# maxjaritz/mvpnet

Measured on AMD Instinct MI355X. Metric: chunks/sec (8192 pts, 3x160x120 views) fwd+bwd, higher is better.
Workload: dtype f32; 1 GPU; configs[2]: MVPNet lifting (unproject + pixel k-NN + gather) + FeatureAggregation + PN2SSG full train step (fwd+loss+bwd+Adam), 2D CNN replaced by a resident 64-ch feature map; cfg=mvpnet_3d_unet_resnet34_pn2ssg.yaml, chunks_per_gpu=32, points=8192, views=3x160x120, feature_channels=64, k=3, parallelism=dp1 (one process per GPU, 1 grad all-reduce/step), launch=eager, cpu_affinity=32 logical cpus of 256 (0 .. 183)

## Files before the change

include/mvp_hip.h:

```cpp
#ifndef MVP_HIP_H_
#define MVP_HIP_H_

#include <stdint.h>

#ifdef __cplusplus
extern "C" {
#endif

typedef void* mvp_stream_t;

#define MVP_OK 0
#define MVP_EINVAL (-1)
#define MVP_EUNSUPPORTED (-2)
#define MVP_ENULL (-3)

const char* mvp_version(void);
const char* mvp_strerror(int code);

int mvp_set_fps_mode(int mode);

int mvp_fps_f32(const float* points, int64_t B, int64_t N, int64_t D, int64_t M, int64_t* index, mvp_stream_t stream);
int mvp_fps_f64(const double* points, int64_t B, int64_t N, int64_t D, int64_t M, int64_t* index, mvp_stream_t stream);
int mvp_fps_shape_f32(const float* points, int64_t B, int64_t N, int64_t D, int64_t M, int64_t* index, int shape, mvp_stream_t stream);
int mvp_fps_shape_f64(const double* points, int64_t B, int64_t N, int64_t D, int64_t M, int64_t* index, int shape, mvp_stream_t stream);
// ... 46 lines not shown

int mvp_knn_distance_f32(const float* query, const float* key, int64_t B, int64_t N1, int64_t N2, int64_t k,
                         int64_t* index, float* distance, mvp_stream_t stream);
int mvp_knn_distance_f64(const double* query, const double* key, int64_t B, int64_t N1, int64_t N2, int64_t k,
                         int64_t* index, double* distance, mvp_stream_t stream);
int mvp_knn3_weights_f32(const float* query, const float* key, int64_t B, int64_t N1, int64_t N2, float eps, int64_t* index,
                         float* weight, float* distance, mvp_stream_t stream);

int mvp_interpolate_forward_f32(const float* input, const int64_t* index, const float* weight, int64_t B, int64_t C,
                                int64_t N1, int64_t N2, float* out, mvp_stream_t stream);
int mvp_interpolate_forward_f64(const double* input, const int64_t* index, const double* weight, int64_t B,
                                int64_t C, int64_t N1, int64_t N2, double* out, mvp_stream_t stream);
int mvp_interpolate_backward_f32(const float* grad_out, const int64_t* index, const float* weight, int64_t B,
                                 int64_t C, int64_t N1, int64_t N2, float* grad_in, mvp_stream_t stream);
int mvp_interpolate_backward_f64(const double* grad_out, const int64_t* index, const double* weight, int64_t B,
                                 int64_t C, int64_t N1, int64_t N2, double* grad_in, mvp_stream_t stream);
int mvp_interpolate_forward_strided_f32(const float* input, int64_t sb, int64_t sc, int64_t sn, const int64_t* index, const float* weight,
                                        int64_t B, int64_t C, int64_t N1, int64_t N2, float* out, mvp_stream_t stream);
int mvp_interpolate_forward_strided_f64(const double* input, int64_t sb, int64_t sc, int64_t sn, const int64_t* index, const double* weight,
                                        int64_t B, int64_t C, int64_t N1, int64_t N2, double* out, mvp_stream_t stream);
int mvp_interpolate_backward_strided_f32(const float* grad_out, int64_t sb, int64_t sc, int64_t sn, const int64_t* index,
                                         const float* weight, int64_t B, int64_t C, int64_t N1, int64_t N2, float* grad_in,
                                         mvp_stream_t stream);
int mvp_interpolate_backward_strided_f64(const double* grad_out, int64_t sb, int64_t sc, int64_t sn, const int64_t* index,
                                         const double* weight, int64_t B, int64_t C, int64_t N1, int64_t N2, double* grad_in,
                                         mvp_stream_t stream);
int mvp_interpolate_forward_bf16(const uint16_t* input, const int64_t* index, const float* weight, int64_t B, int64_t C, int64_t N1,
                                 int64_t N2, uint16_t* out, mvp_stream_t stream);
int mvp_interpolate_backward_bf16(const uint16_t* grad_out, const int64_t* index, const float* weight, int64_t B, int64_t C, int64_t N1,
                                  int64_t N2, uint16_t* grad_in, mvp_stream_t stream);
int mvp_interpolate_forward_strided_bf16(const uint16_t* input, int64_t sb, int64_t sc, int64_t sn, const int64_t* index,
                                         const float* weight, int64_t B, int64_t C, int64_t N1, int64_t N2, uint16_t* out,
                                         mvp_stream_t stream);
int mvp_interpolate_backward_strided_bf16(const uint16_t* grad_out, int64_t sb, int64_t sc, int64_t sn, const int64_t* index,
                                          const float* weight, int64_t B, int64_t C, int64_t N1, int64_t N2, uint16_t* grad_in,
                                          mvp_stream_t stream);

int mvp_unproject_f32(const float* depth_m, const float* kinv, const float* pose, const float* box, int64_t B,
                      int64_t nv, int64_t h, int64_t w, float* image_xyz, uint8_t* mask, mvp_stream_t stream);
int mvp_unproject_u16(const uint16_t* depth_mm, const float* kinv, const float* pose, const float* box, int64_t B,
                      int64_t nv, int64_t h, int64_t w, float* image_xyz, uint8_t* mask, mvp_stream_t stream);

int mvp_pixel_knn_bruteforce_f32(const float* image_xyz, const uint8_t* mask, const float* points, int64_t B,
                                 int64_t P, int64_t N, int64_t k, int64_t* index, float* distance,
                                 mvp_stream_t stream);
int mvp_pixel_knn_projective_f32(const float* image_xyz, const uint8_t* mask, const float* points, const float* cam,
                                 const float* pose, int64_t B, int64_t nv, int64_t h, int64_t w, int64_t N,
                                 int64_t k, int64_t* index, float* distance, mvp_stream_t stream);

int mvp_lift_gather_f32(const float* feature, const float* image_xyz, const int64_t* index, int64_t B, int64_t P,
                        int64_t C, int64_t N, int64_t k, float* gfeature, float* gxyz, mvp_stream_t stream);
int mvp_lift_gather_backward_f32(const float* grad_gfeature, const int64_t* index, int64_t B, int64_t P, int64_t C,
                                 int64_t N, int64_t k, float* grad_feature, mvp_stream_t stream);

int64_t mvp_lift_workspace_bytes(int64_t B, int64_t nv, int64_t h, int64_t w, int64_t N);
int mvp_lift_f32(const void* depth, int depth_is_u16, const float* kinv, const float* cam, const float* pose,
                 const float* box, const float* points, const float* feature, int64_t B, int64_t nv, int64_t h,
                 int64_t w, int64_t N, int64_t C, int64_t k, void* workspace, int64_t* knn_index, float* gfeature,
                 float* gxyz, float* image_xyz, uint8_t* mask, mvp_stream_t stream);
int mvp_lift_aug_f32(const void* depth, int depth_is_u16, const float* kinv, const float* cam, const float* pose,
                     const float* box, const float* points, const float* feature, int64_t B, int64_t nv, int64_t h,
                     int64_t w, int64_t N, int64_t C, int64_t k, void* workspace, int64_t* knn_index, float* gfeature,
                     float* gxyz, float* image_xyz, uint8_t* mask, const uint8_t* flip, const double* rot, float* points_out,
                     mvp_stream_t stream);
int mvp_rotate_rows_f32(const float* xyz, const double* rot, int64_t B, int64_t R, float* out, mvp_stream_t stream);

#define MVP_OVERLAP_MAX_BASE 4096
int mvp_frame_overlap_f32(const float* depth_m, const float* kinv, const float* pose, const float* base_points, int64_t F, int64_t h,
                          int64_t w, int64_t nb, float radius, uint32_t* overlap_bits, mvp_stream_t stream);
int mvp_frame_overlap_u16(const uint16_t* depth_mm, const float* kinv, const float* pose, const float* base_points, int64_t F, int64_t h,
                          int64_t w, int64_t nb, float radius, uint32_t* overlap_bits, mvp_stream_t stream);

int mvp_select_frames_u32(const uint32_t* overlap_bits, const uint32_t* chunk_bits, int64_t F, int64_t C, int64_t W, int64_t n_pick,
                          int64_t* picked, int32_t* gain, mvp_stream_t stream);

int mvp_copy_slices_f32(const int64_t* table, int64_t n, mvp_stream_t stream);

int mvp_group_rows_f32(const float* feature, const float* xyz, const float* center, const int64_t* index, int64_t B,
                       int64_t N, int64_t C, int64_t M, int64_t K, int64_t ld, float* out, mvp_stream_t stream);
int mvp_group_rows_backward_f32(const float* grad_out, const int64_t* index, int64_t B, int64_t N, int64_t C, int64_t M,
                                int64_t K, int64_t ld, float* grad_feature, mvp_stream_t stream);
int mvp_relation_rows_f32(const float* feature, const float* src_xyz, const float* tgt_xyz, int64_t R, int64_t K, int64_t C,
                          float* out, mvp_stream_t stream);
int64_t mvp_group_lin_partial_count(int64_t B, int64_t C, int64_t M, int64_t K);
int mvp_group_lin_rows_f32(const float* zf, const float* xyz, const float* centre, const float* wxyz, const int64_t* index,
                           int64_t B, int64_t N, int64_t C, int64_t M, int64_t K, float* out, float* diff, double* stat,
                           double* partial, mvp_stream_t stream);
int mvp_group_lin_rows_bn_f32(const float* zf, const float* xyz, const float* centre, const float* wxyz, const int64_t* index, int64_t B,
                              int64_t N, int64_t C, int64_t M, int64_t K, float* out, float* diff, double* stat, double* partial, float eps,
                              float momentum, float* mean, float* invstd, float* running_mean, float* running_var,
                              int64_t* num_batches_tracked, mvp_stream_t stream);
int mvp_colstats_f32(const float* y, int64_t R, int64_t C, double* stat, double* partial, mvp_stream_t stream);
int64_t mvp_colstats_partial_count(int64_t R, int64_t C);
int mvp_interp_rows_f32(const float* feature, const int64_t* index, const float* weight, int64_t B, int64_t N1, int64_t C,
                        int64_t N2, int64_t ld, float* out, mvp_stream_t stream);
int mvp_csr_build_i64(const int64_t* index, int64_t B, int64_t E, int64_t N, int32_t* offsets, int32_t* slots, int32_t* cursor,
                      mvp_stream_t stream);
int mvp_csr_build_sorted_i64(const int64_t* index, int64_t B, int64_t E, int64_t N, int32_t* offsets, int32_t* slots, int32_t* cursor,
                             mvp_stream_t stream);
int mvp_gather_rows_backward_csr_f32(const float* grad_out, const int32_t* offsets, const int32_t* slots, const float* weight,
                                     int64_t B, int64_t N, int64_t C, int64_t E, int64_t S, int64_t ld, float* grad_feature,
                                     mvp_stream_t stream);
int mvp_gather_rows_backward_csr_finish_f32(const float* dz, const float* y, const float* mean, const float* invstd, const float* gamma,
                                            const double* stat, int training, const int32_t* offsets, const int32_t* slots, const float* weight,
                                            int64_t B, int64_t N, int64_t C, int64_t E, int64_t S, int64_t ld, float* grad_feature,
                                            mvp_stream_t stream);
int mvp_interp_add_rows_f32(const float* feature, const int64_t* index, const float* weight, const float* add, int64_t B, int64_t N1,
                            int64_t C, int64_t N2, float* out, double* stat, double* partial, mvp_stream_t stream);
int mvp_interp_add_rows_bn_f32(const float* feature, const int64_t* index, const float* weight, const float* add, int64_t B, int64_t N1,
                               int64_t C, int64_t N2, float* out, double* stat, double* partial, float eps, float momentum, float* mean,
                               float* invstd, float* running_mean, float* running_var, int64_t* num_batches_tracked, mvp_stream_t stream);
int mvp_interp_rows_backward_f32(const float* grad_out, const int64_t* index, const float* weight, int64_t B, int64_t N1,
                                 int64_t C, int64_t N2, int64_t ld, float* grad_feature, mvp_stream_t stream);
int mvp_bn_rows_forward_f32(const float* y, const float* gamma, const float* beta, int64_t G, int64_t K, int64_t C,
                            int training, float eps, float momentum, int relu, float* running_mean, float* running_var,
                            double* stat, float* mean, float* invstd, float* out, uint8_t* arg, double* partial,
                            mvp_stream_t stream);
int mvp_bn_rows_backward_f32(const float* dsrc, const float* out, const uint8_t* arg, const float* y, const float* mean,
                             const float* invstd, const float* gamma, const float* beta, int64_t G, int64_t K, int64_t C,
                             int relu, int training, double* stat, float* dy, float* dgamma, float* dbeta, double* partial,
                             mvp_stream_t stream);
int mvp_bn_rows_forward_dropout_f32(const float* y, const float* gamma, const float* beta, int64_t R, int64_t C, int training, float eps,
                                    float momentum, int relu, float* running_mean, float* running_var, double* stat, float* mean,
                                    float* invstd, float* out, double* partial, float drop_p, uint64_t seed, mvp_stream_t stream);
int mvp_bn_rows_backward_dropout_f32(const float* dsrc, const float* y, const float* mean, const float* invstd, const float* gamma,
                                     const float* beta, int64_t R, int64_t C, int relu, int training, double* stat, float* dy,
                                     float* dgamma, float* dbeta, double* partial, float drop_p, uint64_t seed, mvp_stream_t stream);
int mvp_bn_rows_backward_finish_f32(const float* dz, const float* y, const float* mean, const float* invstd,
                                    const float* gamma, const float* beta, int64_t R, int64_t C, int training,
                                    const double* stat, float* dy, float* dgamma, float* dbeta, mvp_stream_t stream);
int mvp_bn_finalize_f32(const double* stat, int64_t R, int64_t C, float eps, float momentum, float* mean, float* invstd,
                        float* running_mean, float* running_var, int64_t* num_batches_tracked, mvp_stream_t stream);
int mvp_sa_fused_forward_f32(const float* zf, const float* xyz, const float* centre, const int64_t* index, const float* wxyz, int64_t B,
                             int64_t N, int64_t M, int64_t K, int64_t C1, const float* bn1_mean, const float* bn1_invstd,
                             const float* bn1_gamma, const float* bn1_beta, const float* W2, int64_t C2, const float* bn2_mean,
                             const float* bn2_invstd, const float* bn2_gamma, const float* bn2_beta, const float* W3, int64_t C3,
                             const float* bn3_mean, const float* bn3_invstd, const float* bn3_gamma, const float* bn3_beta, float* out,
                             uint8_t* arg, mvp_stream_t stream);

int mvp_set_mlp_precision(int terms, int min_width);
int mvp_get_mlp_precision(void);
int mvp_set_mlp_precision_backward(int terms);
int mvp_get_mlp_precision_backward(void);
int mvp_mlp_precision_scope(int terms, int terms_backward);
int mvp_adam_step_f32(void* const* params, const void* const* grads, void* const* exp_avg, void* const* exp_avg_sq, const int64_t* numel,
                      int64_t n, double lr, double beta1, double beta2, double eps, double weight_decay, double step, mvp_stream_t stream);

int mvp_mlp_forward_bf16(const uint16_t* X, int64_t R, int64_t Cin, int64_t ldx, const float* W, int64_t ldw, int64_t Cout,
                         const float* bias, const float* scale, const float* shift, int relu, uint16_t* Y, int64_t ldy,
                         mvp_stream_t stream);

int mvp_set_mlp_stream(int on);

int mvp_mlp_forward_f32(const float* X, int64_t R, int64_t Cin, int64_t ldx, const float* W, int64_t ldw, int64_t Cout,
                        const float* act_mean, const float* act_invstd, const float* act_gamma, const float* act_beta,
                        const float* bias, float* Y, double* stat, double* partial, mvp_stream_t stream);
int mvp_mlp_forward_bn_f32(const float* X, int64_t R, int64_t Cin, int64_t ldx, const float* W, int64_t ldw, int64_t Cout,
                           const float* act_mean, const float* act_invstd, const float* act_gamma, const float* act_beta, float* Y,
                           double* stat, double* partial, float eps, float momentum, float* mean, float* invstd, float* running_mean,
                           float* running_var, int64_t* num_batches_tracked, mvp_stream_t stream);
int mvp_mlp_forward_rel_bn_f32(const float* X, int64_t R, int64_t Cin, int64_t ldx, const float* W, int64_t ldw, int64_t Cout, const float* rel,
                               const float* wrel, float* Y, double* stat, double* partial, float eps, float momentum, float* mean,
                               float* invstd, float* running_mean, float* running_var, int64_t* num_batches_tracked, mvp_stream_t stream);
int mvp_relation4_rows_f32(const float* src_xyz, const float* tgt_xyz, int64_t R, int64_t K, float* out, mvp_stream_t stream);
int mvp_mlp_forward_pool_f32(const float* X, int64_t R, int64_t Cin, int64_t ldx, const float* W, int64_t ldw, int64_t Cout,
                             const float* act_mean, const float* act_invstd, const float* act_gamma, const float* act_beta, float* ymax,
                             float* ymin, uint8_t* amax, uint8_t* amin, double* stat, double* partial, float eps, float momentum,
                             float* mean, float* invstd, float* running_mean, float* running_var, int64_t* num_batches_tracked,
                             mvp_stream_t stream);
int mvp_pool_finalize_f32(const float* ymax, const float* ymin, const uint8_t* amax, const uint8_t* amin, const float* mean,
                          const float* invstd, const float* gamma, const float* beta, int64_t G, int64_t C, int relu, float* out,
                          uint8_t* arg, float* ysel, mvp_stream_t stream);
int mvp_pool_backward_stats_f32(const float* dout, const float* out, const float* ysel, const float* mean, const float* invstd,
                                int64_t G, int64_t C, int relu, double* stat, double* partial, mvp_stream_t stream);
int mvp_mlp_input_grad_f32(const float* dY, int64_t R, int64_t Cout, const float* W, int64_t Cin, const float* y_prev,
                           const float* mean, const float* invstd, const float* gamma, const float* beta, float* dZ,
                           double* stat, double* partial, mvp_stream_t stream);
int mvp_mlp_input_grad_dropout_f32(const float* dY, int64_t R, int64_t Cout, const float* W, int64_t Cin, const float* y_prev,
                                   const float* mean, const float* invstd, const float* gamma, const float* beta, float drop_p,
                                   uint64_t drop_seed, float* dZ, double* stat, double* partial, mvp_stream_t stream);

int64_t mvp_mlp_layer_backward_partial_count(int64_t R, int64_t Cp);
int mvp_mlp_layer_backward_f32(const float* G, const float* Yi, const float* mean_i, const float* invstd_i, const float* gamma_i,
                               const double* stat_i, float* dgamma_i, float* dbeta_i, int training, const float* X, int64_t ldx,
                               const float* act_mean, const float* act_invstd, const float* act_gamma, const float* act_beta,
                               const float* W, int64_t ldw, int64_t R, int64_t C, int64_t Cp, float* dW, int64_t lddw, float* dZ,
                               double* stat_prev, double* partial, const float* pool_dout, const float* pool_out,
                               const uint8_t* pool_arg, mvp_stream_t stream);
int mvp_mlp_layer_backward_ws_f32(const float* G, const float* Yi, const float* mean_i, const float* invstd_i, const float* gamma_i,
                               const double* stat_i, float* dgamma_i, float* dbeta_i, int training, const float* X, int64_t ldx,
                               const float* act_mean, const float* act_invstd, const float* act_gamma, const float* act_beta,
                               const float* W, int64_t ldw, int64_t R, int64_t C, int64_t Cp, float* dW, int64_t lddw, float* dZ,
                               double* stat_prev, double* partial, const float* pool_dout, const float* pool_out,
                               const uint8_t* pool_arg, float* workspace, int64_t workspace_floats, mvp_stream_t stream);
int mvp_mlp_layer_backward_wide_p_f32(const float* G, const float* Yi, const float* mean_i, const float* invstd_i, const float* gamma_i,
                                      const float* beta_i, const double* stat_i, float* dgamma_i, float* dbeta_i, int training, int mode,
                                      float drop_p, uint64_t drop_seed, const float* X, int64_t ldx, const float* act_mean,
                                      const float* act_invstd, const float* act_gamma, const float* act_beta, const float* W, int64_t ldw,
                                      int64_t R, int64_t C, int64_t Cp, float* dW, int64_t lddw, float* dZ, double* stat_prev, int* ticket,
                                      float* workspace, int64_t workspace_floats, int precision, int precision_backward, mvp_stream_t stream);
int mvp_mlp_layer_backward_wide_pooled_p_f32(const float* G, const float* Yi, const float* mean_i, const float* invstd_i, const float* gamma_i,
                                             const float* beta_i, const double* stat_i, float* dgamma_i, float* dbeta_i, int training, int mode,
                                             int64_t pool_k, float drop_p, uint64_t drop_seed, const float* X, int64_t ldx, const float* act_mean,
                                             const float* act_invstd, const float* act_gamma, const float* act_beta, const float* W, int64_t ldw,
                                             int64_t R, int64_t C, int64_t Cp, float* dW, int64_t lddw, float* dZ, double* stat_prev, int* ticket,
                                             float* workspace, int64_t workspace_floats, int precision, int precision_backward, mvp_stream_t stream);
int mvp_mlp_weight_grad_finish_p_f32(const float* dZ, const float* Y, const float* mean, const float* invstd, const float* gamma, const double* stat,
                                     int training, const float* X, int64_t R, int64_t Cout, int64_t Cin, int64_t ldx, float* dW, int64_t lddw,
                                     float* workspace, int64_t workspace_floats, int precision, int precision_backward, mvp_stream_t stream);
int mvp_mlp_weight_grad_finish_rel_p_f32(const float* dZ, const float* Y, const float* mean, const float* invstd, const float* gamma, const double* stat,
                                         int training, const float* X, int64_t R, int64_t Cout, int64_t Cin, int64_t ldx, const float* REL, float* dW,
                                         float* dWrel, int64_t lddw, int precision, int precision_backward, mvp_stream_t stream);
int mvp_mlp_weight_grad_finish_act_p_f32(const float* dZ, const float* Y, const float* mean, const float* invstd, const float* gamma, const double* stat,
                                         int training, const float* X, int64_t R, int64_t Cout, int64_t Cin, int64_t ldx, const float* act_mean,
                                         const float* act_invstd, const float* act_gamma, const float* act_beta, float* dW, int64_t lddw,
                                         float* workspace, int64_t workspace_floats, int precision, int precision_backward, mvp_stream_t stream);
int64_t mvp_mlp_input_grad_wide_workspace_bytes(int64_t C, int64_t Cp);
int mvp_mlp_input_grad_wide_p_f32(const float* G, const float* Yi, const float* mean_i, const float* invstd_i, const float* gamma_i,
                                  const double* stat_i, float* dgamma_i, float* dbeta_i, int training, const float* X, int64_t ldx,
                                  const float* act_mean, const float* act_invstd, const float* act_gamma, const float* act_beta, const float* W,
                                  int64_t ldw, int64_t R, int64_t C, int64_t Cp, float* dZ, double* stat_prev, void* workspace,
                                  int64_t workspace_bytes, int precision, int precision_backward, mvp_stream_t stream);
int mvp_mlp_weight_grad_f32(const float* dY, const float* X, int64_t R, int64_t Cout, int64_t Cin, int64_t ldx,
                            const float* act_mean, const float* act_invstd, const float* act_gamma, const float* act_beta,
                            float* dW, int64_t lddw, mvp_stream_t stream);
int64_t mvp_mlp_weight_grad_workspace_floats(void);
int mvp_mlp_weight_grad_ws_f32(const float* dY, const float* X, int64_t R, int64_t Cout, int64_t Cin, int64_t ldx,
                               const float* act_mean, const float* act_invstd, const float* act_gamma, const float* act_beta,
                               float* dW, int64_t lddw, float* workspace, int64_t workspace_floats, mvp_stream_t stream);

int mvp_sa_train_forward_f32(int stage, const float* zf, const float* xyz, const float* centre, const int64_t* index, const float* wxyz,
                             int64_t B, int64_t N, int64_t M, int64_t K, int64_t C1, const float* bn1_mean, const float* bn1_invstd,
                             const float* bn1_gamma, const float* bn1_beta, const float* W2, int64_t C2, const float* bn2_mean,
                             const float* bn2_invstd, const float* bn2_gamma, const float* bn2_beta, const float* W3, int64_t C3,
                             double* stat, float eps, float momentum, float* mean, float* invstd, float* running_mean,
                             float* running_var, int64_t* num_batches_tracked, float* ymax, float* ymin, uint8_t* amax, uint8_t* amin,
                             mvp_stream_t stream);
int mvp_sa_train_backward_f32(int layer, const float* zf, const float* xyz, const float* centre, const int64_t* index, const float* wxyz,
                              int64_t B, int64_t N, int64_t M, int64_t K, int64_t C1, const float* bn1_mean, const float* bn1_invstd,
                              const float* bn1_gamma, const float* bn1_beta, const float* W2, int64_t C2, const float* bn2_mean,
                              const float* bn2_invstd, const float* bn2_gamma, const float* bn2_beta, const float* W3, int64_t C3,
                              const float* mean_i, const float* invstd_i, const float* gamma_i, const double* stat_i, float* dgamma_i,
                              float* dbeta_i, int training, const float* G, const float* pool_dout, const float* pool_out,
                              const uint8_t* pool_arg, float* dW, int64_t lddw, float* dZ, double* stat_prev, float* tsum, mvp_stream_t stream);
int mvp_sa_train_backward1_f32(const float* dz1, const int32_t* offsets, const int32_t* slots, const float* zf, const float* dsum,
                               const float* wxyz, const float* tsum, const double* zsum, const double* gsum, int64_t B, int64_t N, int64_t M,
                               int64_t K, int64_t C1, const float* mean, const float* invstd, const float* gamma, const double* stat,
                               int training, float* dgamma, float* dbeta, float* gz, float* dWxyz, int64_t lddw, mvp_stream_t stream);
int mvp_sa_geom_sums_f32(const int32_t* offsets, const int32_t* slots, const float* xyz, const float* centre, int64_t B, int64_t N, int64_t M,
                         int64_t K, float* dsum, double* gsum, mvp_stream_t stream);
int mvp_sa_train_stats1_f32(const float* zf, const float* dsum, const float* wxyz, const double* gsum, int64_t B, int64_t N, int64_t M, int64_t K,
                            int64_t C1, double* stat, double* zsum, float eps, float momentum, float* mean, float* invstd, float* running_mean,
                            float* running_var, int64_t* num_batches_tracked, mvp_stream_t stream);
int mvp_sa_train_stats1_ws_f32(const float* zf, const float* dsum, const float* wxyz, const double* gsum, int64_t B, int64_t N, int64_t M, int64_t K,
                               int64_t C1, double* stat, double* zsum, float eps, float momentum, float* mean, float* invstd, float* running_mean,
                               float* running_var, int64_t* num_batches_tracked, double* scratch, int64_t scratch_doubles, mvp_stream_t stream);

int mvp_mlp_forward_p_f32(const float* X, int64_t R, int64_t Cin, int64_t ldx, const float* W, int64_t ldw, int64_t Cout, const
    float* act_mean, const float* act_invstd, const float* act_gamma, const float* act_beta, const float* bias, float* Y,
    double* stat, double* partial, int precision, int precision_backward, mvp_stream_t stream);
int mvp_mlp_forward_bn_p_f32(const float* X, int64_t R, int64_t Cin, int64_t ldx, const float* W, int64_t ldw, int64_t Cout,
    const float* act_mean, const float* act_invstd, const float* act_gamma, const float* act_beta, float* Y, double* stat,
    double* partial, float eps, float momentum, float* mean, float* invstd, float* running_mean, float* running_var, int64_t*
    num_batches_tracked, int precision, int precision_backward, mvp_stream_t stream);
int mvp_mlp_forward_rel_bn_p_f32(const float* X, int64_t R, int64_t Cin, int64_t ldx, const float* W, int64_t ldw, int64_t Cout,
    const float* rel, const float* wrel, float* Y, double* stat, double* partial, float eps, float momentum, float* mean, float*
    invstd, float* running_mean, float* running_var, int64_t* num_batches_tracked, int precision, int precision_backward,
    mvp_stream_t stream);
int mvp_mlp_forward_pool_p_f32(const float* X, int64_t R, int64_t Cin, int64_t ldx, const float* W, int64_t ldw, int64_t Cout,
    const float* act_mean, const float* act_invstd, const float* act_gamma, const float* act_beta, float* ymax, float* ymin,
    uint8_t* amax, uint8_t* amin, double* stat, double* partial, float eps, float momentum, float* mean, float* invstd, float*
    running_mean, float* running_var, int64_t* num_batches_tracked, int precision, int precision_backward, mvp_stream_t stream);
int mvp_mlp_input_grad_p_f32(const float* dY, int64_t R, int64_t Cout, const float* W, int64_t Cin, const float* y_prev, const
    float* mean, const float* invstd, const float* gamma, const float* beta, float* dZ, double* stat, double* partial, int
    precision, int precision_backward, mvp_stream_t stream);
int mvp_mlp_input_grad_dropout_p_f32(const float* dY, int64_t R, int64_t Cout, const float* W, int64_t Cin, const float* y_prev, const
    float* mean, const float* invstd, const float* gamma, const float* beta, float drop_p, uint64_t drop_seed, float* dZ, double* stat,
    double* partial, int precision, int precision_backward, mvp_stream_t stream);
int mvp_mlp_weight_grad_p_f32(const float* dY, const float* X, int64_t R, int64_t Cout, int64_t Cin, int64_t ldx, const float*
    act_mean, const float* act_invstd, const float* act_gamma, const float* act_beta, float* dW, int64_t lddw, int precision,
    int precision_backward, mvp_stream_t stream);
int mvp_mlp_weight_grad_ws_p_f32(const float* dY, const float* X, int64_t R, int64_t Cout, int64_t Cin, int64_t ldx, const
    float* act_mean, const float* act_invstd, const float* act_gamma, const float* act_beta, float* dW, int64_t lddw, float*
    workspace, int64_t workspace_floats, int precision, int precision_backward, mvp_stream_t stream);
int mvp_mlp_layer_backward_p_f32(const float* G, const float* Yi, const float* mean_i, const float* invstd_i, const float*
    gamma_i, const double* stat_i, float* dgamma_i, float* dbeta_i, int training, const float* X, int64_t ldx, const float*
    act_mean, const float* act_invstd, const float* act_gamma, const float* act_beta, const float* W, int64_t ldw, int64_t R,
    int64_t C, int64_t Cp, float* dW, int64_t lddw, float* dZ, double* stat_prev, double* partial, const float* pool_dout, const
    float* pool_out, const uint8_t* pool_arg, int precision, int precision_backward, mvp_stream_t stream);
int mvp_mlp_layer_backward_ws_p_f32(const float* G, const float* Yi, const float* mean_i, const float* invstd_i, const float*
    gamma_i, const double* stat_i, float* dgamma_i, float* dbeta_i, int training, const float* X, int64_t ldx, const float*
    act_mean, const float* act_invstd, const float* act_gamma, const float* act_beta, const float* W, int64_t ldw, int64_t R,
    int64_t C, int64_t Cp, float* dW, int64_t lddw, float* dZ, double* stat_prev, double* partial, const float* pool_dout, const
    float* pool_out, const uint8_t* pool_arg, float* workspace, int64_t workspace_floats, int precision, int precision_backward,
    mvp_stream_t stream);
int mvp_sa_fused_forward_p_f32(const float* zf, const float* xyz, const float* centre, const int64_t* index, const float* wxyz,
    int64_t B, int64_t N, int64_t M, int64_t K, int64_t C1, const float* bn1_mean, const float* bn1_invstd, const float*
    bn1_gamma, const float* bn1_beta, const float* W2, int64_t C2, const float* bn2_mean, const float* bn2_invstd, const float*
    bn2_gamma, const float* bn2_beta, const float* W3, int64_t C3, const float* bn3_mean, const float* bn3_invstd, const float*
    bn3_gamma, const float* bn3_beta, float* out, uint8_t* arg, int precision, int precision_backward, mvp_stream_t stream);

int mvp_sa_train_forward_p_f32(int stage, const float* zf, const float* xyz, const float* centre, const int64_t* index, const
    float* wxyz, int64_t B, int64_t N, int64_t M, int64_t K, int64_t C1, const float* bn1_mean, const float* bn1_invstd, const
    float* bn1_gamma, const float* bn1_beta, const float* W2, int64_t C2, const float* bn2_mean, const float* bn2_invstd, const
    float* bn2_gamma, const float* bn2_beta, const float* W3, int64_t C3, double* stat, float eps, float momentum, float* mean,
    float* invstd, float* running_mean, float* running_var, int64_t* num_batches_tracked, float* ymax, float* ymin, uint8_t*
// ... 35 lines not shown
```

mvpnet_amd/_lib.py:

```python
import ctypes
import os

import torch

_HERE = os.path.dirname(os.path.abspath(__file__))
LIB_PATH = os.environ.get('MVP_LIBRARY') or os.path.join(_HERE, 'libmvp_hip.so')
_lib = None
MLP_PRECISIONS = {'fp32': 0, 'bf16': 1, 'bf16x3': 3, 'bf16x6': 6}

_i64 = ctypes.c_int64
_ptr = ctypes.c_void_p
_f32 = ctypes.c_float

_SIGNATURES = {
    'mvp_fps_f32': [_ptr, _i64, _i64, _i64, _i64, _ptr, _ptr],
    'mvp_fps_f64': [_ptr, _i64, _i64, _i64, _i64, _ptr, _ptr],
    'mvp_fps_shape_f32': [_ptr, _i64, _i64, _i64, _i64, _ptr, ctypes.c_int, _ptr],
    'mvp_fps_shape_f64': [_ptr, _i64, _i64, _i64, _i64, _ptr, ctypes.c_int, _ptr],
    'mvp_fps_checked_f32': [_ptr, _i64, _i64, _i64, _i64, _ptr, ctypes.c_int, _ptr, _ptr],
    'mvp_fps_centroid_levels_f32': [_ptr, _ptr, _i64, _i64, _i64, _i64, _i64, _ptr, _ptr, _ptr],
    'mvp_ball_query_f32': [_ptr, _ptr, _i64, _i64, _i64, _f32, _i64, _ptr, _ptr],
    'mvp_ball_query_f64': [_ptr, _ptr, _i64, _i64, _i64, _f32, _i64, _ptr, _ptr],
    'mvp_ball_query_distance_f32': [_ptr, _ptr, _i64, _i64, _i64, _f32, _i64, _ptr, _ptr, _ptr],
    'mvp_ball_query_distance_f64': [_ptr, _ptr, _i64, _i64, _i64, _f32, _i64, _ptr, _ptr, _ptr],
    'mvp_ball_query_grid_f32': [_ptr, _ptr, _i64, _i64, _i64, _f32, _i64, _ptr, _ptr, _ptr, _i64, _ptr],
    'mvp_knn3_grid_f32': [_ptr, _ptr, _i64, _i64, _i64, _f32, _ptr, _ptr, _ptr, _ptr, _i64, _ptr],
    'mvp_group_points_forward_strided_f32': [_ptr, _i64, _i64, _i64, _ptr, _i64, _i64, _i64, _i64, _i64, _ptr, _ptr],
    'mvp_group_points_backward_strided_f32': [_ptr, _i64, _i64, _i64, _i64, _ptr, _i64, _i64, _i64, _i64, _i64, _ptr, _ptr],
    'mvp_interpolate_forward_strided_f32': [_ptr, _i64, _i64, _i64, _ptr, _ptr, _i64, _i64, _i64, _i64, _ptr, _ptr],
    'mvp_interpolate_backward_strided_f32': [_ptr, _i64, _i64, _i64, _ptr, _ptr, _i64, _i64, _i64, _i64, _ptr, _ptr],
    'mvp_group_points_forward_strided_f64': [_ptr, _i64, _i64, _i64, _ptr, _i64, _i64, _i64, _i64, _i64, _ptr, _ptr],
    'mvp_group_points_forward_strided_bf16': [_ptr, _i64, _i64, _i64, _ptr, _i64, _i64, _i64, _i64, _i64, _ptr, _ptr],
    'mvp_group_points_backward_strided_f64': [_ptr, _i64, _i64, _i64, _i64, _ptr, _i64, _i64, _i64, _i64, _i64, _ptr, _ptr],
    'mvp_group_points_backward_strided_bf16': [_ptr, _i64, _i64, _i64, _i64, _ptr, _i64, _i64, _i64, _i64, _i64, _ptr, _ptr],
    'mvp_interpolate_forward_strided_f64': [_ptr, _i64, _i64, _i64, _ptr, _ptr, _i64, _i64, _i64, _i64, _ptr, _ptr],
    'mvp_interpolate_forward_strided_bf16': [_ptr, _i64, _i64, _i64, _ptr, _ptr, _i64, _i64, _i64, _i64, _ptr, _ptr],
    'mvp_interpolate_backward_strided_f64': [_ptr, _i64, _i64, _i64, _ptr, _ptr, _i64, _i64, _i64, _i64, _ptr, _ptr],
    'mvp_interpolate_backward_strided_bf16': [_ptr, _i64, _i64, _i64, _ptr, _ptr, _i64, _i64, _i64, _i64, _ptr, _ptr],
    'mvp_group_points_forward_f32': [_ptr, _ptr, _i64, _i64, _i64, _i64, _i64, _ptr, _ptr],
    'mvp_group_points_forward_f64': [_ptr, _ptr, _i64, _i64, _i64, _i64, _i64, _ptr, _ptr],
    'mvp_group_points_forward_bf16': [_ptr, _ptr, _i64, _i64, _i64, _i64, _i64, _ptr, _ptr],
    'mvp_group_points_backward_f32': [_ptr, _ptr, _i64, _i64, _i64, _i64, _i64, _ptr, _ptr],
    'mvp_group_points_backward_f64': [_ptr, _ptr, _i64, _i64, _i64, _i64, _i64, _ptr, _ptr],
    'mvp_group_points_backward_bf16': [_ptr, _ptr, _i64, _i64, _i64, _i64, _i64, _ptr, _ptr],
    'mvp_knn_distance_f32': [_ptr, _ptr, _i64, _i64, _i64, _i64, _ptr, _ptr, _ptr],
    'mvp_knn_distance_f64': [_ptr, _ptr, _i64, _i64, _i64, _i64, _ptr, _ptr, _ptr],
    'mvp_knn3_weights_f32': [_ptr, _ptr, _i64, _i64, _i64, _f32, _ptr, _ptr, _ptr, _ptr],
    'mvp_interpolate_forward_f32': [_ptr, _ptr, _ptr, _i64, _i64, _i64, _i64, _ptr, _ptr],
    'mvp_interpolate_forward_f64': [_ptr, _ptr, _ptr, _i64, _i64, _i64, _i64, _ptr, _ptr],
    'mvp_interpolate_forward_bf16': [_ptr, _ptr, _ptr, _i64, _i64, _i64, _i64, _ptr, _ptr],
    'mvp_interpolate_backward_f32': [_ptr, _ptr, _ptr, _i64, _i64, _i64, _i64, _ptr, _ptr],
    'mvp_interpolate_backward_f64': [_ptr, _ptr, _ptr, _i64, _i64, _i64, _i64, _ptr, _ptr],
    'mvp_interpolate_backward_bf16': [_ptr, _ptr, _ptr, _i64, _i64, _i64, _i64, _ptr, _ptr],
    'mvp_unproject_f32': [_ptr, _ptr, _ptr, _ptr, _i64, _i64, _i64, _i64, _ptr, _ptr, _ptr],
    'mvp_unproject_u16': [_ptr, _ptr, _ptr, _ptr, _i64, _i64, _i64, _i64, _ptr, _ptr, _ptr],
    'mvp_pixel_knn_bruteforce_f32': [_ptr, _ptr, _ptr, _i64, _i64, _i64, _i64, _ptr, _ptr, _ptr],
    'mvp_pixel_knn_projective_f32': [_ptr, _ptr, _ptr, _ptr, _ptr, _i64, _i64, _i64, _i64, _i64, _i64, _ptr, _ptr, _ptr],
    'mvp_lift_gather_f32': [_ptr, _ptr, _ptr, _i64, _i64, _i64, _i64, _i64, _ptr, _ptr, _ptr],
    'mvp_lift_gather_backward_f32': [_ptr, _ptr, _i64, _i64, _i64, _i64, _i64, _ptr, _ptr],
    'mvp_lift_f32': [_ptr, ctypes.c_int, _ptr, _ptr, _ptr, _ptr, _ptr, _ptr, _i64, _i64, _i64, _i64, _i64, _i64, _i64, _ptr,
                     _ptr, _ptr, _ptr, _ptr, _ptr, _ptr],
    'mvp_lift_aug_f32': [_ptr, ctypes.c_int, _ptr, _ptr, _ptr, _ptr, _ptr, _ptr, _i64, _i64, _i64, _i64, _i64, _i64, _i64, _ptr,
                         _ptr, _ptr, _ptr, _ptr, _ptr, _ptr, _ptr, _ptr, _ptr],
    'mvp_rotate_rows_f32': [_ptr, _ptr, _i64, _i64, _ptr, _ptr],
    'mvp_copy_slices_f32': [_ptr, _i64, _ptr],
    'mvp_group_rows_f32': [_ptr, _ptr, _ptr, _ptr, _i64, _i64, _i64, _i64, _i64, _i64, _ptr, _ptr],
    'mvp_group_rows_backward_f32': [_ptr, _ptr, _i64, _i64, _i64, _i64, _i64, _i64, _ptr, _ptr],
    'mvp_group_lin_rows_f32': [_ptr, _ptr, _ptr, _ptr, _ptr, _i64, _i64, _i64, _i64, _i64, _ptr, _ptr, _ptr, _ptr, _ptr],
    'mvp_group_lin_rows_bn_f32': [_ptr, _ptr, _ptr, _ptr, _ptr, _i64, _i64, _i64, _i64, _i64, _ptr, _ptr, _ptr, _ptr, _f32, _f32, _ptr, _ptr, _ptr, _ptr, _ptr, _ptr],
    'mvp_colstats_f32': [_ptr, _i64, _i64, _ptr, _ptr, _ptr],
    'mvp_relation_rows_f32': [_ptr, _ptr, _ptr, _i64, _i64, _i64, _ptr, _ptr],
    'mvp_interp_rows_f32': [_ptr, _ptr, _ptr, _i64, _i64, _i64, _i64, _i64, _ptr, _ptr],
    'mvp_mlp_forward_bf16': [_ptr, _i64, _i64, _i64, _ptr, _i64, _i64, _ptr, _ptr, _ptr, ctypes.c_int, _ptr, _i64, _ptr],
    'mvp_adam_step_f32': [_ptr, _ptr, _ptr, _ptr, _ptr, _i64] + [ctypes.c_double] * 6 + [_ptr],
    'mvp_csr_build_i64': [_ptr, _i64, _i64, _i64, _ptr, _ptr, _ptr, _ptr],
    'mvp_csr_build_sorted_i64': [_ptr, _i64, _i64, _i64, _ptr, _ptr, _ptr, _ptr],
    'mvp_gather_rows_backward_csr_f32': [_ptr, _ptr, _ptr, _ptr, _i64, _i64, _i64, _i64, _i64, _i64, _ptr, _ptr],
    'mvp_gather_rows_backward_csr_finish_f32': [_ptr, _ptr, _ptr, _ptr, _ptr, _ptr, ctypes.c_int, _ptr, _ptr, _ptr, _i64, _i64, _i64, _i64, _i64, _i64, _ptr, _ptr],
    'mvp_interp_add_rows_f32': [_ptr, _ptr, _ptr, _ptr, _i64, _i64, _i64, _i64, _ptr, _ptr, _ptr, _ptr],
    'mvp_interp_add_rows_bn_f32': [_ptr, _ptr, _ptr, _ptr, _i64, _i64, _i64, _i64, _ptr, _ptr, _ptr, _f32, _f32, _ptr, _ptr, _ptr, _ptr, _ptr, _ptr],
    'mvp_interp_rows_backward_f32': [_ptr, _ptr, _ptr, _i64, _i64, _i64, _i64, _i64, _ptr, _ptr],
    'mvp_bn_rows_forward_f32': [_ptr, _ptr, _ptr, _i64, _i64, _i64, ctypes.c_int, _f32, _f32, ctypes.c_int, _ptr, _ptr, _ptr, _ptr,
                                _ptr, _ptr, _ptr, _ptr, _ptr],
    'mvp_bn_rows_backward_f32': [_ptr, _ptr, _ptr, _ptr, _ptr, _ptr, _ptr, _ptr, _i64, _i64, _i64, ctypes.c_int, ctypes.c_int, _ptr,
                                 _ptr, _ptr, _ptr, _ptr, _ptr],
    'mvp_bn_rows_forward_dropout_f32': [_ptr, _ptr, _ptr, _i64, _i64, ctypes.c_int, _f32, _f32, ctypes.c_int, _ptr, _ptr, _ptr, _ptr, _ptr, _ptr,
                                        _ptr, _f32, ctypes.c_uint64, _ptr],
    'mvp_bn_rows_backward_dropout_f32': [_ptr, _ptr, _ptr, _ptr, _ptr, _ptr, _i64, _i64, ctypes.c_int, ctypes.c_int, _ptr, _ptr, _ptr, _ptr,
                                         _ptr, _f32, ctypes.c_uint64, _ptr],
    'mvp_bn_rows_backward_finish_f32': [_ptr, _ptr, _ptr, _ptr, _ptr, _ptr, _i64, _i64, ctypes.c_int, _ptr, _ptr, _ptr, _ptr, _ptr],
    'mvp_bn_finalize_f32': [_ptr, _i64, _i64, _f32, _f32, _ptr, _ptr, _ptr, _ptr, _ptr, _ptr],
    'mvp_mlp_weight_grad_f32': [_ptr, _ptr, _i64, _i64, _i64, _i64, _ptr, _ptr, _ptr, _ptr, _ptr, _i64, _ptr],
    'mvp_mlp_weight_grad_ws_f32': [_ptr, _ptr, _i64, _i64, _i64, _i64, _ptr, _ptr, _ptr, _ptr, _ptr, _i64, _ptr, _i64, _ptr],
    'mvp_mlp_input_grad_f32': [_ptr, _i64, _i64, _ptr, _i64, _ptr, _ptr, _ptr, _ptr, _ptr, _ptr, _ptr, _ptr, _ptr],
    'mvp_mlp_input_grad_dropout_f32': [_ptr, _i64, _i64, _ptr, _i64, _ptr, _ptr, _ptr, _ptr, _ptr, _f32, ctypes.c_uint64, _ptr, _ptr, _ptr, _ptr],
    'mvp_mlp_layer_backward_f32': [_ptr, _ptr, _ptr, _ptr, _ptr, _ptr, _ptr, _ptr, ctypes.c_int, _ptr, _i64, _ptr, _ptr, _ptr, _ptr, _ptr, _i64,
                                   _i64, _i64, _i64, _ptr, _i64, _ptr, _ptr, _ptr, _ptr, _ptr, _ptr, _ptr],
    'mvp_mlp_layer_backward_ws_f32': [_ptr, _ptr, _ptr, _ptr, _ptr, _ptr, _ptr, _ptr, ctypes.c_int, _ptr, _i64, _ptr, _ptr, _ptr, _ptr, _ptr, _i64,
                                   _i64, _i64, _i64, _ptr, _i64, _ptr, _ptr, _ptr, _ptr, _ptr, _ptr, _ptr, _i64, _ptr],
    'mvp_mlp_forward_pool_f32': [_ptr, _i64, _i64, _i64, _ptr, _i64, _i64, _ptr, _ptr, _ptr, _ptr, _ptr, _ptr, _ptr, _ptr, _ptr, _ptr, _f32, _f32,
                                 _ptr, _ptr, _ptr, _ptr, _ptr, _ptr],
    'mvp_pool_finalize_f32': [_ptr, _ptr, _ptr, _ptr, _ptr, _ptr, _ptr, _ptr, _i64, _i64, ctypes.c_int, _ptr, _ptr, _ptr, _ptr],
    'mvp_pool_backward_stats_f32': [_ptr, _ptr, _ptr, _ptr, _ptr, _i64, _i64, ctypes.c_int, _ptr, _ptr, _ptr],
    'mvp_sa_fused_forward_f32': [_ptr, _ptr, _ptr, _ptr, _ptr, _i64, _i64, _i64, _i64, _i64, _ptr, _ptr, _ptr, _ptr, _ptr, _i64, _ptr, _ptr, _ptr,
                                 _ptr, _ptr, _i64, _ptr, _ptr, _ptr, _ptr, _ptr, _ptr, _ptr],
    'mvp_sa_train_forward_f32': [ctypes.c_int, _ptr, _ptr, _ptr, _ptr, _ptr, _i64, _i64, _i64, _i64, _i64, _ptr, _ptr, _ptr, _ptr, _ptr, _i64, _ptr, _ptr,
                                 _ptr, _ptr, _ptr, _i64, _ptr, _f32, _f32, _ptr, _ptr, _ptr, _ptr, _ptr, _ptr, _ptr, _ptr, _ptr, _ptr],
    'mvp_sa_train_backward_f32': [ctypes.c_int, _ptr, _ptr, _ptr, _ptr, _ptr, _i64, _i64, _i64, _i64, _i64, _ptr, _ptr, _ptr, _ptr, _ptr, _i64, _ptr, _ptr,
                                  _ptr, _ptr, _ptr, _i64, _ptr, _ptr, _ptr, _ptr, _ptr, _ptr, ctypes.c_int, _ptr, _ptr, _ptr, _ptr, _ptr, _i64, _ptr, _ptr,
                                  _ptr, _ptr],
    'mvp_sa_train_backward1_f32': [_ptr, _ptr, _ptr, _ptr, _ptr, _ptr, _ptr, _ptr, _ptr, _i64, _i64, _i64, _i64, _i64, _ptr, _ptr, _ptr, _ptr,
                                   ctypes.c_int, _ptr, _ptr, _ptr, _ptr, _i64, _ptr],
    'mvp_pn2_plan_f32': [_ptr, _i64, _i64, _i64, _ptr, _ptr, _ptr, _ptr, ctypes.c_int, ctypes.c_int, _f32, _ptr, _i64, _ptr, _ptr, _ptr],
    'mvp_sa_geom_sums_f32': [_ptr, _ptr, _ptr, _ptr, _i64, _i64, _i64, _i64, _ptr, _ptr, _ptr],
    'mvp_sa_train_stats1_f32': [_ptr, _ptr, _ptr, _ptr, _i64, _i64, _i64, _i64, _i64, _ptr, _ptr, _f32, _f32, _ptr, _ptr, _ptr, _ptr, _ptr, _ptr],
    'mvp_sa_train_stats1_ws_f32': [_ptr, _ptr, _ptr, _ptr, _i64, _i64, _i64, _i64, _i64, _ptr, _ptr, _f32, _f32, _ptr, _ptr, _ptr, _ptr, _ptr, _ptr, _i64, _ptr],
    'mvp_mlp_forward_bn_f32': [_ptr, _i64, _i64, _i64, _ptr, _i64, _i64, _ptr, _ptr, _ptr, _ptr, _ptr, _ptr, _ptr, _f32, _f32, _ptr, _ptr, _ptr,
                               _ptr, _ptr, _ptr],
    'mvp_mlp_forward_rel_bn_f32': [_ptr, _i64, _i64, _i64, _ptr, _i64, _i64, _ptr, _ptr, _ptr, _ptr, _ptr, _f32, _f32, _ptr, _ptr, _ptr, _ptr, _ptr, _ptr],
    'mvp_relation4_rows_f32': [_ptr, _ptr, _i64, _i64, _ptr, _ptr],
    'mvp_mlp_forward_f32': [_ptr, _i64, _i64, _i64, _ptr, _i64, _i64, _ptr, _ptr, _ptr, _ptr, _ptr, _ptr, _ptr, _ptr, _ptr],
    'mvp_vote_accumulate_f32': [_ptr, _i64, _i64, _ptr, _i64, _i64, _ptr, _ptr, _ptr],
    'mvp_vote_gather_f32': [_ptr, _i64, _i64, _i64, _ptr, _i64, _ptr, _ptr, _i64, _i64, _ptr, _ptr, _ptr],
    'mvp_vote_finish_f32': [_ptr, _ptr, _i64, _i64, _ptr, _ptr, _ptr],
    'mvp_seg_loss_f32': [_ptr, _i64, _i64, _i64, _i64, _i64, _i64, _ptr, _ptr, _i64, _ptr, _ptr, _ptr],
    'mvp_seg_loss_backward_f32': [_ptr, _i64, _i64, _i64, _i64, _i64, _i64, _ptr, _ptr, _i64, _ptr, _ptr, _ptr, _i64, _i64, _i64, _ptr],
    'mvp_seg_confusion_f32': [_ptr, _i64, _i64, _i64, _i64, _i64, _i64, _ptr, _i64, _ptr, _ptr],
    'mvp_frame_overlap_f32': [_ptr, _ptr, _ptr, _ptr, _i64, _i64, _i64, _i64, _f32, _ptr, _ptr],
    'mvp_frame_overlap_u16': [_ptr, _ptr, _ptr, _ptr, _i64, _i64, _i64, _i64, _f32, _ptr, _ptr],
    'mvp_select_frames_u32': [_ptr, _ptr, _i64, _i64, _i64, _i64, _ptr, _ptr, _ptr],
}
for _n in ['mvp_mlp_forward_f32', 'mvp_mlp_forward_bn_f32', 'mvp_mlp_forward_rel_bn_f32', 'mvp_mlp_forward_pool_f32', 'mvp_mlp_input_grad_f32', 'mvp_mlp_input_grad_dropout_f32',
           'mvp_mlp_weight_grad_f32', 'mvp_mlp_weight_grad_ws_f32', 'mvp_mlp_layer_backward_f32', 'mvp_mlp_layer_backward_ws_f32',
           'mvp_sa_fused_forward_f32', 'mvp_sa_train_forward_f32', 'mvp_sa_train_backward_f32']:
    _SIGNATURES[_n[:-4] + '_p_f32'] = _SIGNATURES[_n][:-1] + [ctypes.c_int, ctypes.c_int, _ptr]
_SIGNATURES['mvp_mlp_layer_backward_wide_p_f32'] = [_ptr] * 9 + [ctypes.c_int, ctypes.c_int, _f32, ctypes.c_uint64, _ptr, _i64, _ptr, _ptr, _ptr, _ptr, _ptr, _i64,
                                                    _i64, _i64, _i64, _ptr, _i64, _ptr, _ptr, _ptr, _ptr, _i64, ctypes.c_int, ctypes.c_int, _ptr]
_SIGNATURES['mvp_mlp_layer_backward_wide_pooled_p_f32'] = [_ptr] * 9 + [ctypes.c_int, ctypes.c_int, _i64, _f32, ctypes.c_uint64, _ptr, _i64, _ptr, _ptr, _ptr, _ptr, _ptr, _i64,
                                                           _i64, _i64, _i64, _ptr, _i64, _ptr, _ptr, _ptr, _ptr, _i64, ctypes.c_int, ctypes.c_int, _ptr]
_SIGNATURES['mvp_mlp_weight_grad_finish_p_f32'] = [_ptr] * 6 + [ctypes.c_int, _ptr, _i64, _i64, _i64, _i64, _ptr, _i64, _ptr, _i64, ctypes.c_int, ctypes.c_int, _ptr]
_SIGNATURES['mvp_mlp_weight_grad_finish_rel_p_f32'] = [_ptr] * 6 + [ctypes.c_int, _ptr, _i64, _i64, _i64, _i64, _ptr, _ptr, _ptr, _i64, ctypes.c_int, ctypes.c_int, _ptr]
_SIGNATURES['mvp_mlp_weight_grad_finish_act_p_f32'] = [_ptr] * 6 + [ctypes.c_int, _ptr, _i64, _i64, _i64, _i64, _ptr, _ptr, _ptr, _ptr, _ptr, _i64, _ptr, _i64, ctypes.c_int,
                                                        ctypes.c_int, _ptr]
_SIGNATURES['mvp_mlp_input_grad_wide_p_f32'] = [_ptr] * 8 + [ctypes.c_int, _ptr, _i64, _ptr, _ptr, _ptr, _ptr, _ptr, _i64, _i64, _i64, _i64, _ptr, _ptr, _ptr, _i64,
                                                 ctypes.c_int, ctypes.c_int, _ptr]
EXPORTS = ['mvp_version', 'mvp_strerror', 'mvp_lift_workspace_bytes', 'mvp_ball_query_grid_workspace', 'mvp_knn3_grid_workspace', 'mvp_mlp_weight_grad_workspace_floats', 'mvp_mlp_input_grad_wide_workspace_bytes', 'mvp_group_lin_partial_count', 'mvp_colstats_partial_count',
           'mvp_set_mlp_precision', 'mvp_get_mlp_precision', 'mvp_mlp_layer_backward_partial_count', 'mvp_set_mlp_stream', 'mvp_set_mlp_precision_backward', 'mvp_get_mlp_precision_backward', 'mvp_mlp_precision_scope', 'mvp_set_fps_mode', 'mvp_fps_debug_spin_limit', 'mvp_fps_last_kernel'] + sorted(_SIGNATURES)


def lib():
    global _lib
    if _lib is None:
        if not os.path.exists(LIB_PATH):
            raise RuntimeError('libmvp_hip.so is not built: run `python -c "import __graft_entry__ as g; g.build()"` '
                               'or `make -C mvpnet_amd/csrc` ({})'.format(LIB_PATH))
        handle = ctypes.CDLL(LIB_PATH)
        handle.mvp_version.restype = ctypes.c_char_p
        handle.mvp_strerror.restype = ctypes.c_char_p
        handle.mvp_strerror.argtypes = [ctypes.c_int]
        handle.mvp_lift_workspace_bytes.restype = ctypes.c_int64
        handle.mvp_lift_workspace_bytes.argtypes = [_i64, _i64, _i64, _i64, _i64]
        handle.mvp_ball_query_grid_workspace.restype = ctypes.c_int64
        handle.mvp_ball_query_grid_workspace.argtypes = [_i64, _i64, _i64]
        handle.mvp_knn3_grid_workspace.restype = ctypes.c_int64
        handle.mvp_knn3_grid_workspace.argtypes = [_i64, _i64, _i64]
        handle.mvp_group_lin_partial_count.restype = ctypes.c_int64
        handle.mvp_group_lin_partial_count.argtypes = [_i64, _i64, _i64, _i64]
        handle.mvp_mlp_weight_grad_workspace_floats.restype = ctypes.c_int64
        handle.mvp_mlp_weight_grad_workspace_floats.argtypes = []
        handle.mvp_mlp_input_grad_wide_workspace_bytes.restype = ctypes.c_int64
        handle.mvp_mlp_input_grad_wide_workspace_bytes.argtypes = [ctypes.c_int64, ctypes.c_int64]
        handle.mvp_colstats_partial_count.restype = ctypes.c_int64
        handle.mvp_colstats_partial_count.argtypes = [_i64, _i64]
        handle.mvp_set_mlp_precision.restype = ctypes.c_int
        handle.mvp_set_mlp_precision.argtypes = [ctypes.c_int, ctypes.c_int]
        handle.mvp_get_mlp_precision.restype = ctypes.c_int
        handle.mvp_get_mlp_precision.argtypes = []
        handle.mvp_mlp_layer_backward_partial_count.restype = ctypes.c_int64
        handle.mvp_mlp_layer_backward_partial_count.argtypes = [_i64, _i64]
        for name, argtypes in _SIGNATURES.items():
            fn = getattr(handle, name)
            fn.argtypes = argtypes
            fn.restype = ctypes.c_int
        _lib = handle
        handle.mvp_set_mlp_stream.restype = ctypes.c_int
        handle.mvp_set_mlp_stream.argtypes = [ctypes.c_int]
        handle.mvp_set_fps_mode.restype = ctypes.c_int
        handle.mvp_set_fps_mode.argtypes = [ctypes.c_int]
        handle.mvp_fps_debug_spin_limit.restype = ctypes.c_int
        handle.mvp_fps_debug_spin_limit.argtypes = [ctypes.c_int]
        handle.mvp_fps_last_kernel.restype = ctypes.c_int
        handle.mvp_fps_last_kernel.argtypes = []
        if os.environ.get('MVP_MLP_STREAM') is not None:
            handle.mvp_set_mlp_stream(int(os.environ['MVP_MLP_STREAM']))
        handle.mvp_set_mlp_precision_backward.restype = ctypes.c_int
        handle.mvp_set_mlp_precision_backward.argtypes = [ctypes.c_int]
        handle.mvp_get_mlp_precision_backward.restype = ctypes.c_int
        handle.mvp_get_mlp_precision_backward.argtypes = []
        handle.mvp_mlp_precision_scope.restype = ctypes.c_int
        handle.mvp_mlp_precision_scope.argtypes = [ctypes.c_int, ctypes.c_int]
        if os.environ.get('MVP_MLP_PRECISION_BWD'):
            check(handle.mvp_set_mlp_precision_backward(MLP_PRECISIONS[os.environ['MVP_MLP_PRECISION_BWD']]), 'mvp_set_mlp_precision_backward')
        env = os.environ.get('MVP_MLP_PRECISION')
        if env:
            set_mlp_precision(env, int(os.environ.get('MVP_MLP_MIN_WIDTH', '0')))
    return _lib




def set_mlp_precision(name, min_width=0):
    if name not in MLP_PRECISIONS:
        raise ValueError('mlp precision must be one of {}'.format(sorted(MLP_PRECISIONS)))
    check(lib().mvp_set_mlp_precision(MLP_PRECISIONS[name], int(min_width)), 'mvp_set_mlp_precision')
    global _mlp_min_width
    _mlp_min_width = int(min_width)


_mlp_min_width = 0


def mlp_min_width():
    return _mlp_min_width


def set_mlp_precision_backward(name):
    if name not in ('bf16', 'bf16x3', 'bf16x6'):
        raise ValueError("backward mlp precision must be 'bf16', 'bf16x3' or 'bf16x6'")
    check(lib().mvp_set_mlp_precision_backward(MLP_PRECISIONS[name]), 'mvp_set_mlp_precision_backward')


class mlp_precision:

    def __init__(self, forward=None, backward=None):
        self.terms = -1 if forward is None else MLP_PRECISIONS[forward]
        self.bwd = -1 if backward is None else MLP_PRECISIONS[backward]
        if self.bwd == 0:
            raise ValueError("backward mlp precision must be 'bf16', 'bf16x3' or 'bf16x6'")

    def __enter__(self):
        old = lib().mvp_mlp_precision_scope(self.terms, self.bwd)
        if old < 0:
            check(old, 'mvp_mlp_precision_scope')
        self.old = (old // 16 - 1, old % 16 - 1)
        return self

    def __exit__(self, *exc):
        lib().mvp_mlp_precision_scope(*self.old)


def current_precision():
    h = lib()
    return (h.mvp_get_mlp_precision(), h.mvp_get_mlp_precision_backward())


def get_mlp_precision():
    terms = lib().mvp_get_mlp_precision()
    return {v: k for k, v in MLP_PRECISIONS.items()}[terms]


_FPS_STATUS = {}


def fps_status(device):
    t = _FPS_STATUS.get(device)
    if t is None:
        t = _FPS_STATUS[device] = torch.zeros(1, dtype=torch.int32, device=device)
    return t


def fps_timed_out(device=None, reset=False):
    device = torch.device('cuda', torch.cuda.current_device()) if device is None else torch.device(device)
    t = _FPS_STATUS.get(device)
    if t is None:
        return False
    hit = bool(int(t.item()))
    if reset:
        t.zero_()
    return hit


def check(code, what):
    if code != 0:
        raise RuntimeError('{} failed: {} (code {})'.format(what, lib().mvp_strerror(code).decode(), code))


def stream_of(t):
    return ctypes.c_void_p(torch.cuda.current_stream(t.device).cuda_stream)


def ptr(t):
    return None if t is None else t.data_ptr()


def ptr_at(t, element_offset):
    return t.data_ptr() + int(element_offset) * t.element_size()


def require_gpu(*tensors):
    for t in tensors:
        if t is None:
            continue
        if not t.is_cuda:
            raise RuntimeError('mvpnet_amd ops run on the GPU only (got a {} tensor); there is no CPU fallback'.format(t.device))
        if not t.is_contiguous():
            raise RuntimeError('tensor must be contiguous')


def suffix(t):
    if t.dtype == torch.float32:
        return 'f32'
    if t.dtype == torch.float64:
        return 'f64'
    raise RuntimeError('expected a float32 or float64 tensor, got {}'.format(t.dtype))


def value_suffix(t):
    return 'bf16' if t.dtype == torch.bfloat16 else suffix(t)


_FN = {}
_raw_stream = getattr(torch._C, '_cuda_getCurrentRawStream', None)
_raw_device = getattr(torch._C, '_cuda_getDevice', None)


def _fn(name):
    f = _FN.get(name)
    if f is None:
        f = _FN[name] = getattr(_lib if _lib is not None else lib(), name)
    return f


DW_WORKSPACE = os.environ.get('MVP_DETERMINISTIC', '0') == '1'


def set_deterministic(flag):
    global DW_WORKSPACE
    old, DW_WORKSPACE = DW_WORKSPACE, bool(flag)
    return old
# ... 55 lines not shown
```

mvpnet_amd/csrc/mlp.hip:

```cpp
#include "common.h"
#include "stats_reduce.h"
#include "mlp_common.h"
#include "dropout.h"
#include <algorithm>

int mvp_mlp_stream_forward(const float* X, int64_t R, int Cin, int ldx, const float* W, int ldw, int Cout, const float* act_mean,
                           const float* act_invstd, const float* act_gamma, const float* act_beta, const float* bias, float* Y,
                           double* stat, double* partial, int ns, float bn_eps, float bn_momentum, float* bn_mean, float* bn_invstd,
                           float* bn_running_mean, float* bn_running_var, int64_t* bn_num_batches, float* ymax, float* ymin,
                           uint8_t* amax, uint8_t* amin, hipStream_t s);

int g_mlp_terms = 6;
int g_mlp_terms_bwd = 3;
int g_mlp_min_width = 0;
thread_local int tl_mlp_terms = -1;
thread_local int tl_mlp_terms_bwd = -1;
int g_mlp_stream = 1;

namespace {


constexpr int kMT = 256;
constexpr int kBM = 128;


struct EpiBwd {
  const float* y;
  const float* mean;
  const float* invstd;
  const float* gamma;
  const float* beta;
  const float* rel;
  const float* wrel;
  Dropout drop;
};

#ifndef MVP_MFMA_PRIO
#define MVP_MFMA_PRIO 2
#endif
#ifndef MVP_DW_PRIO
#define MVP_DW_PRIO 2
#endif
constexpr int kMaxActCin = 512;

#ifndef MVP_MLP_WAVES128
#define MVP_MLP_WAVES128 3
#endif
template <int BN, int BK, bool WT, bool VEC, int ACT, int NS>
__global__ __launch_bounds__(kMT, (BN == 128 && VEC && WT && NS == 0) ? MVP_MLP_WAVES128 : (NS != 0 && BN == 128) ? 2 : 1) void mlp_fwd_kernel(const float* __restrict__ X, int64_t R, int Cin, int ldx,
                                                      const float* __restrict__ W, int ldw, int Cout,
                                                      InAct act, const float* __restrict__ bias, EpiBwd epi,
                                                      float* __restrict__ Y , double* __restrict__ stat,
                                                      double* __restrict__ partial) {
  static_assert(NS == 0 || (VEC && BK == 32), "split-bf16 needs the vector path and 32-wide slabs");
  constexpr int kLdB = BK + 4;
  constexpr int NT = BK / 8;
  constexpr int kColB = 80;
  constexpr int kPieceB = BN * kColB;
  constexpr int kBufB = NS == 0 ? BN * kLdB * 4 : NS * kPieceB;
  __shared__ __attribute__((aligned(16))) unsigned char BsRaw[2 * kBufB];
  float* const Bs0 = reinterpret_cast<float*>(BsRaw);
  __shared__ __attribute__((aligned(16))) float Ps[4][kMaxActCin];
  constexpr int kLdS = 36;
  constexpr int kSsFloats = 4 * 32 * kLdS;
  constexpr bool kAliasS = sizeof(float) * kSsFloats + sizeof(double) * 2 * 4 * BN <= (size_t)2 * kBufB;
  __shared__ __attribute__((aligned(16))) float Ss_own[kAliasS ? 4 : kSsFloats];
  float (*Ss)[32 * kLdS] = reinterpret_cast<float (*)[32 * kLdS]>(kAliasS ? Bs0 : &Ss_own[0]);
  static_assert(sizeof(double) * 2 * 4 * BN <= (size_t)2 * kBufB, "sred must fit in Bs");
  double (*sred)[4][BN] = reinterpret_cast<double (*)[4][BN]>(Bs0 + (kAliasS ? kSsFloats : 0));
  constexpr int NB = BN / 32;
  const int tid = threadIdx.x, lane = tid & 63, wave = tid >> 6;
  const int64_t row0 = (int64_t)blockIdx.x * kBM;
  const int col0 = blockIdx.y * BN;
  const int li = lane & 31, lh = lane >> 5;

  f32x16 acc[NB];
#pragma unroll
  for (int j = 0; j < NB; ++j)
#pragma unroll
    for (int i = 0; i < 16; ++i) acc[j][i] = 0.f;

  constexpr bool has_act = ACT != 0;
  constexpr bool act_lds = ACT == 1;
  if constexpr (act_lds) {
    for (int k = tid; k < min(kMaxActCin, (Cin + BK - 1) / BK * BK); k += kMT) {
      const int kc = min(k, Cin - 1);
      Ps[0][k] = act.mean[kc];
      Ps[1][k] = act.invstd[kc];
      Ps[2][k] = act.gamma[kc];
      Ps[3][k] = act.beta[kc];
    }
  }

  const int64_t arow = row0 + wave * 32 + li;
  const bool arow_ok = arow < R;
  const float* xrow = X + (size_t)(arow_ok ? arow : 0) * ldx;
  float4 an[NT];
  auto load_a = [&](int k0) {
#pragma unroll
    for (int t = 0; t < NT; ++t) {
      const int k = k0 + 8 * t + 4 * lh;
      if constexpr (VEC) {
        an[t] = *reinterpret_cast<const float4*>(xrow + min(k, Cin - 4));
      } else {
        an[t].x = xrow[min(k + 0, Cin - 1)];
        an[t].y = xrow[min(k + 1, Cin - 1)];
        an[t].z = xrow[min(k + 2, Cin - 1)];
        an[t].w = xrow[min(k + 3, Cin - 1)];
      }
    }
  };
  float ac[NT][4];
  auto activate = [&](int k0) {
#pragma unroll
    for (int t = 0; t < NT; ++t) {
      const int k = k0 + 8 * t + 4 * lh;
      float v[4] = {an[t].x, an[t].y, an[t].z, an[t].w};
      if constexpr (has_act) {
        float pm[4], pi[4], pg[4], pb[4];
        if constexpr (act_lds) {
          const float4 m4 = *reinterpret_cast<const float4*>(&Ps[0][k]), i4 = *reinterpret_cast<const float4*>(&Ps[1][k]);
          const float4 g4 = *reinterpret_cast<const float4*>(&Ps[2][k]), b4 = *reinterpret_cast<const float4*>(&Ps[3][k]);
          pm[0] = m4.x; pm[1] = m4.y; pm[2] = m4.z; pm[3] = m4.w;
          pi[0] = i4.x; pi[1] = i4.y; pi[2] = i4.z; pi[3] = i4.w;
          pg[0] = g4.x; pg[1] = g4.y; pg[2] = g4.z; pg[3] = g4.w;
          pb[0] = b4.x; pb[1] = b4.y; pb[2] = b4.z; pb[3] = b4.w;
        } else {
#pragma unroll
          for (int e = 0; e < 4; ++e) {
            const int kc = min(k + e, Cin - 1);
            pm[e] = act.mean[kc];
            pi[e] = act.invstd[kc];
            pg[e] = act.gamma[kc];
            pb[e] = act.beta[kc];
          }
        }
#pragma unroll
        for (int e = 0; e < 4; ++e) {
          const float a = ((v[e] - pm[e]) * pi[e]) * pg[e] + pb[e];
          v[e] = a > 0.f ? a : 0.f;
        }
      }
#pragma unroll
      for (int e = 0; e < 4; ++e) ac[t][e] = v[e];
    }
  };

  constexpr int LPC = BK / 4;
  constexpr int CPP = kMT / LPC;
  constexpr int NV = BN / CPP;
  constexpr int KH = BK / 32;
  float4 bn[WT ? NB * KH : NV];
  auto load_b = [&](int k0) {
    if constexpr (WT && NS != 0) {
      const int c = tid & 31, kq = (tid >> 5) * 4;
#pragma unroll
      for (int u = 0; u < NB; ++u) {
        const int co = min(col0 + u * 32 + c, Cout - 1);
        bn[u].x = W[(size_t)min(k0 + kq + 0, Cin - 1) * ldw + co];
        bn[u].y = W[(size_t)min(k0 + kq + 1, Cin - 1) * ldw + co];
        bn[u].z = W[(size_t)min(k0 + kq + 2, Cin - 1) * ldw + co];
        bn[u].w = W[(size_t)min(k0 + kq + 3, Cin - 1) * ldw + co];
      }
    } else if constexpr (!WT) {
      const int c = tid / LPC, k = k0 + (tid % LPC) * 4;
#pragma unroll
      for (int u = 0; u < NV; ++u) {
        const float* src = W + (size_t)min(col0 + u * CPP + c, Cout - 1) * ldw;
        if constexpr (VEC) {
          bn[u] = *reinterpret_cast<const float4*>(src + min(k, Cin - 4));
// ... 982 lines not shown
                                             float* dW, int64_t lddw, float* workspace, int64_t workspace_floats, int precision,
                                             int precision_backward, mvp_stream_t stream) {
  MVP_NONNULL(Y);
  MVP_NONNULL(mean);
  MVP_NONNULL(invstd);
  MVP_NONNULL(gamma);
  MVP_NONNULL(stat);
  MVP_REQUIRE((precision == -1 || precision == 0 || precision == 1 || precision == 3 || precision == 6) &&
              (precision_backward == -1 || precision_backward == 1 || precision_backward == 3 || precision_backward == 6));
  if (Cout % 4 != 0 || Cout <= 32 || ((uintptr_t)dZ | (uintptr_t)Y) % 16 != 0) return MVP_EUNSUPPORTED;
  const int old_terms = tl_mlp_terms, old_bwd = tl_mlp_terms_bwd;
  if (precision >= 0) tl_mlp_terms = precision;
  if (precision_backward >= 0) tl_mlp_terms_bwd = precision_backward;
  const DyFinish fin{Y, mean, invstd, gamma, stat, (training && R > 0) ? 1.0f / (float)R : 0.f};
  const int rc = weight_grad_impl(dZ, X, R, Cout, Cin, ldx, nullptr, nullptr, nullptr, nullptr, dW, lddw, workspace, workspace_floats, stream, &fin);
  tl_mlp_terms = old_terms;
  tl_mlp_terms_bwd = old_bwd;
  return rc;
}

MVP_API int mvp_mlp_weight_grad_finish_rel_p_f32(const float* dZ, const float* Y, const float* mean, const float* invstd, const float* gamma,
                                                 const double* stat, int training, const float* X, int64_t R, int64_t Cout, int64_t Cin, int64_t ldx,
                                                 const float* REL, float* dW, float* dWrel, int64_t lddw, int precision, int precision_backward,
                                                 mvp_stream_t stream) {
  MVP_NONNULL(dZ);
  MVP_NONNULL(Y);
  MVP_NONNULL(mean);
  MVP_NONNULL(invstd);
  MVP_NONNULL(gamma);
  MVP_NONNULL(stat);
  MVP_NONNULL(X);
  MVP_NONNULL(REL);
  MVP_NONNULL(dW);
  MVP_NONNULL(dWrel);
  MVP_REQUIRE(R >= 0 && Cin > 0 && Cout > 0 && ldx >= Cin && lddw >= Cin && lddw >= 4 && lddw < (1 << 24) && Cout < (1 << 20));
  MVP_REQUIRE((precision == -1 || precision == 0 || precision == 1 || precision == 3 || precision == 6) &&
              (precision_backward == -1 || precision_backward == 1 || precision_backward == 3 || precision_backward == 6));
  const int terms = precision >= 0 ? precision : mlp_terms();
  const int bwd = precision_backward >= 0 ? precision_backward : mlp_terms_bwd();
  const int ns = terms == 0 ? 0 : (bwd == 6 ? 3 : bwd == 1 ? 1 : 2);
  if ((ns != 1 && ns != 2) || Cout <= 32 || Cin <= 32 || Cin > 64 || std::max(Cin, Cout) < g_mlp_min_width) return MVP_EUNSUPPORTED;
  if (R == 0) return MVP_OK;
  hipStream_t s = static_cast<hipStream_t>(stream);
  static const int64_t wg_target = []() { const char* e = getenv("MVP_DW_WORKGROUPS"); return e ? (int64_t)atoi(e) : (int64_t)1024; }();
  const int64_t tiles = cdiv(Cout, 64);
  int64_t splits = std::min<int64_t>(cdiv(wg_target, tiles), 512);
  int64_t rows_per_block = cdiv(cdiv(R, splits), 64) * 64;
  if (rows_per_block < 256) rows_per_block = 256;
  splits = cdiv(R, rows_per_block);
  const DyFinish fin{Y, mean, invstd, gamma, stat, training ? 1.0f / (float)R : 0.f};
  const InAct act{nullptr, nullptr, nullptr, nullptr};
  dim3 grid((unsigned)tiles, 1, (unsigned)splits);
  if (ns == 1)
    hipLaunchKernelGGL((mlp_dw_bf_kernel<2, 2, 1, true, true>), grid, dim3(kMT), 0, s, dZ, X, R, (int)Cout, (int)Cin, (int)ldx, act, rows_per_block, dW,
                       (int)lddw, nullptr, fin, REL, dWrel);
  else
    hipLaunchKernelGGL((mlp_dw_bf_kernel<2, 2, 2, true, true>), grid, dim3(kMT), 0, s, dZ, X, R, (int)Cout, (int)Cin, (int)ldx, act, rows_per_block, dW,
                       (int)lddw, nullptr, fin, REL, dWrel);
  return mvp_launch_status();
}

MVP_API int mvp_mlp_weight_grad_finish_act_p_f32(const float* dZ, const float* Y, const float* mean, const float* invstd, const float* gamma,
                                                 const double* stat, int training, const float* X, int64_t R, int64_t Cout, int64_t Cin, int64_t ldx,
                                                 const float* act_mean, const float* act_invstd, const float* act_gamma, const float* act_beta,
                                                 float* dW, int64_t lddw, float* workspace, int64_t workspace_floats, int precision,
                                                 int precision_backward, mvp_stream_t stream) {
  MVP_NONNULL(Y);
  MVP_NONNULL(mean);
  MVP_NONNULL(invstd);
  MVP_NONNULL(gamma);
  MVP_NONNULL(stat);
  MVP_REQUIRE((precision == -1 || precision == 0 || precision == 1 || precision == 3 || precision == 6) &&
              (precision_backward == -1 || precision_backward == 1 || precision_backward == 3 || precision_backward == 6));
  if (Cout % 4 != 0 || Cout <= 32 || ((uintptr_t)dZ | (uintptr_t)Y) % 16 != 0 || (act_mean && Cin <= 32)) return MVP_EUNSUPPORTED;
  const int old_terms = tl_mlp_terms, old_bwd = tl_mlp_terms_bwd;
  if (precision >= 0) tl_mlp_terms = precision;
  if (precision_backward >= 0) tl_mlp_terms_bwd = precision_backward;
  const DyFinish fin{Y, mean, invstd, gamma, stat, (training && R > 0) ? 1.0f / (float)R : 0.f};
  const int rc = weight_grad_impl(dZ, X, R, Cout, Cin, ldx, act_mean, act_invstd, act_gamma, act_beta, dW, lddw, workspace, workspace_floats, stream, &fin);
  tl_mlp_terms = old_terms;
  tl_mlp_terms_bwd = old_bwd;
  return rc;
}

namespace {
int input_grad_impl(const float* dY, int64_t R, int64_t Cout, const float* W, int64_t Cin, const float* y_prev, const float* mean, const float* invstd,
                    const float* gamma, const float* beta, float drop_p, uint64_t drop_seed, float* dZ, double* stat, double* partial, mvp_stream_t stream) {
  MVP_NONNULL(dY);
  MVP_NONNULL(W);
  MVP_NONNULL(dZ);
  MVP_REQUIRE(R >= 0 && Cin > 0 && Cout > 0 && Cin < (1 << 20) && Cout < (1 << 20));
  if (y_prev) {
    MVP_NONNULL(mean);
    MVP_NONNULL(invstd);
    MVP_NONNULL(gamma);
    MVP_NONNULL(beta);
    MVP_NONNULL(stat);
  }
  hipStream_t s = static_cast<hipStream_t>(stream);
  if (R == 0) return MVP_OK;
  InAct act{nullptr, nullptr, nullptr, nullptr};
  EpiBwd epi{y_prev, mean, invstd, gamma, beta};
  if (make_dropout(y_prev ? drop_p : 0.f, drop_seed, R, Cin, 1, &epi.drop) != MVP_OK) return MVP_EINVAL;
  double* st = y_prev ? stat : nullptr;
  const unsigned gx = (unsigned)cdiv(R, kBM);
  launch_mlp<true>(dY, R, (int)Cout, (int)Cout, W, (int)Cin, (int)Cin, act, nullptr, epi, dZ, st, st ? partial : nullptr, s);
  if (st && partial)
    launch_stats_reduce(partial, (int64_t)gx, (int)(2 * Cin), stat, s);
  return mvp_launch_status();
}
}

MVP_API int mvp_mlp_input_grad_f32(const float* dY, int64_t R, int64_t Cout, const float* W, int64_t Cin,
                                   const float* y_prev, const float* mean, const float* invstd, const float* gamma,
                                   const float* beta, float* dZ, double* stat, double* partial, mvp_stream_t stream) {
  return input_grad_impl(dY, R, Cout, W, Cin, y_prev, mean, invstd, gamma, beta, 0.f, 0, dZ, stat, partial, stream);
}

MVP_API int mvp_mlp_input_grad_dropout_f32(const float* dY, int64_t R, int64_t Cout, const float* W, int64_t Cin, const float* y_prev, const float* mean,
                                           const float* invstd, const float* gamma, const float* beta, float drop_p, uint64_t drop_seed, float* dZ,
                                           double* stat, double* partial, mvp_stream_t stream) {
  MVP_NONNULL(y_prev);
  return input_grad_impl(dY, R, Cout, W, Cin, y_prev, mean, invstd, gamma, beta, drop_p, drop_seed, dZ, stat, partial, stream);
}

MVP_API int mvp_set_mlp_precision(int terms, int min_width) {
  MVP_REQUIRE(terms == 0 || terms == 1 || terms == 3 || terms == 6);
  MVP_REQUIRE(min_width >= 0);
  g_mlp_terms = terms;
  g_mlp_min_width = min_width;
  return MVP_OK;
}
MVP_API int mvp_get_mlp_precision(void) { return mlp_terms(); }
MVP_API int mvp_set_mlp_precision_backward(int terms) {
  MVP_REQUIRE(terms == 1 || terms == 3 || terms == 6);
  g_mlp_terms_bwd = terms;
  return MVP_OK;
}
MVP_API int mvp_get_mlp_precision_backward(void) { return mlp_terms_bwd(); }
MVP_API int mvp_mlp_precision_scope(int terms, int terms_backward) {
  if (!(terms == -1 || terms == 0 || terms == 1 || terms == 3 || terms == 6) ||
      !(terms_backward == -1 || terms_backward == 1 || terms_backward == 3 || terms_backward == 6))
    return MVP_EINVAL;
  const int old = (tl_mlp_terms + 1) * 16 + (tl_mlp_terms_bwd + 1);
  tl_mlp_terms = terms;
  tl_mlp_terms_bwd = terms_backward;
  return old;
}
MVP_API int mvp_set_mlp_stream(int on) {
  const int old = g_mlp_stream;
  g_mlp_stream = on ? 1 : 0;
  return old;
}
```

mvpnet_amd/csrc/mlp_common.h:

```cpp
#pragma once
#include "common.h"

extern int g_mlp_terms;
extern int g_mlp_terms_bwd;
extern int g_mlp_min_width;

extern thread_local int tl_mlp_terms;
extern thread_local int tl_mlp_terms_bwd;
static inline int mlp_terms() { return tl_mlp_terms >= 0 ? tl_mlp_terms : g_mlp_terms; }
static inline int mlp_terms_bwd() { return tl_mlp_terms_bwd >= 0 ? tl_mlp_terms_bwd : g_mlp_terms_bwd; }
static inline int mlp_fwd_pieces() { return mlp_terms() == 1 ? 1 : mlp_terms() == 3 ? 2 : mlp_terms() == 6 ? 3 : 0; }
static inline int mlp_bwd_pieces() { return mlp_terms() == 0 ? 0 : (mlp_terms_bwd() == 6 ? 3 : mlp_terms_bwd() == 1 ? 1 : 2); }

int mlp_dw_wide_launch(const float* G, const float* Yi, const float* mean_i, const float* invstd_i, const float* gamma_i, const double* stat_i,
                       float inv_rows, const float* X, int64_t ldx, const float* act_mean, const float* act_invstd, const float* act_gamma,
                       const float* act_beta, int64_t R, int64_t C, int64_t Cp, float* dW, int64_t lddw, int ns, hipStream_t s);

namespace {

struct InAct {
  const float* mean;
  const float* invstd;
  const float* gamma;
  const float* beta;
};

struct DyFinish {
  const float* Y;
  const float* mean;
  const float* invstd;
  const float* gamma;
  const double* stat;
  float inv_rows;
};

typedef float f32x16 __attribute__((ext_vector_type(16)));
typedef float f32x4 __attribute__((ext_vector_type(4)));
typedef __bf16 bf16x8 __attribute__((ext_vector_type(8)));
typedef __bf16 bf16x2 __attribute__((ext_vector_type(2)));
typedef unsigned u32x4 __attribute__((ext_vector_type(4)));

__device__ __forceinline__ unsigned pack_bf16(float x, float y) {
  bf16x2 p = {(__bf16)x, (__bf16)y};
  return __builtin_bit_cast(unsigned, p);
}
template <int NS>
__device__ __forceinline__ void split_pair(float x, float y, unsigned (&pc)[NS]) {
  pc[0] = pack_bf16(x, y);
  if constexpr (NS == 1) return;
  float rx = x - __uint_as_float(pc[0] << 16), ry = y - __uint_as_float(pc[0] & 0xffff0000u);
  pc[1] = pack_bf16(rx, ry);
  if constexpr (NS == 3) {
    rx -= __uint_as_float(pc[1] << 16);
    ry -= __uint_as_float(pc[1] & 0xffff0000u);
    pc[2] = pack_bf16(rx, ry);
  }
}
template <int NS> struct SplitPairs;
template <> struct SplitPairs<1> { static constexpr int N = 1; static constexpr int A[1] = {0}; static constexpr int B[1] = {0}; };
template <> struct SplitPairs<2> { static constexpr int N = 3; static constexpr int A[3] = {1, 0, 0}; static constexpr int B[3] = {0, 1, 0}; };
template <> struct SplitPairs<3> { static constexpr int N = 6; static constexpr int A[6] = {2, 0, 1, 1, 0, 0}; static constexpr int B[6] = {0, 2, 1, 0, 1, 0}; };


template <int TMB, int TNB>
__global__ __launch_bounds__(256) void dw_reduce_kernel(const float* __restrict__ ws, int splits, int tiles_x, int tiles_y, int Cout, int Cin,
                                                        float* __restrict__ dW, int lddw) {
  constexpr int NBLK = TMB * TNB;
  __shared__ float part[4][64];
  const int lane = threadIdx.x & 63, wave = threadIdx.x >> 6;
  const int e = blockIdx.x;
  const int i = e & 15, ab = (e >> 4) % NBLK, tile = (e >> 4) / NBLK;
  const int a = ab / TNB, b = ab % TNB;
  const int tx = tile / tiles_y, ty = tile % tiles_y;
  const size_t stride = (size_t)tiles_x * tiles_y * NBLK * 1024;
  const float* p = ws + (size_t)tile * (NBLK * 1024) + (size_t)(ab * 16 + i) * 64 + lane;
  float v0 = 0.f, v1 = 0.f, v2 = 0.f, v3 = 0.f;
  int sI = wave;
  for (; sI + 12 < splits; sI += 16) {
    v0 += p[(size_t)sI * stride];
    v1 += p[(size_t)(sI + 4) * stride];
    v2 += p[(size_t)(sI + 8) * stride];
    v3 += p[(size_t)(sI + 12) * stride];
  }
  for (; sI < splits; sI += 4) v0 += p[(size_t)sI * stride];
  part[wave][lane] = (v0 + v1) + (v2 + v3);
  __syncthreads();
  if (wave == 0) {
    const float sum = (part[0][lane] + part[1][lane]) + (part[2][lane] + part[3][lane]);
    const int co = tx * (32 * TMB) + 32 * a + (i & 3) + 8 * (i >> 2) + 4 * (lane >> 5);
    const int ci = ty * (32 * TNB) + 32 * b + (lane & 31);
    if (co < Cout && ci < Cin) dW[(size_t)co * lddw + ci] += sum;
  }
}


}
```

mvpnet_amd/csrc/mlp_stream.hip:

```cpp
#include "mlp_common.h"
#include "stats_reduce.h"
#include <algorithm>

namespace {

constexpr int kST = 256;
constexpr int kSLd = 36;

struct StreamArgs {
  const float* X;
  int64_t R;
  int Cin, ldx;
  const float* W;
  int ldw, Cout;
  InAct act;
  const float* bias;
  float* Y;
  double* partial;
  double* stat;
  int finalize;
  BnFinalize fin;
  int64_t tiles_per_wg;
  float* ymax;
  float* ymin;
  uint8_t* amax;
  uint8_t* amin;
};

template <int KS, int NB, bool ACT, int NS, bool POOL>
__global__ __launch_bounds__(kST) void mlp_stream_fwd_kernel(StreamArgs p) {
  using SP = SplitPairs<NS>;
  constexpr int kCols = NB * 32;
  constexpr int kWBytes = KS * NS * kCols * 64;
  __shared__ __attribute__((aligned(16))) unsigned char Wl[kWBytes];
  __shared__ __attribute__((aligned(16))) float Ps[4][KS * 32];
  __shared__ __attribute__((aligned(16))) float tiles[4][32 * kSLd];
  __shared__ double sred[2][4][kCols];
  const int tid = threadIdx.x, lane = tid & 63, wave = tid >> 6;
  const int li = lane & 31, lh = lane >> 5;
  const int Cin = p.Cin, Cout = p.Cout;

  for (int t = tid; t < kCols * KS * 8; t += kST) {
    const int co = t % kCols, kqi = t / kCols;
    const int k = 4 * kqi;
    float v[4];
#pragma unroll
    for (int e = 0; e < 4; ++e) v[e] = (co < Cout && k + e < Cin) ? p.W[(size_t)co * p.ldw + k + e] : 0.f;
    unsigned lo[NS], hi[NS];
    split_pair<NS>(v[0], v[1], lo);
    split_pair<NS>(v[2], v[3], hi);
    const int slab = kqi >> 3, kq = (kqi & 7) * 4;
    const int tt = kq >> 3, hh = (kq >> 2) & 1;
    const int unit = 2 * (tt >> 1) + hh, half = tt & 1;
#pragma unroll
    for (int pc = 0; pc < NS; ++pc)
      *reinterpret_cast<uint2*>(Wl + ((size_t)(slab * NS + pc) * kCols + co) * 64 + ((unit ^ ((co >> 2) & 3)) * 16) + half * 8) = make_uint2(lo[pc], hi[pc]);
  }
  if constexpr (ACT) {
    for (int k = tid; k < KS * 32; k += kST) {
      const int kc = min(k, Cin - 1);
      Ps[0][k] = p.act.mean[kc];
      Ps[1][k] = p.act.invstd[kc];
      Ps[2][k] = p.act.gamma[kc];
      Ps[3][k] = p.act.beta[kc];
    }
  }
  float bv[NB];
#pragma unroll
  for (int j = 0; j < NB; ++j) bv[j] = (p.bias && 32 * j + li < Cout) ? p.bias[32 * j + li] : 0.f;
  float ssum[NB], qsum[NB];
#pragma unroll
  for (int j = 0; j < NB; ++j) ssum[j] = qsum[j] = 0.f;
  __syncthreads();

  const int64_t ntiles = (p.R + 31) / 32;
  const int64_t t_begin = (int64_t)blockIdx.x * p.tiles_per_wg;
  const int64_t t_end = min(ntiles, t_begin + p.tiles_per_wg);
  float* st = tiles[wave];
  constexpr int PF = KS == 1 ? 3 : KS == 2 ? 2 : 1;
  float4 an[PF][KS][4];
  auto load_a = [&](float4 (&dst)[KS][4], int64_t t) {
    const int64_t row = min(t * 32 + li, p.R - 1);
    const float* xrow = p.X + (size_t)row * p.ldx;
#pragma unroll
    for (int sl = 0; sl < KS; ++sl)
#pragma unroll
      for (int tt = 0; tt < 4; ++tt) dst[sl][tt] = *reinterpret_cast<const float4*>(xrow + min(32 * sl + 8 * tt + 4 * lh, Cin - 4));
  };
#pragma unroll
  for (int u = 0; u < PF; ++u)
    if (t_begin + wave + 4 * u < t_end) load_a(an[u], t_begin + wave + 4 * u);
  for (int64_t tb = t_begin + wave; tb < t_end; tb += 4 * PF) {
#pragma unroll
   for (int u = 0; u < PF; ++u) {
    const int64_t t = tb + 4 * u;
    if (t >= t_end) break;
    float4 ac[KS][4];
#pragma unroll
    for (int sl = 0; sl < KS; ++sl)
#pragma unroll
      for (int tt = 0; tt < 4; ++tt) ac[sl][tt] = an[u][sl][tt];
    if (t + 4 * PF < t_end) load_a(an[u], t + 4 * PF);
    f32x16 acc[NB];
#pragma unroll
    for (int j = 0; j < NB; ++j)
#pragma unroll
      for (int i = 0; i < 16; ++i) acc[j][i] = 0.f;
#pragma unroll
    for (int sl = 0; sl < KS; ++sl) {
      float v[4][4];
#pragma unroll
      for (int tt = 0; tt < 4; ++tt) {
        v[tt][0] = ac[sl][tt].x; v[tt][1] = ac[sl][tt].y; v[tt][2] = ac[sl][tt].z; v[tt][3] = ac[sl][tt].w;
        if constexpr (ACT) {
          const int k = 32 * sl + 8 * tt + 4 * lh;
          const float4 m4 = *reinterpret_cast<const float4*>(&Ps[0][k]), i4 = *reinterpret_cast<const float4*>(&Ps[1][k]);
          const float4 g4 = *reinterpret_cast<const float4*>(&Ps[2][k]), b4 = *reinterpret_cast<const float4*>(&Ps[3][k]);
          const float pm[4] = {m4.x, m4.y, m4.z, m4.w}, pi[4] = {i4.x, i4.y, i4.z, i4.w};
          const float pg[4] = {g4.x, g4.y, g4.z, g4.w}, pb[4] = {b4.x, b4.y, b4.z, b4.w};
#pragma unroll
          for (int e = 0; e < 4; ++e) {
            const float a = ((v[tt][e] - pm[e]) * pi[e]) * pg[e] + pb[e];
            v[tt][e] = a > 0.f ? a : 0.f;
          }
        }
      }
#pragma unroll
      for (int s = 0; s < 2; ++s) {
        unsigned q0[NS], q1[NS], q2[NS], q3[NS];
        split_pair<NS>(v[2 * s][0], v[2 * s][1], q0);
        split_pair<NS>(v[2 * s][2], v[2 * s][3], q1);
        split_pair<NS>(v[2 * s + 1][0], v[2 * s + 1][1], q2);
        split_pair<NS>(v[2 * s + 1][2], v[2 * s + 1][3], q3);
        u32x4 af[NS];
#pragma unroll
        for (int pc = 0; pc < NS; ++pc) af[pc] = u32x4{q0[pc], q1[pc], q2[pc], q3[pc]};
        constexpr int JG = NB >= 2 ? 2 : 1;
#pragma unroll
        for (int j0 = 0; j0 < NB; j0 += JG) {
          u32x4 bfr[JG][NS];
#pragma unroll
          for (int jj = 0; jj < JG; ++jj) {
            const int co = 32 * (j0 + jj) + li;
#pragma unroll
            for (int pc = 0; pc < NS; ++pc)
              bfr[jj][pc] = *reinterpret_cast<const u32x4*>(Wl + ((size_t)(sl * NS + pc) * kCols + co) * 64 + (((2 * s + lh) ^ ((co >> 2) & 3)) * 16));
          }
#pragma unroll
          for (int qd = 0; qd < SP::N; ++qd)
#pragma unroll
            for (int jj = 0; jj < JG; ++jj)
              acc[j0 + jj] = __builtin_amdgcn_mfma_f32_32x32x16_bf16(__builtin_bit_cast(bf16x8, af[SP::A[qd]]),
                                                                     __builtin_bit_cast(bf16x8, bfr[jj][SP::B[qd]]), acc[j0 + jj], 0, 0, 0);
        }
      }
    }
    const int64_t r0 = t * 32;
#pragma unroll
    for (int j = 0; j < NB; ++j) {
      const bool cok = 32 * j + li < Cout;
      float s = 0.f, q = 0.f;
      if constexpr (POOL) {
        float vmax = -INFINITY, vmin = INFINITY;
        int rmax = 0, rmin = 0;
#pragma unroll
        for (int i = 0; i < 16; ++i) {
          const int m = (i & 3) + 8 * (i >> 2) + 4 * lh;
          const float y = acc[j][i] + bv[j];
          s += y;
          q += y * y;
          if (y > vmax) { vmax = y; rmax = m; }
          if (y < vmin) { vmin = y; rmin = m; }
        }
        const float omax = __shfl_xor(vmax, 32, kWave), omin = __shfl_xor(vmin, 32, kWave);
        const int ormax = __shfl_xor(rmax, 32, kWave), ormin = __shfl_xor(rmin, 32, kWave);
        if (omax > vmax || (omax == vmax && ormax < rmax)) { vmax = omax; rmax = ormax; }
        if (omin < vmin || (omin == vmin && ormin < rmin)) { vmin = omin; rmin = ormin; }
        if (lh == 0 && cok) {
          const size_t o = (size_t)t * Cout + 32 * j + li;
          p.ymax[o] = vmax;
          p.ymin[o] = vmin;
          p.amax[o] = (uint8_t)rmax;
          p.amin[o] = (uint8_t)rmin;
        }
        if (!cok) s = q = 0.f;
        ssum[j] += s;
        qsum[j] += q;
        continue;
      }
#pragma unroll
      for (int i = 0; i < 16; ++i) {
        const int m = (i & 3) + 8 * (i >> 2) + 4 * lh;
        float y = acc[j][i] + bv[j];
        y = (r0 + m < p.R && cok) ? y : 0.f;
        s += y;
        q += y * y;
        st[m * kSLd + li] = y;
      }
      ssum[j] += s;
      qsum[j] += q;
      __builtin_amdgcn_wave_barrier();
#pragma unroll
      for (int pp = 0; pp < 4; ++pp) {
        const int row = pp * 8 + (lane >> 3), c4 = (lane & 7) * 4;
        const f32x4 vv = *reinterpret_cast<const f32x4*>(st + row * kSLd + c4);
        const int64_t r = r0 + row;
        const int cc = 32 * j + c4;
        if (r < p.R && cc < Cout) __builtin_nontemporal_store(vv, reinterpret_cast<f32x4*>(p.Y + (size_t)r * Cout + cc));
      }
      __builtin_amdgcn_wave_barrier();
    }
   }
  }
  if (p.partial) {
#pragma unroll
    for (int j = 0; j < NB; ++j) {
      const float s = ssum[j] + __shfl_xor(ssum[j], 32, kWave), q = qsum[j] + __shfl_xor(qsum[j], 32, kWave);
      if (lane < 32) {
        sred[0][wave][32 * j + li] = (double)s;
        sred[1][wave][32 * j + li] = (double)q;
      }
    }
    __syncthreads();
    for (int col = tid; col < kCols; col += kST)
      if (col < Cout) {
        p.partial[((size_t)blockIdx.x * 2 + 0) * Cout + col] = sred[0][0][col] + sred[0][1][col] + sred[0][2][col] + sred[0][3][col];
        p.partial[((size_t)blockIdx.x * 2 + 1) * Cout + col] = sred[1][0][col] + sred[1][1][col] + sred[1][2][col] + sred[1][3][col];
      }
  } else if (p.stat) {
#pragma unroll
    for (int j = 0; j < NB; ++j) {
      const float s = ssum[j] + __shfl_xor(ssum[j], 32, kWave), q = qsum[j] + __shfl_xor(qsum[j], 32, kWave);
      if (lane < 32) {
        sred[0][wave][32 * j + li] = (double)s;
        sred[1][wave][32 * j + li] = (double)q;
      }
    }
    __syncthreads();
    for (int col = tid; col < kCols; col += kST)
      if (col < Cout) {
        atomicAdd(p.stat + col, sred[0][0][col] + sred[0][1][col] + sred[0][2][col] + sred[0][3][col]);
        atomicAdd(p.stat + Cout + col, sred[1][0][col] + sred[1][1][col] + sred[1][2][col] + sred[1][3][col]);
      }
    if (p.finalize) {
      __shared__ unsigned last;
      wait_vm_complete();
      __syncthreads();
      unsigned* ticket = reinterpret_cast<unsigned*>(p.stat + 2 * Cout);
      if (tid == 0) last = atomicAdd(ticket, 1u) == gridDim.x - 1 ? 1u : 0u;
      __syncthreads();
      if (!last) return;
      const BnFinalize& fin = p.fin;
      for (int c = tid; c < Cout; c += kST) {
        const double s1 = __hip_atomic_load(p.stat + c, __ATOMIC_RELAXED, __HIP_MEMORY_SCOPE_AGENT);
        const double s2 = __hip_atomic_load(p.stat + Cout + c, __ATOMIC_RELAXED, __HIP_MEMORY_SCOPE_AGENT);
        const double m = s1 / (double)fin.rows;
        double var = s2 / (double)fin.rows - m * m;
        if (var < 0.0) var = 0.0;
        fin.mean[c] = (float)m;
        fin.invstd[c] = (float)(1.0 / sqrt(var + (double)fin.eps));
        if (fin.running_mean) {
          const double unbiased = fin.rows > 1 ? var * ((double)fin.rows / (double)(fin.rows - 1)) : var;
          fin.running_mean[c] = (float)((1.0 - fin.momentum) * (double)fin.running_mean[c] + fin.momentum * m);
          fin.running_var[c] = (float)((1.0 - fin.momentum) * (double)fin.running_var[c] + fin.momentum * unbiased);
        }
      }
      if (tid == 0) {
        if (fin.num_batches_tracked) *fin.num_batches_tracked += 1;
        *ticket = 0u;
      }
    }
  }
}

template <int KS, int NB, int NS>
void launch_stream(const StreamArgs& a, unsigned grid, bool has_act, hipStream_t s) {
  if (a.ymax) {
    if (has_act) hipLaunchKernelGGL((mlp_stream_fwd_kernel<KS, NB, true, NS, true>), dim3(grid), dim3(kST), 0, s, a);
    else hipLaunchKernelGGL((mlp_stream_fwd_kernel<KS, NB, false, NS, true>), dim3(grid), dim3(kST), 0, s, a);
    return;
  }
  if (has_act) hipLaunchKernelGGL((mlp_stream_fwd_kernel<KS, NB, true, NS, false>), dim3(grid), dim3(kST), 0, s, a);
  else hipLaunchKernelGGL((mlp_stream_fwd_kernel<KS, NB, false, NS, false>), dim3(grid), dim3(kST), 0, s, a);
}

}

int mvp_mlp_stream_forward(const float* X, int64_t R, int Cin, int ldx, const float* W, int ldw, int Cout, const float* act_mean,
                           const float* act_invstd, const float* act_gamma, const float* act_beta, const float* bias, float* Y,
                           double* stat, double* partial, int ns, float bn_eps, float bn_momentum, float* bn_mean, float* bn_invstd,
                           float* bn_running_mean, float* bn_running_var, int64_t* bn_num_batches, float* ymax, float* ymin,
                           uint8_t* amax, uint8_t* amin, hipStream_t s) {
  const InAct act{act_mean, act_invstd, act_gamma, act_beta};
  if (ns == 0 || Cin > 128 || Cout > 128 || Cin < 4 || Cout % 4 != 0 || R < 32768 || (stat && !partial)) return MVP_EUNSUPPORTED;
  if (ldx % 4 != 0 || Cin % 4 != 0 || ((uintptr_t)X % 16) != 0 || (!ymax && ((uintptr_t)Y % 16) != 0)) return MVP_EUNSUPPORTED;
  if (ymax && R % 32 != 0) return MVP_EUNSUPPORTED;
  static const bool tail = []() { const char* e = getenv("MVP_STREAM_TAIL"); return !(e && e[0] == '0'); }();
  StreamArgs a{X, R, Cin, ldx, W, ldw, Cout, act, bias, Y, (stat && !tail) ? partial : nullptr, (stat && tail) ? stat : nullptr, bn_mean ? 1 : 0,
               BnFinalize{R, bn_eps, bn_momentum, bn_mean, bn_invstd, bn_running_mean, bn_running_var, bn_num_batches}, 0, ymax, ymin, amax, amin};
  const int64_t ntiles = cdiv(R, 32);
  const int ks = (int)cdiv(Cin, 32), nb = Cout <= 32 ? 1 : Cout <= 64 ? 2 : 4;
  const int64_t lds = (int64_t)ks * ns * nb * 32 * 64;
  const int64_t per_cu = std::max<int64_t>(1, std::min<int64_t>(4, (140 * 1024) / (lds + 24 * 1024)));
  int64_t wgs = std::min<int64_t>(256 * per_cu, std::min<int64_t>(cdiv(R, 128), cdiv(ntiles, 16)));
  wgs = std::max<int64_t>(wgs, 1);
  a.tiles_per_wg = cdiv(cdiv(ntiles, wgs), 4) * 4;
  const unsigned grid = (unsigned)cdiv(ntiles, a.tiles_per_wg);
  const bool has_act = act.mean != nullptr;
#define MVP_STREAM(KS_, NB_)                                                      \
  do {                                                                            \
    if (ns == 1) launch_stream<KS_, NB_, 1>(a, grid, has_act, s);                  \
    else if (ns == 2) launch_stream<KS_, NB_, 2>(a, grid, has_act, s);             \
    else launch_stream<KS_, NB_, 3>(a, grid, has_act, s);                          \
  } while (0)
#define MVP_STREAM_NB(KS_)                       \
  do {                                           \
    if (nb == 1) MVP_STREAM(KS_, 1);             \
    else if (nb == 2) MVP_STREAM(KS_, 2);        \
    else MVP_STREAM(KS_, 4);                     \
  } while (0)
  switch (ks) {
    case 1: MVP_STREAM_NB(1); break;
    case 2: MVP_STREAM_NB(2); break;
    case 3: MVP_STREAM_NB(3); break;
    default: MVP_STREAM_NB(4); break;
  }
#undef MVP_STREAM_NB
#undef MVP_STREAM
  int rc = mvp_launch_status();
  if (rc != MVP_OK) return rc;
  if (a.partial) {
    if (bn_mean)
      launch_stats_reduce_finalize(partial, (int64_t)grid, 2 * Cout, stat,
                                   BnFinalize{R, bn_eps, bn_momentum, bn_mean, bn_invstd, bn_running_mean, bn_running_var, bn_num_batches}, s);
    else
      launch_stats_reduce(partial, (int64_t)grid, 2 * Cout, stat, s);
  }
  return mvp_launch_status();
}
```

mvpnet_amd/csrc/sa_common.h:

```cpp
#pragma once
#include "mlp_common.h"

namespace {

constexpr int kFT = 256;
constexpr int kFLd = 36;


template <int NS>
__device__ __forceinline__ void stage_weight(unsigned char* Wl, const float* __restrict__ W, int Cout, int Cin, int cols, int slabs, int tid) {
  for (int t = tid; t < cols * slabs * 8; t += kFT) {
    const int co = t % cols, kqi = t / cols;
    const int k = 4 * kqi;
    float v[4];
#pragma unroll
    for (int e = 0; e < 4; ++e) v[e] = (co < Cout && k + e < Cin) ? W[(size_t)co * Cin + k + e] : 0.f;
    unsigned lo[NS], hi[NS];
    split_pair<NS>(v[0], v[1], lo);
    split_pair<NS>(v[2], v[3], hi);
    const int slab = kqi >> 3, kq = (kqi & 7) * 4;
    const int tt = kq >> 3, hh = (kq >> 2) & 1;
    const int unit = 2 * (tt >> 1) + hh, half = tt & 1;
#pragma unroll
    for (int pc = 0; pc < NS; ++pc)
      *reinterpret_cast<uint2*>(Wl + ((size_t)(slab * NS + pc) * cols + co) * 64 + ((unit ^ ((co >> 2) & 3)) * 16) + half * 8) = make_uint2(lo[pc], hi[pc]);
  }
}

template <int KS, int NB, int NS>
__device__ __forceinline__ void layer_mfma(const float (&v)[KS][4][4], const unsigned char* Wl, int li, int lh, f32x16 (&acc)[NB]) {
  using SP = SplitPairs<NS>;
  constexpr int kCols = NB * 32;
#pragma unroll
  for (int j = 0; j < NB; ++j)
#pragma unroll
    for (int i = 0; i < 16; ++i) acc[j][i] = 0.f;
#pragma unroll
  for (int sl = 0; sl < KS; ++sl)
#pragma unroll
    for (int s = 0; s < 2; ++s) {
      unsigned q0[NS], q1[NS], q2[NS], q3[NS];
      split_pair<NS>(v[sl][2 * s][0], v[sl][2 * s][1], q0);
      split_pair<NS>(v[sl][2 * s][2], v[sl][2 * s][3], q1);
      split_pair<NS>(v[sl][2 * s + 1][0], v[sl][2 * s + 1][1], q2);
      split_pair<NS>(v[sl][2 * s + 1][2], v[sl][2 * s + 1][3], q3);
      u32x4 af[NS];
#pragma unroll
      for (int pc = 0; pc < NS; ++pc) af[pc] = u32x4{q0[pc], q1[pc], q2[pc], q3[pc]};
      constexpr int JG = NB >= 2 ? 2 : 1;
#pragma unroll
      for (int j0 = 0; j0 < NB; j0 += JG) {
        u32x4 bfr[JG][NS];
#pragma unroll
        for (int jj = 0; jj < JG; ++jj) {
          const int co = 32 * (j0 + jj) + li;
#pragma unroll
          for (int pc = 0; pc < NS; ++pc)
            bfr[jj][pc] = *reinterpret_cast<const u32x4*>(Wl + ((size_t)(sl * NS + pc) * kCols + co) * 64 + (((2 * s + lh) ^ ((co >> 2) & 3)) * 16));
        }
#pragma unroll
        for (int qd = 0; qd < SP::N; ++qd)
#pragma unroll
          for (int jj = 0; jj < JG; ++jj)
            acc[j0 + jj] = __builtin_amdgcn_mfma_f32_32x32x16_bf16(__builtin_bit_cast(bf16x8, af[SP::A[qd]]),
                                                                   __builtin_bit_cast(bf16x8, bfr[jj][SP::B[qd]]), acc[j0 + jj], 0, 0, 0);
      }
    }
}


}
```

mvpnet_amd/csrc/sa_train.hip:

```cpp
#include "sa_common.h"
#include "stats_reduce.h"
#include <algorithm>
#include <stdlib.h>

namespace {

struct SaSrc {
  const float* zf;
  const float* xyz;
  const float* centre;
  const int64_t* index;
  const float* wxyz;
  const float* bn1[4];
  int64_t G;
  int N, M, C1;
};

template <int C1B>
__device__ __forceinline__ void stage_layer1(const SaSrc& p, float* P1 , float (*Wx)[4], int tid) {
  for (int k = tid; k < C1B * 32; k += kFT) {
    const int kc = min(k, p.C1 - 1);
#pragma unroll
    for (int a = 0; a < 4; ++a) P1[a * (C1B * 32) + k] = p.bn1[a] ? p.bn1[a][kc] : 0.f;
    Wx[k][0] = k < p.C1 ? p.wxyz[k * 3 + 0] : 0.f;
    Wx[k][1] = k < p.C1 ? p.wxyz[k * 3 + 1] : 0.f;
    Wx[k][2] = k < p.C1 ? p.wxyz[k * 3 + 2] : 0.f;
    Wx[k][3] = 0.f;
  }
}

template <int C1B>
struct BallRows {
  float4 z[C1B][4];
  float p[3], q[3];
  bool ok;
};
template <int C1B>
__device__ __forceinline__ void gather_issue(const SaSrc& p, int g, int64_t j, int lh, BallRows<C1B>& r) {
  const int b = g / p.M;
  r.ok = j >= 0 && j < p.N;
  const unsigned jj = r.ok ? (unsigned)j : 0u;
  const float* zr = p.zf + (size_t)b * p.N * p.C1 + jj * (unsigned)p.C1;
#pragma unroll
  for (int sl = 0; sl < C1B; ++sl)
#pragma unroll
    for (int tt = 0; tt < 4; ++tt) r.z[sl][tt] = *reinterpret_cast<const float4*>(zr + min(32 * sl + 8 * tt + 4 * lh, p.C1 - 4));
  const float* pp = p.xyz + (size_t)b * p.N * 3 + jj * 3u;
  const float* qc = p.centre + (size_t)g * 3;
  r.p[0] = pp[0]; r.p[1] = pp[1]; r.p[2] = pp[2];
  r.q[0] = qc[0]; r.q[1] = qc[1]; r.q[2] = qc[2];
}
template <int C1B>
__device__ __forceinline__ void gather_finish(const BallRows<C1B>& r, int lh, const float (*Wx)[4], float (&v)[C1B][4][4], float (&diff)[3]) {
  const bool ok = r.ok;
  const float dx = r.p[0] - r.q[0], dy = r.p[1] - r.q[1], dz = r.p[2] - r.q[2];
  diff[0] = ok ? dx : 0.f;
  diff[1] = ok ? dy : 0.f;
  diff[2] = ok ? dz : 0.f;
#pragma unroll
  for (int sl = 0; sl < C1B; ++sl)
#pragma unroll
    for (int tt = 0; tt < 4; ++tt) {
      const int k = 32 * sl + 8 * tt + 4 * lh;
      const float zz[4] = {r.z[sl][tt].x, r.z[sl][tt].y, r.z[sl][tt].z, r.z[sl][tt].w};
#pragma unroll
      for (int e = 0; e < 4; ++e) {
        const float4 w = *reinterpret_cast<const float4*>(&Wx[k + e][0]);
        float y = (w.x * dx + w.y * dy) + w.z * dz;
        y = y + zz[e];
        v[sl][tt][e] = ok ? y : 0.f;
      }
    }
}

template <int C1B>
__device__ __forceinline__ void act_rows(float (&v)[C1B][4][4], const float* P1, int lh) {
#pragma unroll
  for (int sl = 0; sl < C1B; ++sl)
#pragma unroll
    for (int tt = 0; tt < 4; ++tt) {
      const int k = 32 * sl + 8 * tt + 4 * lh;
      const float4 mm = *reinterpret_cast<const float4*>(P1 + 0 * (C1B * 32) + k), ii = *reinterpret_cast<const float4*>(P1 + 1 * (C1B * 32) + k);
      const float4 gg = *reinterpret_cast<const float4*>(P1 + 2 * (C1B * 32) + k), bb = *reinterpret_cast<const float4*>(P1 + 3 * (C1B * 32) + k);
      const float pm[4] = {mm.x, mm.y, mm.z, mm.w}, pi[4] = {ii.x, ii.y, ii.z, ii.w};
      const float pg[4] = {gg.x, gg.y, gg.z, gg.w}, pb[4] = {bb.x, bb.y, bb.z, bb.w};
#pragma unroll
      for (int e = 0; e < 4; ++e) {
        const float a = ((v[sl][tt][e] - pm[e]) * pi[e]) * pg[e] + pb[e];
        v[sl][tt][e] = a > 0.f ? a : 0.f;
      }
    }
}

template <int NB>
__device__ __forceinline__ void stats_tail(const float (&ssum)[NB], const float (&qsum)[NB], double (*sred)[4][NB * 32], double* stat, int C,
                                           const BnFinalize& fin, bool finalize) {
  const int tid = threadIdx.x, lane = tid & 63, wave = tid >> 6, li = lane & 31;
#pragma unroll
  for (int j = 0; j < NB; ++j) {
    const float s = ssum[j] + __shfl_xor(ssum[j], 32, kWave), q = qsum[j] + __shfl_xor(qsum[j], 32, kWave);
    if (lane < 32) {
      sred[0][wave][32 * j + li] = (double)s;
      sred[1][wave][32 * j + li] = (double)q;
    }
  }
  __syncthreads();
  for (int col = tid; col < NB * 32; col += kFT)
    if (col < C) {
      atomicAdd(stat + col, sred[0][0][col] + sred[0][1][col] + sred[0][2][col] + sred[0][3][col]);
      atomicAdd(stat + C + col, sred[1][0][col] + sred[1][1][col] + sred[1][2][col] + sred[1][3][col]);
    }
  if (!finalize) return;
  __shared__ unsigned last;
  wait_vm_complete();
  __syncthreads();
  unsigned* ticket = reinterpret_cast<unsigned*>(stat + 2 * C);
  if (tid == 0) last = atomicAdd(ticket, 1u) == gridDim.x - 1 ? 1u : 0u;
  __syncthreads();
  if (!last) return;
  for (int c = tid; c < C; c += kFT) {
    const double s1 = __hip_atomic_load(stat + c, __ATOMIC_RELAXED, __HIP_MEMORY_SCOPE_AGENT);
    const double s2 = __hip_atomic_load(stat + C + c, __ATOMIC_RELAXED, __HIP_MEMORY_SCOPE_AGENT);
    const double m = s1 / (double)fin.rows;
    double var = s2 / (double)fin.rows - m * m;
    if (var < 0.0) var = 0.0;
    fin.mean[c] = (float)m;
    fin.invstd[c] = (float)(1.0 / sqrt(var + (double)fin.eps));
    if (fin.running_mean) {
      const double unbiased = fin.rows > 1 ? var * ((double)fin.rows / (double)(fin.rows - 1)) : var;
      fin.running_mean[c] = (float)((1.0 - fin.momentum) * (double)fin.running_mean[c] + fin.momentum * m);
      fin.running_var[c] = (float)((1.0 - fin.momentum) * (double)fin.running_var[c] + fin.momentum * unbiased);
    }
  }
  if (tid == 0) {
    if (fin.num_batches_tracked) *fin.num_batches_tracked += 1;
    *ticket = 0u;
  }
}

struct SaFwdArgs {
  SaSrc s;
  const float* W2;
  const float* bn2[4];
  const float* W3;
  int C2, C3;
  double* stat;
  BnFinalize fin;
  float* ymax;
  float* ymin;
  uint8_t* amax;
  uint8_t* amin;
  int64_t tiles_per_wg;
};

template <int C1B, int C2B, int C3B, int NS, int STAGE>
__global__ __launch_bounds__(kFT) void sa_train_fwd_kernel(SaFwdArgs p) {
  constexpr bool PF = STAGE == 2;
  constexpr int kW2 = C1B * NS * C2B * 32 * 64;
  constexpr int kW3 = STAGE == 3 ? C2B * NS * C3B * 32 * 64 : 16;
  constexpr int NBS = STAGE == 3 ? C3B : C2B;
  __shared__ __attribute__((aligned(16))) unsigned char W2l[kW2];
  __shared__ __attribute__((aligned(16))) unsigned char W3l[kW3];
  __shared__ __attribute__((aligned(16))) float P1[4 * C1B * 32];
  __shared__ __attribute__((aligned(16))) float Wx[C1B * 32][4];
  __shared__ __attribute__((aligned(16))) float tiles[4][32 * kFLd];
  __shared__ double sred[2][4][NBS * 32];
  const int tid = threadIdx.x, lane = tid & 63, wave = tid >> 6;
  const int li = lane & 31, lh = lane >> 5;
  const int C1 = p.s.C1, C2 = p.C2, C3 = p.C3;
  stage_weight<NS>(W2l, p.W2, C2, C1, C2B * 32, C1B, tid);
  if constexpr (STAGE == 3) stage_weight<NS>(W3l, p.W3, C3, C2, C3B * 32, C2B, tid);
  stage_layer1<C1B>(p.s, P1, Wx, tid);
  float m2[C2B], i2[C2B], g2[C2B], b2[C2B];
#pragma unroll
  for (int j = 0; j < C2B; ++j) {
    m2[j] = i2[j] = g2[j] = b2[j] = 0.f;
    if constexpr (STAGE == 3) {
      const int col = min(32 * j + li, C2 - 1);
      m2[j] = p.bn2[0][col]; i2[j] = p.bn2[1][col]; g2[j] = p.bn2[2][col]; b2[j] = p.bn2[3][col];
    }
  }
  float ssum[NBS], qsum[NBS];
#pragma unroll
  for (int j = 0; j < NBS; ++j) ssum[j] = qsum[j] = 0.f;
  __syncthreads();
  float* st = tiles[wave];
  const int64_t t_begin = (int64_t)blockIdx.x * p.tiles_per_wg;
  const int64_t t_end = min(p.s.G, t_begin + p.tiles_per_wg);
  int g = __builtin_amdgcn_readfirstlane((int)(t_begin + wave));
  BallRows<C1B> rn;
  int64_t jn = -1;
  if (PF) {
    if (g < t_end) gather_issue<C1B>(p.s, g, p.s.index[(size_t)g * 32 + li], lh, rn);
    if (g + 4 < t_end) jn = p.s.index[(size_t)(g + 4) * 32 + li];
  } else if (g < t_end) {
    jn = p.s.index[(size_t)g * 32 + li];
  }
  for (; g < t_end; g += 4) {
    BallRows<C1B> rc = rn;
    if (PF && g + 4 < t_end) {
      gather_issue<C1B>(p.s, g + 4, jn, lh, rn);
      if (g + 8 < t_end) jn = p.s.index[(size_t)(g + 8) * 32 + li];
    }
    if (!PF) {
      const int64_t j = jn;
      if (g + 4 < t_end) jn = p.s.index[(size_t)(g + 4) * 32 + li];
      gather_issue<C1B>(p.s, g, j, lh, rc);
    }
    float v1[C1B][4][4], dif[3];
    gather_finish<C1B>(rc, lh, Wx, v1, dif);
    act_rows<C1B>(v1, P1, lh);
    f32x16 acc2[C2B];
    layer_mfma<C1B, C2B, NS>(v1, W2l, li, lh, acc2);
    if constexpr (STAGE == 2) {
#pragma unroll
      for (int jb = 0; jb < C2B; ++jb) {
        float s = 0.f, q = 0.f;
#pragma unroll
        for (int i = 0; i < 16; ++i) {
          const float y = acc2[jb][i];
          s += y;
          q += y * y;
        }
        ssum[jb] += s;
        qsum[jb] += q;
      }
    } else {
      float v2[C2B][4][4];
#pragma unroll
      for (int jb = 0; jb < C2B; ++jb) {
#pragma unroll
        for (int i = 0; i < 16; ++i) {
          const int m = (i & 3) + 8 * (i >> 2) + 4 * lh;
          const float a = ((acc2[jb][i] - m2[jb]) * i2[jb]) * g2[jb] + b2[jb];
          st[m * kFLd + li] = a > 0.f ? a : 0.f;
        }
        __builtin_amdgcn_wave_barrier();
#pragma unroll
        for (int tt = 0; tt < 4; ++tt) {
          const float4 a = *reinterpret_cast<const float4*>(st + li * kFLd + 8 * tt + 4 * lh);
          v2[jb][tt][0] = a.x; v2[jb][tt][1] = a.y; v2[jb][tt][2] = a.z; v2[jb][tt][3] = a.w;
        }
        __builtin_amdgcn_wave_barrier();
      }
      f32x16 acc3[C3B];
      layer_mfma<C2B, C3B, NS>(v2, W3l, li, lh, acc3);
#pragma unroll
      for (int jb = 0; jb < C3B; ++jb) {
        const bool cok = 32 * jb + li < C3;
        float s = 0.f, q = 0.f;
        float vmax = -INFINITY, vmin = INFINITY;
        int rmax = 0, rmin = 0;
#pragma unroll
        for (int i = 0; i < 16; ++i) {
          const int m = (i & 3) + 8 * (i >> 2) + 4 * lh;
          const float y = acc3[jb][i];
          s += y;
          q += y * y;
          if (y > vmax) { vmax = y; rmax = m; }
          if (y < vmin) { vmin = y; rmin = m; }
        }
        const float omax = __shfl_xor(vmax, 32, kWave), omin = __shfl_xor(vmin, 32, kWave);
        const int ormax = __shfl_xor(rmax, 32, kWave), ormin = __shfl_xor(rmin, 32, kWave);
        if (omax > vmax || (omax == vmax && ormax < rmax)) { vmax = omax; rmax = ormax; }
        if (omin < vmin || (omin == vmin && ormin < rmin)) { vmin = omin; rmin = ormin; }
        if (lh == 0 && cok) {
          const size_t ob = (size_t)g * C3;
          const unsigned o = (unsigned)(32 * jb + li);
          (p.ymax + ob)[o] = vmax;
          (p.ymin + ob)[o] = vmin;
          (p.amax + ob)[o] = (uint8_t)rmax;
          (p.amin + ob)[o] = (uint8_t)rmin;
        }
        if (!cok) s = q = 0.f;
        ssum[jb] += s;
        qsum[jb] += q;
      }
    }
  }
  stats_tail<NBS>(ssum, qsum, sred, p.stat, STAGE == 3 ? C3 : C2, p.fin, true);
}

struct SaBwdArgs {
  SaSrc s;
  const float* W2;
  const float* bn2[4];
  const float* W3;
  int C2, C3;
  const float* mean_i;
  const float* invstd_i;
  const float* gamma_i;
  const double* stat_i;
  float* dgamma_i;
  float* dbeta_i;
  float inv_rows;
  const float* G;
  const float* pool_dout;
  const float* pool_out;
  const uint8_t* pool_arg;
  float* dW;
  int lddw;
  float* dZ;
  double* stat_prev;
  float* tsum;
  int64_t tiles_per_wg;
};

template <int C1B, int C2B, int C3B, int NS, int LAYER, int NSF>
__global__ __launch_bounds__(kFT, ((LAYER == 3 ? C1B * C2B * C3B <= 2 : C1B * C2B == 1) ? 2 : 1)) void sa_train_bwd_kernel(SaBwdArgs p) {
  using SP = SplitPairs<NS>;
  constexpr bool PF = LAYER == 3;
  constexpr int CB = LAYER == 3 ? C3B : C2B;
  constexpr int CPB = LAYER == 3 ? C2B : C1B;
  constexpr int kW2f = C1B * NSF * C2B * 32 * 64;
  constexpr int kW3f = LAYER == 3 ? C2B * NS * C3B * 32 * 64 : 0;
  constexpr int kWb = NS * CB * CPB * 32 * 64;
  constexpr int kTileBytes = 4 * 32 * kFLd * 4;
  constexpr int kRedBytes = 2 * CB * CPB * 16 * 64 * 4;
  constexpr int kMain = kW2f + kW3f + kWb + kTileBytes;
  constexpr int kLds = kMain > kRedBytes ? kMain : kRedBytes;
  __shared__ __attribute__((aligned(16))) unsigned char lds[kLds];
  __shared__ __attribute__((aligned(16))) float P1[4 * C1B * 32];
  __shared__ __attribute__((aligned(16))) float Wx[C1B * 32][4];
  __shared__ __attribute__((aligned(16))) float dtile[4][32][4];
  __shared__ double sred[2][4][CPB * 32];
  unsigned char* W2f = lds;
  unsigned char* W3f = lds + kW2f;
  unsigned char* Wb = lds + kW2f + kW3f;
  const int tid = threadIdx.x, lane = tid & 63, wave = tid >> 6;
  const int c = lane & 31, h = lane >> 5;
  float* tile = reinterpret_cast<float*>(lds + kW2f + kW3f + kWb) + wave * 32 * kFLd;
  const int C1 = p.s.C1, C2 = p.C2, C3 = p.C3;
  const int C = LAYER == 3 ? C3 : C2, Cp = LAYER == 3 ? C2 : C1;
  const float* W = LAYER == 3 ? p.W3 : p.W2;

  stage_weight<NSF>(W2f, p.W2, C2, C1, C2B * 32, C1B, tid);
  if constexpr (LAYER == 3) stage_weight<NS>(W3f, p.W3, C3, C2, C3B * 32, C2B, tid);
  stage_layer1<C1B>(p.s, P1, Wx, tid);
  {
    const int quads = CB * 8;
    for (int t = tid; t < quads * CPB * 32; t += kFT) {
      const int ci = t % (CPB * 32), cq = t / (CPB * 32);
      const int co = 4 * cq;
      float v[4];
#pragma unroll
      for (int e = 0; e < 4; ++e) v[e] = (co + e < C && ci < Cp) ? W[(size_t)(co + e) * Cp + ci] : 0.f;
      unsigned lo[NS], hi[NS];
      split_pair<NS>(v[0], v[1], lo);
      split_pair<NS>(v[2], v[3], hi);
      const int a = cq >> 3, coq = cq & 7;
      const int tt = coq >> 1, hh = coq & 1;
      const int unit = 2 * (tt >> 1) + hh, half = tt & 1;
      const int sw = (ci >> 2) & 3;
#pragma unroll
      for (int pc = 0; pc < NS; ++pc)
        *reinterpret_cast<uint2*>(Wb + ((size_t)(pc * CB + a) * (CPB * 32) + ci) * 64 + ((unit ^ sw) * 16) + half * 8) = make_uint2(lo[pc], hi[pc]);
    }
  }
  if (p.dgamma_i && blockIdx.x == 0)
    for (int col = tid; col < C; col += kFT) {
      p.dbeta_i[col] = (float)p.stat_i[col];
      p.dgamma_i[col] = (float)p.stat_i[C + col];
    }
  float sc[CB], mu[CB], is[CB], db[CB], dg[CB];
  bool cok[CB];
#pragma unroll
  for (int a = 0; a < CB; ++a) {
    const int col = 32 * a + c;
    cok[a] = col < C;
    sc[a] = mu[a] = is[a] = db[a] = dg[a] = 0.f;
    if (cok[a]) {
      mu[a] = p.mean_i[col];
      is[a] = p.invstd_i[col];
      sc[a] = p.gamma_i[col] * is[a];
      db[a] = (float)p.stat_i[col] * p.inv_rows;
      dg[a] = (float)p.stat_i[C + col] * p.inv_rows;
    }
  }
  const float* const act_mean = LAYER == 3 ? p.bn2[0] : p.s.bn1[0];
  const float* const act_invstd = LAYER == 3 ? p.bn2[1] : p.s.bn1[1];
  const float* const act_gamma = LAYER == 3 ? p.bn2[2] : p.s.bn1[2];
  const float* const act_beta = LAYER == 3 ? p.bn2[3] : p.s.bn1[3];
  float pm[CPB], pi[CPB], pg[CPB], pb[CPB];
  bool xok[CPB];
#pragma unroll
  for (int b = 0; b < CPB; ++b) {
    const int col = 32 * b + c;
    xok[b] = col < Cp;
    pm[b] = pi[b] = pg[b] = pb[b] = 0.f;
    if (xok[b]) {
      pm[b] = act_mean[col];
      pi[b] = act_invstd[col];
      pg[b] = act_gamma[col];
      pb[b] = act_beta[col];
    }
  }
  f32x16 accw[CB][CPB];
#pragma unroll
  for (int a = 0; a < CB; ++a)
#pragma unroll
    for (int b = 0; b < CPB; ++b)
#pragma unroll
      for (int i = 0; i < 16; ++i) accw[a][b][i] = 0.f;
  float ssum[CPB], tsum[CPB], txs[CPB][3];
#pragma unroll
  for (int b = 0; b < CPB; ++b) ssum[b] = tsum[b] = txs[b][0] = txs[b][1] = txs[b][2] = 0.f;
  __syncthreads();

  const int64_t t_begin = (int64_t)blockIdx.x * p.tiles_per_wg;
  const int64_t t_end = min(p.s.G, t_begin + p.tiles_per_wg);
  int g = __builtin_amdgcn_readfirstlane((int)(t_begin + wave));
  BallRows<C1B> rn;
  int64_t jn = -1;
  if (PF) {
    if (g < t_end) gather_issue<C1B>(p.s, g, p.s.index[(size_t)g * 32 + c], h, rn);
    if (g + 4 < t_end) jn = p.s.index[(size_t)(g + 4) * 32 + c];
  } else if (g < t_end) {
    jn = p.s.index[(size_t)g * 32 + c];
  }
  for (; g < t_end; g += 4) {
    BallRows<C1B> rc = rn;
    if (PF && g + 4 < t_end) {
      gather_issue<C1B>(p.s, g + 4, jn, h, rn);
      if (g + 8 < t_end) jn = p.s.index[(size_t)(g + 8) * 32 + c];
    }
    if (!PF) {
      const int64_t j = jn;
      if (g + 4 < t_end) jn = p.s.index[(size_t)(g + 4) * 32 + c];
      gather_issue<C1B>(p.s, g, j, h, rc);
    }
    float gn[16];
    auto load_g = [&](int a) {
      const float* Gt = p.G + (size_t)g * 32 * C;
// ... 372 lines not shown
      for (int u = 0; u < 20; ++u) tot[u] += (double)red[gq * C4 + c4][u];
    if (blockIdx.x == 0) {
      const double* S = p.gsum;
#pragma unroll
      for (int i = 0; i < 4; ++i) {
        const double a = w[i][0], b = w[i][1], cc = w[i][2];
        tot[i] += a * S[0] + b * S[1] + cc * S[2];
        tot[4 + i] += a * a * S[3] + b * b * S[6] + cc * cc * S[8] + 2.0 * (a * b * S[4] + a * cc * S[5] + b * cc * S[7]);
      }
    }
    double* s1 = p.rep ? p.rep + (size_t)(blockIdx.x % p.nrep) * 5 * C1 : p.stat;
    double* zz = p.rep ? s1 + 2 * C1 : p.zsum;
#pragma unroll
    for (int i = 0; i < 4; ++i) {
      atomicAdd(s1 + c + i, tot[i]);
      atomicAdd(s1 + C1 + c + i, tot[4 + i]);
#pragma unroll
      for (int k = 0; k < 3; ++k) atomicAdd(zz + (c + i) * 3 + k, tot[8 + 3 * i + k]);
    }
  }
  __shared__ unsigned last;
  wait_vm_complete();
  __syncthreads();
  unsigned* ticket = reinterpret_cast<unsigned*>(p.stat + 2 * C1);
  if (threadIdx.x == 0) last = atomicAdd(ticket, 1u) == gridDim.x - 1 ? 1u : 0u;
  __syncthreads();
  if (!last) return;
  const BnFinalize& fin = p.fin;
  if (p.rep) {
    for (int e = threadIdx.x; e < 5 * C1; e += 256) {
      double t = 0.0;
      for (int r = 0; r < p.nrep; ++r) t += __hip_atomic_load(p.rep + (size_t)r * 5 * C1 + e, __ATOMIC_RELAXED, __HIP_MEMORY_SCOPE_AGENT);
      if (e < 2 * C1) __hip_atomic_store(p.stat + e, t, __ATOMIC_RELAXED, __HIP_MEMORY_SCOPE_AGENT);
      else p.zsum[e - 2 * C1] = t;
    }
    __syncthreads();
  }
  for (int col = threadIdx.x; col < C1; col += 256) {
    const double s1 = __hip_atomic_load(p.stat + col, __ATOMIC_RELAXED, __HIP_MEMORY_SCOPE_AGENT);
    const double s2 = __hip_atomic_load(p.stat + C1 + col, __ATOMIC_RELAXED, __HIP_MEMORY_SCOPE_AGENT);
    const double m = s1 / (double)fin.rows;
    double var = s2 / (double)fin.rows - m * m;
    if (var < 0.0) var = 0.0;
    fin.mean[col] = (float)m;
    fin.invstd[col] = (float)(1.0 / sqrt(var + (double)fin.eps));
    if (fin.running_mean) {
      const double unbiased = fin.rows > 1 ? var * ((double)fin.rows / (double)(fin.rows - 1)) : var;
      fin.running_mean[col] = (float)((1.0 - fin.momentum) * (double)fin.running_mean[col] + fin.momentum * m);
      fin.running_var[col] = (float)((1.0 - fin.momentum) * (double)fin.running_var[col] + fin.momentum * unbiased);
    }
  }
  if (threadIdx.x == 0) {
    if (fin.num_batches_tracked) *fin.num_batches_tracked += 1;
    *ticket = 0u;
  }
}

struct SaBwd1Args {
  const float* dz1;
  const int* offsets;
  const int* slots;
  const float* zf;
  const float4* dsum;
  const float* wxyz;
  const float* mean;
  const float* invstd;
  const float* gamma;
  const double* stat;
  const float* tsum;
  const double* zsum;
  const double* gsum;
  float inv_rows;
  float* dgamma;
  float* dbeta;
  float* gz;
  float* dWx;
  int lddw;
  int B, N, M, C1;
};

__global__ __launch_bounds__(256) void sa_train_bwd1_kernel(SaBwd1Args p) {
  const int C1 = p.C1, C4 = C1 >> 2;
  if (blockIdx.x == 0 && blockIdx.y == 0) {
    const double* S = p.gsum;
    for (int t = threadIdx.x; t < C1 * 3; t += 256) {
      const int col = t / 3, k = t - col * 3;
      const double is = p.invstd[col], sc = (double)p.gamma[col] * is, mu = p.mean[col];
      const double db = p.stat[col] * (double)p.inv_rows, dg = p.stat[C1 + col] * (double)p.inv_rows;
      const double w0 = p.wxyz[col * 3 + 0], w1 = p.wxyz[col * 3 + 1], w2 = p.wxyz[col * 3 + 2];
      const double s2k0 = k == 0 ? S[3] : k == 1 ? S[4] : S[5], s2k1 = k == 0 ? S[4] : k == 1 ? S[6] : S[7], s2k2 = k == 0 ? S[5] : k == 1 ? S[7] : S[8];
      const double q = is * (p.zsum[col * 3 + k] + (w0 * s2k0 + w1 * s2k1 + w2 * s2k2) - mu * S[k]);
      double T = 0.0;
      for (int slot = 0; slot < 16; ++slot) T += (double)p.tsum[(size_t)slot * C1 * 4 + col * 4 + k];
      const double g = sc * ((T - db * S[k]) - dg * q);
      p.dWx[(size_t)col * p.lddw + k] += (float)g;
    }
    if (p.dgamma)
      for (int col = threadIdx.x; col < C1; col += 256) {
        p.dbeta[col] = (float)p.stat[col];
        p.dgamma[col] = (float)p.stat[C1 + col];
      }
  }
  const int b = blockIdx.y;
  const int64_t t = (int64_t)blockIdx.x * 256 + threadIdx.x;
  const int64_t j = t / C4;
  const int c = (int)(t - j * C4) * 4;
  if (j >= p.N) return;
  const int64_t E = (int64_t)p.M * 32;
  const int* o = p.offsets + (size_t)b * (p.N + 1) + j;
  const int p0 = o[0], p1 = o[1];
  const int* sl = p.slots + (size_t)b * E;
  const float* g = p.dz1 + (size_t)b * E * C1;
  float4 acc = make_float4(0.f, 0.f, 0.f, 0.f);
  int q = p0;
  for (; q + 3 < p1; q += 4) {
    int e[4];
#pragma unroll
    for (int u = 0; u < 4; ++u) e[u] = sl[q + u];
    float4 a[4];
#pragma unroll
    for (int u = 0; u < 4; ++u) a[u] = *reinterpret_cast<const float4*>(g + (size_t)e[u] * C1 + c);
#pragma unroll
    for (int u = 0; u < 4; ++u) {
      acc.x += a[u].x; acc.y += a[u].y; acc.z += a[u].z; acc.w += a[u].w;
    }
  }
  for (; q < p1; ++q) {
    const float4 a = *reinterpret_cast<const float4*>(g + (size_t)sl[q] * C1 + c);
    acc.x += a.x; acc.y += a.y; acc.z += a.z; acc.w += a.w;
  }
  const size_t pt = (size_t)b * p.N + j;
  const float4 z4 = *reinterpret_cast<const float4*>(p.zf + pt * C1 + c);
  const float4 d = p.dsum[pt];
  const float A[4] = {acc.x, acc.y, acc.z, acc.w}, z[4] = {z4.x, z4.y, z4.z, z4.w};
  float out[4];
#pragma unroll
  for (int i = 0; i < 4; ++i) {
    const int col = c + i;
    const float is = p.invstd[col], sc = p.gamma[col] * is, mu = p.mean[col];
    const float db = (float)p.stat[col] * p.inv_rows, dg = (float)p.stat[C1 + col] * p.inv_rows;
    const float wd = (p.wxyz[col * 3 + 0] * d.x + p.wxyz[col * 3 + 1] * d.y) + p.wxyz[col * 3 + 2] * d.z;
    const float xs = is * (d.w * (z[i] - mu) + wd);
    out[i] = sc * ((A[i] - d.w * db) - dg * xs);
  }
  *reinterpret_cast<float4*>(p.gz + pt * C1 + c) = make_float4(out[0], out[1], out[2], out[3]);
}

int blocks_of(int64_t c) { return c <= 32 ? 1 : c <= 64 ? 2 : 4; }

bool level_supported(int64_t K, int64_t C1, int64_t C2, int64_t C3) {
  return K == 32 && C1 >= 4 && C1 <= 64 && C2 <= 64 && C3 <= 128 && C1 % 4 == 0 && C2 % 4 == 0 && C3 % 4 == 0;
}

int64_t grid_for(int64_t G, int64_t lds_bytes, int64_t* tiles_per_wg, int64_t max_per_cu = 4) {
  const int64_t per_cu = std::max<int64_t>(1, std::min<int64_t>(max_per_cu, (150 * 1024) / lds_bytes));
  const int64_t wgs = std::max<int64_t>(1, std::min<int64_t>(std::min<int64_t>(1024, 256 * per_cu), cdiv(G, 16)));
  *tiles_per_wg = cdiv(cdiv(G, wgs), 4) * 4;
  return cdiv(G, *tiles_per_wg);
}

}

MVP_API int mvp_sa_train_forward_f32(int stage, const float* zf, const float* xyz, const float* centre, const int64_t* index, const float* wxyz,
                                     int64_t B, int64_t N, int64_t M, int64_t K, int64_t C1, const float* bn1_mean, const float* bn1_invstd,
                                     const float* bn1_gamma, const float* bn1_beta, const float* W2, int64_t C2, const float* bn2_mean,
                                     const float* bn2_invstd, const float* bn2_gamma, const float* bn2_beta, const float* W3, int64_t C3,
                                     double* stat, float eps, float momentum, float* mean, float* invstd, float* running_mean,
                                     float* running_var, int64_t* num_batches_tracked, float* ymax, float* ymin, uint8_t* amax,
                                     uint8_t* amin, mvp_stream_t stream) {
  MVP_NONNULL(zf);
  MVP_NONNULL(xyz);
  MVP_NONNULL(centre);
  MVP_NONNULL(index);
  MVP_NONNULL(wxyz);
  MVP_NONNULL(bn1_mean);
  MVP_NONNULL(bn1_invstd);
  MVP_NONNULL(bn1_gamma);
  MVP_NONNULL(bn1_beta);
  MVP_NONNULL(W2);
  MVP_NONNULL(stat);
  MVP_NONNULL(mean);
  MVP_NONNULL(invstd);
  MVP_REQUIRE(stage == 2 || stage == 3);
  MVP_REQUIRE(B >= 0 && N > 0 && M >= 0 && K > 0 && C1 > 0 && C2 > 0);
  if (stage == 3) {
    MVP_NONNULL(bn2_mean);
    MVP_NONNULL(bn2_invstd);
    MVP_NONNULL(bn2_gamma);
    MVP_NONNULL(bn2_beta);
    MVP_NONNULL(W3);
    MVP_NONNULL(ymax);
    MVP_NONNULL(ymin);
    MVP_NONNULL(amax);
    MVP_NONNULL(amin);
    MVP_REQUIRE(C3 > 0);
  }
  const int ns = mlp_fwd_pieces();
  if (ns == 0 || !level_supported(K, C1, C2, stage == 3 ? C3 : 4) || ((uintptr_t)zf % 16) != 0) return MVP_EUNSUPPORTED;
  if (B == 0 || M == 0) return MVP_OK;
  SaFwdArgs a;
  a.s.zf = zf; a.s.xyz = xyz; a.s.centre = centre; a.s.index = index; a.s.wxyz = wxyz;
  a.s.bn1[0] = bn1_mean; a.s.bn1[1] = bn1_invstd; a.s.bn1[2] = bn1_gamma; a.s.bn1[3] = bn1_beta;
  a.s.G = B * M; a.s.N = (int)N; a.s.M = (int)M; a.s.C1 = (int)C1;
  a.W2 = W2; a.C2 = (int)C2; a.W3 = W3; a.C3 = (int)(stage == 3 ? C3 : 0);
  a.bn2[0] = bn2_mean; a.bn2[1] = bn2_invstd; a.bn2[2] = bn2_gamma; a.bn2[3] = bn2_beta;
  a.stat = stat;
  a.fin = BnFinalize{B * M * K, eps, momentum, mean, invstd, running_mean, running_var, num_batches_tracked};
  a.ymax = ymax; a.ymin = ymin; a.amax = amax; a.amin = amin;
  const int c1b = blocks_of(C1), c2b = blocks_of(C2), c3b = stage == 3 ? blocks_of(C3) : 1;
  const int64_t lds = (int64_t)ns * 2048 * (c1b * c2b + (stage == 3 ? c2b * c3b : 0)) + 32 * 1024;
  const unsigned grid = (unsigned)grid_for(a.s.G, lds, &a.tiles_per_wg);
  hipStream_t s = static_cast<hipStream_t>(stream);
#define MVP_SAF(A_, B_, C_, ST_)                                                                                     \
  do {                                                                                                               \
    if (ns == 1) hipLaunchKernelGGL((sa_train_fwd_kernel<A_, B_, C_, 1, ST_>), dim3(grid), dim3(kFT), 0, s, a);       \
    else if (ns == 2) hipLaunchKernelGGL((sa_train_fwd_kernel<A_, B_, C_, 2, ST_>), dim3(grid), dim3(kFT), 0, s, a);  \
    else hipLaunchKernelGGL((sa_train_fwd_kernel<A_, B_, C_, 3, ST_>), dim3(grid), dim3(kFT), 0, s, a);               \
  } while (0)
  const int key = c1b * 100 + c2b * 10 + c3b;
  if (stage == 2) {
    switch (c1b * 10 + c2b) {
      case 11: MVP_SAF(1, 1, 1, 2); break;
      case 12: MVP_SAF(1, 2, 1, 2); break;
      case 21: MVP_SAF(2, 1, 1, 2); break;
      case 22: MVP_SAF(2, 2, 1, 2); break;
      default: return MVP_EUNSUPPORTED;
    }
  } else {
    switch (key) {
      case 111: MVP_SAF(1, 1, 1, 3); break;
      case 112: MVP_SAF(1, 1, 2, 3); break;
      case 121: MVP_SAF(1, 2, 1, 3); break;
      case 122: MVP_SAF(1, 2, 2, 3); break;
      case 211: MVP_SAF(2, 1, 1, 3); break;
      case 212: MVP_SAF(2, 1, 2, 3); break;
      case 221: MVP_SAF(2, 2, 1, 3); break;
      case 222: MVP_SAF(2, 2, 2, 3); break;
      case 224: MVP_SAF(2, 2, 4, 3); break;
      default: return MVP_EUNSUPPORTED;
    }
  }
#undef MVP_SAF
  return mvp_launch_status();
}

MVP_API int mvp_sa_train_backward_f32(int layer, const float* zf, const float* xyz, const float* centre, const int64_t* index,
                                      const float* wxyz, int64_t B, int64_t N, int64_t M, int64_t K, int64_t C1, const float* bn1_mean,
                                      const float* bn1_invstd, const float* bn1_gamma, const float* bn1_beta, const float* W2, int64_t C2,
                                      const float* bn2_mean, const float* bn2_invstd, const float* bn2_gamma, const float* bn2_beta,
                                      const float* W3, int64_t C3, const float* mean_i, const float* invstd_i, const float* gamma_i,
                                      const double* stat_i, float* dgamma_i, float* dbeta_i, int training, const float* G,
                                      const float* pool_dout, const float* pool_out, const uint8_t* pool_arg, float* dW, int64_t lddw,
                                      float* dZ, double* stat_prev, float* tsum, mvp_stream_t stream) {
  MVP_NONNULL(zf);
  MVP_NONNULL(xyz);
  MVP_NONNULL(centre);
  MVP_NONNULL(index);
  MVP_NONNULL(wxyz);
  MVP_NONNULL(bn1_mean);
  MVP_NONNULL(bn1_invstd);
  MVP_NONNULL(bn1_gamma);
  MVP_NONNULL(bn1_beta);
  MVP_NONNULL(W2);
  MVP_NONNULL(mean_i);
  MVP_NONNULL(invstd_i);
  MVP_NONNULL(gamma_i);
  MVP_NONNULL(stat_i);
  MVP_NONNULL(dW);
  MVP_NONNULL(dZ);
  MVP_NONNULL(stat_prev);
  MVP_REQUIRE(layer == 2 || layer == 3);
  MVP_REQUIRE(B >= 0 && N > 0 && M >= 0 && K > 0 && C1 > 0 && C2 > 0 && lddw > 0 && lddw < (1 << 24));
  if (layer == 3) {
    MVP_NONNULL(bn2_mean);
    MVP_NONNULL(bn2_invstd);
    MVP_NONNULL(bn2_gamma);
    MVP_NONNULL(bn2_beta);
    MVP_NONNULL(W3);
    MVP_NONNULL(pool_dout);
    MVP_NONNULL(pool_out);
    MVP_NONNULL(pool_arg);
    MVP_REQUIRE(C3 > 0 && lddw >= C2);
  } else {
    MVP_NONNULL(G);
    MVP_NONNULL(tsum);
    MVP_REQUIRE(lddw >= C1);
  }
  const int ns = mlp_bwd_pieces();
  if (ns == 0 || !level_supported(K, C1, C2, layer == 3 ? C3 : 4) || ((uintptr_t)zf % 16) != 0 || ((uintptr_t)dZ % 16) != 0) return MVP_EUNSUPPORTED;
  if (B == 0 || M == 0) return MVP_OK;
  SaBwdArgs a;
  a.s.zf = zf; a.s.xyz = xyz; a.s.centre = centre; a.s.index = index; a.s.wxyz = wxyz;
  a.s.bn1[0] = bn1_mean; a.s.bn1[1] = bn1_invstd; a.s.bn1[2] = bn1_gamma; a.s.bn1[3] = bn1_beta;
  a.s.G = B * M; a.s.N = (int)N; a.s.M = (int)M; a.s.C1 = (int)C1;
  a.W2 = W2; a.C2 = (int)C2; a.W3 = W3; a.C3 = (int)(layer == 3 ? C3 : 0);
  a.bn2[0] = bn2_mean; a.bn2[1] = bn2_invstd; a.bn2[2] = bn2_gamma; a.bn2[3] = bn2_beta;
  a.mean_i = mean_i; a.invstd_i = invstd_i; a.gamma_i = gamma_i; a.stat_i = stat_i;
  a.dgamma_i = dbeta_i ? dgamma_i : nullptr; a.dbeta_i = dbeta_i;
  a.inv_rows = training ? 1.0f / (float)(B * M * K) : 0.f;
  a.G = G; a.pool_dout = pool_dout; a.pool_out = pool_out; a.pool_arg = pool_arg;
  a.dW = dW; a.lddw = (int)lddw; a.dZ = dZ; a.stat_prev = stat_prev; a.tsum = tsum;
  const int c1b = blocks_of(C1), c2b = blocks_of(C2), c3b = layer == 3 ? blocks_of(C3) : 1;
  const int cb = layer == 3 ? c3b : c2b, cpb = layer == 3 ? c2b : c1b;
  const int nsf = (mlp_fwd_pieces() == 3) ? 3 : ns;
  const int64_t lds = (int64_t)2048 * (nsf * c1b * c2b + ns * ((layer == 3 ? c2b * c3b : 0) + cb * cpb)) + 32 * 1024;
  const bool narrow = layer == 3 ? c1b * c2b * c3b <= 2 : c1b * c2b == 1;
  const unsigned grid = (unsigned)grid_for(a.s.G, lds, &a.tiles_per_wg, narrow ? 2 : 1);
  hipStream_t s = static_cast<hipStream_t>(stream);
#define MVP_SAB(A_, B_, C_, L_)                                                                                          \
  do {                                                                                                                   \
    if (ns == 1 && nsf == 3) hipLaunchKernelGGL((sa_train_bwd_kernel<A_, B_, C_, 1, L_, 3>), dim3(grid), dim3(kFT), 0, s, a);      \
    else if (ns == 1) hipLaunchKernelGGL((sa_train_bwd_kernel<A_, B_, C_, 1, L_, 1>), dim3(grid), dim3(kFT), 0, s, a);             \
    else if (ns == 2 && nsf == 3) hipLaunchKernelGGL((sa_train_bwd_kernel<A_, B_, C_, 2, L_, 3>), dim3(grid), dim3(kFT), 0, s, a); \
    else if (ns == 2) hipLaunchKernelGGL((sa_train_bwd_kernel<A_, B_, C_, 2, L_, 2>), dim3(grid), dim3(kFT), 0, s, a);             \
    else hipLaunchKernelGGL((sa_train_bwd_kernel<A_, B_, C_, 3, L_, 3>), dim3(grid), dim3(kFT), 0, s, a);                          \
  } while (0)
  if (layer == 2) {
    switch (c1b * 10 + c2b) {
      case 11: MVP_SAB(1, 1, 1, 2); break;
      case 12: MVP_SAB(1, 2, 1, 2); break;
      case 21: MVP_SAB(2, 1, 1, 2); break;
      case 22: MVP_SAB(2, 2, 1, 2); break;
      default: return MVP_EUNSUPPORTED;
    }
  } else {
    switch (c1b * 100 + c2b * 10 + c3b) {
      case 111: MVP_SAB(1, 1, 1, 3); break;
      case 112: MVP_SAB(1, 1, 2, 3); break;
      case 121: MVP_SAB(1, 2, 1, 3); break;
      case 122: MVP_SAB(1, 2, 2, 3); break;
      case 211: MVP_SAB(2, 1, 1, 3); break;
      case 212: MVP_SAB(2, 1, 2, 3); break;
      case 221: MVP_SAB(2, 2, 1, 3); break;
      case 222: MVP_SAB(2, 2, 2, 3); break;
      case 224: MVP_SAB(2, 2, 4, 3); break;
      default: return MVP_EUNSUPPORTED;
    }
  }
#undef MVP_SAB
  return mvp_launch_status();
}

MVP_API int mvp_sa_geom_sums_f32(const int32_t* offsets, const int32_t* slots, const float* xyz, const float* centre, int64_t B, int64_t N,
                                 int64_t M, int64_t K, float* dsum, double* gsum, mvp_stream_t stream) {
  MVP_NONNULL(offsets);
  MVP_NONNULL(slots);
  MVP_NONNULL(xyz);
  MVP_NONNULL(centre);
  MVP_NONNULL(dsum);
  MVP_NONNULL(gsum);
  MVP_REQUIRE(B >= 0 && N > 0 && M >= 0);
  if (K != 32 || ((uintptr_t)dsum % 16) != 0) return MVP_EUNSUPPORTED;
  if (B == 0) return MVP_OK;
  const unsigned grid = (unsigned)std::max<int64_t>(1, std::min<int64_t>(1024, cdiv(B * N, 256)));
  hipLaunchKernelGGL(sa_geom_sums_kernel, dim3(grid), dim3(256), 0, static_cast<hipStream_t>(stream), offsets, slots, xyz, centre, (int)B, (int)N,
                     (int)M, reinterpret_cast<float4*>(dsum), gsum);
  return mvp_launch_status();
}

MVP_API int mvp_sa_train_stats1_ws_f32(const float* zf, const float* dsum, const float* wxyz, const double* gsum, int64_t B, int64_t N, int64_t M,
                                       int64_t K, int64_t C1, double* stat, double* zsum, float eps, float momentum, float* mean, float* invstd,
                                       float* running_mean, float* running_var, int64_t* num_batches_tracked, double* scratch,
                                       int64_t scratch_doubles, mvp_stream_t stream) {
  MVP_NONNULL(zf);
  MVP_NONNULL(dsum);
  MVP_NONNULL(wxyz);
  MVP_NONNULL(gsum);
  MVP_NONNULL(stat);
  MVP_NONNULL(zsum);
  MVP_NONNULL(mean);
  MVP_NONNULL(invstd);
  MVP_REQUIRE(B >= 0 && N > 0 && M >= 0 && K > 0 && C1 > 0);
  if (C1 % 4 != 0 || C1 > 1024 || 256 % (C1 / 4) != 0 || ((uintptr_t)zf % 16) != 0 || ((uintptr_t)dsum % 16) != 0) return MVP_EUNSUPPORTED;
  if (B == 0 || M == 0) return MVP_OK;
  MVP_REQUIRE(scratch_doubles >= 0 && (scratch != nullptr || scratch_doubles == 0));
  const int nrep = scratch ? (int)std::min<int64_t>(16, scratch_doubles / (5 * C1)) : 0;
  SaStats1Args a{zf, reinterpret_cast<const float4*>(dsum), wxyz, gsum, stat, zsum, nrep >= 2 ? scratch : nullptr, nrep,
                 BnFinalize{B * M * K, eps, momentum, mean, invstd, running_mean, running_var, num_batches_tracked}, B * N, (int)C1};
  const int64_t ppw = 256 / (C1 / 4);
  static const int wgs = []() { const char* e = getenv("MVP_SA_STATS1_WGS"); return e ? atoi(e) : 256; }();
  const unsigned grid = (unsigned)std::max<int64_t>(1, std::min<int64_t>(wgs, cdiv(B * N, ppw * 8)));
  hipLaunchKernelGGL(sa_train_stats1_kernel, dim3(grid), dim3(256), 0, static_cast<hipStream_t>(stream), a);
  return mvp_launch_status();
}

MVP_API int mvp_sa_train_stats1_f32(const float* zf, const float* dsum, const float* wxyz, const double* gsum, int64_t B, int64_t N, int64_t M,
                                    int64_t K, int64_t C1, double* stat, double* zsum, float eps, float momentum, float* mean, float* invstd,
                                    float* running_mean, float* running_var, int64_t* num_batches_tracked, mvp_stream_t stream) {
  return mvp_sa_train_stats1_ws_f32(zf, dsum, wxyz, gsum, B, N, M, K, C1, stat, zsum, eps, momentum, mean, invstd, running_mean, running_var,
                                    num_batches_tracked, nullptr, 0, stream);
}
// ... 30 lines not shown
```

Baseline: 5166 chunks/s.

## Add eight-wave workgroup variants for streaming MLP and SA stage-3 forward kernels

Moves the streaming MLP forward and SA train-forward kernel bodies into shared headers parameterised by wave count, and adds 8-wave (512-thread) instances for the widest configurations (KS=4, NB=4, NS=3 MLP; SA stage 3 with 2/2/4 blocks). With the default setting of 8 waves, these shapes launch with twice the waves per workgroup, sharing one staged copy of the weights in LDS across more waves and changing how tiles are split across workgroups. The aim is to spread the weight-staging cost over more tiles and hide more latency. The risk is fewer workgroups per CU, since the SA path caps at one per CU, plus some register pressure.

```diff
diff --git a/include/mvp_hip.h b/include/mvp_hip.h
--- a/include/mvp_hip.h
+++ b/include/mvp_hip.h
@@ -222,6 +222,8 @@
 
 int mvp_set_mlp_stream(int on);
 
+int mvp_set_forward_waves(int waves);
+
 int mvp_mlp_forward_f32(const float* X, int64_t R, int64_t Cin, int64_t ldx, const float* W, int64_t ldw, int64_t Cout,
                         const float* act_mean, const float* act_invstd, const float* act_gamma, const float* act_beta,
                         const float* bias, float* Y, double* stat, double* partial, mvp_stream_t stream);
diff --git a/mvpnet_amd/_lib.py b/mvpnet_amd/_lib.py
--- a/mvpnet_amd/_lib.py
+++ b/mvpnet_amd/_lib.py
@@ -145,7 +145,7 @@
 _SIGNATURES['mvp_mlp_input_grad_wide_p_f32'] = [_ptr] * 8 + [ctypes.c_int, _ptr, _i64, _ptr, _ptr, _ptr, _ptr, _ptr, _i64, _i64, _i64, _i64, _ptr, _ptr, _ptr, _i64,
                                                  ctypes.c_int, ctypes.c_int, _ptr]
 EXPORTS = ['mvp_version', 'mvp_strerror', 'mvp_lift_workspace_bytes', 'mvp_ball_query_grid_workspace', 'mvp_knn3_grid_workspace', 'mvp_mlp_weight_grad_workspace_floats', 'mvp_mlp_input_grad_wide_workspace_bytes', 'mvp_group_lin_partial_count', 'mvp_colstats_partial_count',
-           'mvp_set_mlp_precision', 'mvp_get_mlp_precision', 'mvp_mlp_layer_backward_partial_count', 'mvp_set_mlp_stream', 'mvp_set_mlp_precision_backward', 'mvp_get_mlp_precision_backward', 'mvp_mlp_precision_scope', 'mvp_set_fps_mode', 'mvp_fps_debug_spin_limit', 'mvp_fps_last_kernel'] + sorted(_SIGNATURES)
+           'mvp_set_mlp_precision', 'mvp_get_mlp_precision', 'mvp_mlp_layer_backward_partial_count', 'mvp_set_mlp_stream', 'mvp_set_forward_waves', 'mvp_set_mlp_precision_backward', 'mvp_get_mlp_precision_backward', 'mvp_mlp_precision_scope', 'mvp_set_fps_mode', 'mvp_fps_debug_spin_limit', 'mvp_fps_last_kernel'] + sorted(_SIGNATURES)
 
 
 def lib():
@@ -185,6 +185,8 @@
         _lib = handle
         handle.mvp_set_mlp_stream.restype = ctypes.c_int
         handle.mvp_set_mlp_stream.argtypes = [ctypes.c_int]
+        handle.mvp_set_forward_waves.restype = ctypes.c_int
+        handle.mvp_set_forward_waves.argtypes = [ctypes.c_int]
         handle.mvp_set_fps_mode.restype = ctypes.c_int
         handle.mvp_set_fps_mode.argtypes = [ctypes.c_int]
         handle.mvp_fps_debug_spin_limit.restype = ctypes.c_int
diff --git a/mvpnet_amd/csrc/mlp.hip b/mvpnet_amd/csrc/mlp.hip
--- a/mvpnet_amd/csrc/mlp.hip
+++ b/mvpnet_amd/csrc/mlp.hip
@@ -16,6 +16,9 @@
 thread_local int tl_mlp_terms = -1;
 thread_local int tl_mlp_terms_bwd = -1;
 int g_mlp_stream = 1;
+
+int g_fwd_waves = []() { const char* e = getenv("MVP_FWD_WAVES"); return (e && e[0] == '4' && e[1] == 0) ? 4 : 8; }();
+int g_fwd_waves_set = []() { const char* e = getenv("MVP_FWD_WAVES"); return (e && (e[0] == '4' || e[0] == '8') && e[1] == 0) ? 1 : 0; }();
 
 namespace {
 
@@ -1304,3 +1307,10 @@
   g_mlp_stream = on ? 1 : 0;
   return old;
 }
+MVP_API int mvp_set_forward_waves(int waves) {
+  if (waves != 4 && waves != 8) return MVP_EINVAL;
+  const int old = g_fwd_waves;
+  g_fwd_waves = waves;
+  g_fwd_waves_set = 1;
+  return old;
+}
diff --git a/mvpnet_amd/csrc/mlp_common.h b/mvpnet_amd/csrc/mlp_common.h
--- a/mvpnet_amd/csrc/mlp_common.h
+++ b/mvpnet_amd/csrc/mlp_common.h
@@ -3,6 +3,8 @@
 
 extern int g_mlp_terms;
 extern int g_mlp_terms_bwd;
+extern int g_fwd_waves;
+extern int g_fwd_waves_set;
 extern int g_mlp_min_width;
 
 extern thread_local int tl_mlp_terms;
diff --git a/mvpnet_amd/csrc/mlp_stream.hip b/mvpnet_amd/csrc/mlp_stream.hip
--- a/mvpnet_amd/csrc/mlp_stream.hip
+++ b/mvpnet_amd/csrc/mlp_stream.hip
@@ -29,252 +29,28 @@
 
 template <int KS, int NB, bool ACT, int NS, bool POOL>
 __global__ __launch_bounds__(kST) void mlp_stream_fwd_kernel(StreamArgs p) {
-  using SP = SplitPairs<NS>;
-  constexpr int kCols = NB * 32;
-  constexpr int kWBytes = KS * NS * kCols * 64;
-  __shared__ __attribute__((aligned(16))) unsigned char Wl[kWBytes];
-  __shared__ __attribute__((aligned(16))) float Ps[4][KS * 32];
-  __shared__ __attribute__((aligned(16))) float tiles[4][32 * kSLd];
-  __shared__ double sred[2][4][kCols];
-  const int tid = threadIdx.x, lane = tid & 63, wave = tid >> 6;
-  const int li = lane & 31, lh = lane >> 5;
-  const int Cin = p.Cin, Cout = p.Cout;
+  constexpr int NW = 4;
+#include "mlp_stream_body.h"
+}
 
-  for (int t = tid; t < kCols * KS * 8; t += kST) {
-    const int co = t % kCols, kqi = t / kCols;
-    const int k = 4 * kqi;
-    float v[4];
-#pragma unroll
-    for (int e = 0; e < 4; ++e) v[e] = (co < Cout && k + e < Cin) ? p.W[(size_t)co * p.ldw + k + e] : 0.f;
-    unsigned lo[NS], hi[NS];
-    split_pair<NS>(v[0], v[1], lo);
-    split_pair<NS>(v[2], v[3], hi);
-    const int slab = kqi >> 3, kq = (kqi & 7) * 4;
-    const int tt = kq >> 3, hh = (kq >> 2) & 1;
-    const int unit = 2 * (tt >> 1) + hh, half = tt & 1;
-#pragma unroll
-    for (int pc = 0; pc < NS; ++pc)
-      *reinterpret_cast<uint2*>(Wl + ((size_t)(slab * NS + pc) * kCols + co) * 64 + ((unit ^ ((co >> 2) & 3)) * 16) + half * 8) = make_uint2(lo[pc], hi[pc]);
-  }
-  if constexpr (ACT) {
-    for (int k = tid; k < KS * 32; k += kST) {
-      const int kc = min(k, Cin - 1);
-      Ps[0][k] = p.act.mean[kc];
-      Ps[1][k] = p.act.invstd[kc];
-      Ps[2][k] = p.act.gamma[kc];
-      Ps[3][k] = p.act.beta[kc];
+template <int KS, int NB, bool ACT, int NS>
+__global__ __launch_bounds__(2 * kST) void mlp_stream_fwd_w8_kernel(StreamArgs p) {
+  constexpr int NW = 8;
+  constexpr bool POOL = false;
+#include "mlp_stream_body.h"
+}
+
+constexpr bool stream_has_w8(int ks, int nb, int ns) { return ks == 4 && nb == 4 && ns == 3; }
+
+template <int KS, int NB, int NS>
+void launch_stream(const StreamArgs& a, unsigned grid, bool has_act, int waves, hipStream_t s) {
+  if constexpr (stream_has_w8(KS, NB, NS)) {
+    if (waves == 8 && !a.ymax) {
+      if (has_act) hipLaunchKernelGGL((mlp_stream_fwd_w8_kernel<KS, NB, true, NS>), dim3(grid), dim3(2 * kST), 0, s, a);
+      else hipLaunchKernelGGL((mlp_stream_fwd_w8_kernel<KS, NB, false, NS>), dim3(grid), dim3(2 * kST), 0, s, a);
+      return;
     }
   }
-  float bv[NB];
-#pragma unroll
-  for (int j = 0; j < NB; ++j) bv[j] = (p.bias && 32 * j + li < Cout) ? p.bias[32 * j + li] : 0.f;
-  float ssum[NB], qsum[NB];
-#pragma unroll
-  for (int j = 0; j < NB; ++j) ssum[j] = qsum[j] = 0.f;
-  __syncthreads();
-
-  const int64_t ntiles = (p.R + 31) / 32;
-  const int64_t t_begin = (int64_t)blockIdx.x * p.tiles_per_wg;
-  const int64_t t_end = min(ntiles, t_begin + p.tiles_per_wg);
-  float* st = tiles[wave];
-  constexpr int PF = KS == 1 ? 3 : KS == 2 ? 2 : 1;
-  float4 an[PF][KS][4];
-  auto load_a = [&](float4 (&dst)[KS][4], int64_t t) {
-    const int64_t row = min(t * 32 + li, p.R - 1);
-    const float* xrow = p.X + (size_t)row * p.ldx;
-#pragma unroll
-    for (int sl = 0; sl < KS; ++sl)
-#pragma unroll
-      for (int tt = 0; tt < 4; ++tt) dst[sl][tt] = *reinterpret_cast<const float4*>(xrow + min(32 * sl + 8 * tt + 4 * lh, Cin - 4));
-  };
-#pragma unroll
-  for (int u = 0; u < PF; ++u)
-    if (t_begin + wave + 4 * u < t_end) load_a(an[u], t_begin + wave + 4 * u);
-  for (int64_t tb = t_begin + wave; tb < t_end; tb += 4 * PF) {
-#pragma unroll
-   for (int u = 0; u < PF; ++u) {
-    const int64_t t = tb + 4 * u;
-    if (t >= t_end) break;
-    float4 ac[KS][4];
-#pragma unroll
-    for (int sl = 0; sl < KS; ++sl)
-#pragma unroll
-      for (int tt = 0; tt < 4; ++tt) ac[sl][tt] = an[u][sl][tt];
-    if (t + 4 * PF < t_end) load_a(an[u], t + 4 * PF);
-    f32x16 acc[NB];
-#pragma unroll
-    for (int j = 0; j < NB; ++j)
-#pragma unroll
-      for (int i = 0; i < 16; ++i) acc[j][i] = 0.f;
-#pragma unroll
-    for (int sl = 0; sl < KS; ++sl) {
-      float v[4][4];
-#pragma unroll
-      for (int tt = 0; tt < 4; ++tt) {
-        v[tt][0] = ac[sl][tt].x; v[tt][1] = ac[sl][tt].y; v[tt][2] = ac[sl][tt].z; v[tt][3] = ac[sl][tt].w;
-        if constexpr (ACT) {
-          const int k = 32 * sl + 8 * tt + 4 * lh;
-          const float4 m4 = *reinterpret_cast<const float4*>(&Ps[0][k]), i4 = *reinterpret_cast<const float4*>(&Ps[1][k]);
-          const float4 g4 = *reinterpret_cast<const float4*>(&Ps[2][k]), b4 = *reinterpret_cast<const float4*>(&Ps[3][k]);
-          const float pm[4] = {m4.x, m4.y, m4.z, m4.w}, pi[4] = {i4.x, i4.y, i4.z, i4.w};
-          const float pg[4] = {g4.x, g4.y, g4.z, g4.w}, pb[4] = {b4.x, b4.y, b4.z, b4.w};
-#pragma unroll
-          for (int e = 0; e < 4; ++e) {
-            const float a = ((v[tt][e] - pm[e]) * pi[e]) * pg[e] + pb[e];
-            v[tt][e] = a > 0.f ? a : 0.f;
-          }
-        }
-      }
-#pragma unroll
-      for (int s = 0; s < 2; ++s) {
-        unsigned q0[NS], q1[NS], q2[NS], q3[NS];
-        split_pair<NS>(v[2 * s][0], v[2 * s][1], q0);
-        split_pair<NS>(v[2 * s][2], v[2 * s][3], q1);
-        split_pair<NS>(v[2 * s + 1][0], v[2 * s + 1][1], q2);
-        split_pair<NS>(v[2 * s + 1][2], v[2 * s + 1][3], q3);
-        u32x4 af[NS];
-#pragma unroll
-        for (int pc = 0; pc < NS; ++pc) af[pc] = u32x4{q0[pc], q1[pc], q2[pc], q3[pc]};
-        constexpr int JG = NB >= 2 ? 2 : 1;
-#pragma unroll
-        for (int j0 = 0; j0 < NB; j0 += JG) {
-          u32x4 bfr[JG][NS];
-#pragma unroll
-          for (int jj = 0; jj < JG; ++jj) {
-            const int co = 32 * (j0 + jj) + li;
-#pragma unroll
-            for (int pc = 0; pc < NS; ++pc)
-              bfr[jj][pc] = *reinterpret_cast<const u32x4*>(Wl + ((size_t)(sl * NS + pc) * kCols + co) * 64 + (((2 * s + lh) ^ ((co >> 2) & 3)) * 16));
-          }
-#pragma unroll
-          for (int qd = 0; qd < SP::N; ++qd)
-#pragma unroll
-            for (int jj = 0; jj < JG; ++jj)
-              acc[j0 + jj] = __builtin_amdgcn_mfma_f32_32x32x16_bf16(__builtin_bit_cast(bf16x8, af[SP::A[qd]]),
-                                                                     __builtin_bit_cast(bf16x8, bfr[jj][SP::B[qd]]), acc[j0 + jj], 0, 0, 0);
-        }
-      }
-    }
-    const int64_t r0 = t * 32;
-#pragma unroll
-    for (int j = 0; j < NB; ++j) {
-      const bool cok = 32 * j + li < Cout;
-      float s = 0.f, q = 0.f;
-      if constexpr (POOL) {
-        float vmax = -INFINITY, vmin = INFINITY;
-        int rmax = 0, rmin = 0;
-#pragma unroll
-        for (int i = 0; i < 16; ++i) {
-          const int m = (i & 3) + 8 * (i >> 2) + 4 * lh;
-          const float y = acc[j][i] + bv[j];
-          s += y;
-          q += y * y;
-          if (y > vmax) { vmax = y; rmax = m; }
-          if (y < vmin) { vmin = y; rmin = m; }
-        }
-        const float omax = __shfl_xor(vmax, 32, kWave), omin = __shfl_xor(vmin, 32, kWave);
-        const int ormax = __shfl_xor(rmax, 32, kWave), ormin = __shfl_xor(rmin, 32, kWave);
-        if (omax > vmax || (omax == vmax && ormax < rmax)) { vmax = omax; rmax = ormax; }
-        if (omin < vmin || (omin == vmin && ormin < rmin)) { vmin = omin; rmin = ormin; }
-        if (lh == 0 && cok) {
-          const size_t o = (size_t)t * Cout + 32 * j + li;
-          p.ymax[o] = vmax;
-          p.ymin[o] = vmin;
-          p.amax[o] = (uint8_t)rmax;
-          p.amin[o] = (uint8_t)rmin;
-        }
-        if (!cok) s = q = 0.f;
-        ssum[j] += s;
-        qsum[j] += q;
-        continue;
-      }
-#pragma unroll
-      for (int i = 0; i < 16; ++i) {
-        const int m = (i & 3) + 8 * (i >> 2) + 4 * lh;
-        float y = acc[j][i] + bv[j];
-        y = (r0 + m < p.R && cok) ? y : 0.f;
-        s += y;
-        q += y * y;
-        st[m * kSLd + li] = y;
-      }
-      ssum[j] += s;
-      qsum[j] += q;
-      __builtin_amdgcn_wave_barrier();
-#pragma unroll
-      for (int pp = 0; pp < 4; ++pp) {
-        const int row = pp * 8 + (lane >> 3), c4 = (lane & 7) * 4;
-        const f32x4 vv = *reinterpret_cast<const f32x4*>(st + row * kSLd + c4);
-        const int64_t r = r0 + row;
-        const int cc = 32 * j + c4;
-        if (r < p.R && cc < Cout) __builtin_nontemporal_store(vv, reinterpret_cast<f32x4*>(p.Y + (size_t)r * Cout + cc));
-      }
-      __builtin_amdgcn_wave_barrier();
-    }
-   }
-  }
-  if (p.partial) {
-#pragma unroll
-    for (int j = 0; j < NB; ++j) {
-      const float s = ssum[j] + __shfl_xor(ssum[j], 32, kWave), q = qsum[j] + __shfl_xor(qsum[j], 32, kWave);
-      if (lane < 32) {
-        sred[0][wave][32 * j + li] = (double)s;
-        sred[1][wave][32 * j + li] = (double)q;
-      }
-    }
-    __syncthreads();
-    for (int col = tid; col < kCols; col += kST)
-      if (col < Cout) {
-        p.partial[((size_t)blockIdx.x * 2 + 0) * Cout + col] = sred[0][0][col] + sred[0][1][col] + sred[0][2][col] + sred[0][3][col];
-        p.partial[((size_t)blockIdx.x * 2 + 1) * Cout + col] = sred[1][0][col] + sred[1][1][col] + sred[1][2][col] + sred[1][3][col];
-      }
-  } else if (p.stat) {
-#pragma unroll
-    for (int j = 0; j < NB; ++j) {
-      const float s = ssum[j] + __shfl_xor(ssum[j], 32, kWave), q = qsum[j] + __shfl_xor(qsum[j], 32, kWave);
-      if (lane < 32) {
-        sred[0][wave][32 * j + li] = (double)s;
-        sred[1][wave][32 * j + li] = (double)q;
-      }
-    }
-    __syncthreads();
-    for (int col = tid; col < kCols; col += kST)
-      if (col < Cout) {
-        atomicAdd(p.stat + col, sred[0][0][col] + sred[0][1][col] + sred[0][2][col] + sred[0][3][col]);
-        atomicAdd(p.stat + Cout + col, sred[1][0][col] + sred[1][1][col] + sred[1][2][col] + sred[1][3][col]);
-      }
-    if (p.finalize) {
-      __shared__ unsigned last;
-      wait_vm_complete();
-      __syncthreads();
-      unsigned* ticket = reinterpret_cast<unsigned*>(p.stat + 2 * Cout);
-      if (tid == 0) last = atomicAdd(ticket, 1u) == gridDim.x - 1 ? 1u : 0u;
-      __syncthreads();
-      if (!last) return;
-      const BnFinalize& fin = p.fin;
-      for (int c = tid; c < Cout; c += kST) {
-        const double s1 = __hip_atomic_load(p.stat + c, __ATOMIC_RELAXED, __HIP_MEMORY_SCOPE_AGENT);
-        const double s2 = __hip_atomic_load(p.stat + Cout + c, __ATOMIC_RELAXED, __HIP_MEMORY_SCOPE_AGENT);
-        const double m = s1 / (double)fin.rows;
-        double var = s2 / (double)fin.rows - m * m;
-        if (var < 0.0) var = 0.0;
-        fin.mean[c] = (float)m;
-        fin.invstd[c] = (float)(1.0 / sqrt(var + (double)fin.eps));
-        if (fin.running_mean) {
-          const double unbiased = fin.rows > 1 ? var * ((double)fin.rows / (double)(fin.rows - 1)) : var;
-          fin.running_mean[c] = (float)((1.0 - fin.momentum) * (double)fin.running_mean[c] + fin.momentum * m);
-          fin.running_var[c] = (float)((1.0 - fin.momentum) * (double)fin.running_var[c] + fin.momentum * unbiased);
-        }
-      }
-      if (tid == 0) {
-        if (fin.num_batches_tracked) *fin.num_batches_tracked += 1;
-        *ticket = 0u;
-      }
-    }
-  }
-}
-
-template <int KS, int NB, int NS>
-void launch_stream(const StreamArgs& a, unsigned grid, bool has_act, hipStream_t s) {
   if (a.ymax) {
     if (has_act) hipLaunchKernelGGL((mlp_stream_fwd_kernel<KS, NB, true, NS, true>), dim3(grid), dim3(kST), 0, s, a);
     else hipLaunchKernelGGL((mlp_stream_fwd_kernel<KS, NB, false, NS, true>), dim3(grid), dim3(kST), 0, s, a);
@@ -301,17 +77,18 @@
   const int64_t ntiles = cdiv(R, 32);
   const int ks = (int)cdiv(Cin, 32), nb = Cout <= 32 ? 1 : Cout <= 64 ? 2 : 4;
   const int64_t lds = (int64_t)ks * ns * nb * 32 * 64;
-  const int64_t per_cu = std::max<int64_t>(1, std::min<int64_t>(4, (140 * 1024) / (lds + 24 * 1024)));
+  const int waves = (g_fwd_waves == 8 && (g_fwd_waves_set || !act.mean) && !ymax && stream_has_w8(ks, nb, ns)) ? 8 : 4;
+  const int64_t per_cu = std::max<int64_t>(1, std::min<int64_t>(4, (140 * 1024) / (lds + waves * 6 * 1024)));
   int64_t wgs = std::min<int64_t>(256 * per_cu, std::min<int64_t>(cdiv(R, 128), cdiv(ntiles, 16)));
   wgs = std::max<int64_t>(wgs, 1);
-  a.tiles_per_wg = cdiv(cdiv(ntiles, wgs), 4) * 4;
+  a.tiles_per_wg = cdiv(cdiv(ntiles, wgs), waves) * waves;
   const unsigned grid = (unsigned)cdiv(ntiles, a.tiles_per_wg);
   const bool has_act = act.mean != nullptr;
 #define MVP_STREAM(KS_, NB_)                                                      \
   do {                                                                            \
-    if (ns == 1) launch_stream<KS_, NB_, 1>(a, grid, has_act, s);                  \
-    else if (ns == 2) launch_stream<KS_, NB_, 2>(a, grid, has_act, s);             \
-    else launch_stream<KS_, NB_, 3>(a, grid, has_act, s);                          \
+    if (ns == 1) launch_stream<KS_, NB_, 1>(a, grid, has_act, waves, s);                  \
+    else if (ns == 2) launch_stream<KS_, NB_, 2>(a, grid, has_act, waves, s);             \
+    else launch_stream<KS_, NB_, 3>(a, grid, has_act, waves, s);                          \
   } while (0)
 #define MVP_STREAM_NB(KS_)                       \
   do {                                           \
diff --git a/mvpnet_amd/csrc/mlp_stream_body.h b/mvpnet_amd/csrc/mlp_stream_body.h
--- /dev/null
+++ b/mvpnet_amd/csrc/mlp_stream_body.h
@@ -0,0 +1,277 @@
+  using SP = SplitPairs<NS>;
+  constexpr int kThreads = 64 * NW;
+  constexpr bool SLABWISE = NW == 8;
+  static_assert(!SLABWISE || !POOL, "no pooled two-wave instances");
+  constexpr int kCols = NB * 32;
+  constexpr int kWBytes = KS * NS * kCols * 64;
+  __shared__ __attribute__((aligned(16))) unsigned char Wl[kWBytes];
+  __shared__ __attribute__((aligned(16))) float Ps[4][KS * 32];
+  __shared__ __attribute__((aligned(16))) float tiles[NW][32 * kSLd];
+  __shared__ double sred[2][NW][kCols];
+  const int tid = threadIdx.x, lane = tid & 63, wave = tid >> 6;
+  const int li = lane & 31, lh = lane >> 5;
+  const int Cin = p.Cin, Cout = p.Cout;
+
+  for (int t = tid; t < kCols * KS * 8; t += kThreads) {
+    const int co = t % kCols, kqi = t / kCols;
+    const int k = 4 * kqi;
+    float v[4];
+#pragma unroll
+    for (int e = 0; e < 4; ++e) v[e] = (co < Cout && k + e < Cin) ? p.W[(size_t)co * p.ldw + k + e] : 0.f;
+    unsigned lo[NS], hi[NS];
+    split_pair<NS>(v[0], v[1], lo);
+    split_pair<NS>(v[2], v[3], hi);
+    const int slab = kqi >> 3, kq = (kqi & 7) * 4;
+    const int tt = kq >> 3, hh = (kq >> 2) & 1;
+    const int unit = 2 * (tt >> 1) + hh, half = tt & 1;
+#pragma unroll
+    for (int pc = 0; pc < NS; ++pc)
+      *reinterpret_cast<uint2*>(Wl + ((size_t)(slab * NS + pc) * kCols + co) * 64 + ((unit ^ ((co >> 2) & 3)) * 16) + half * 8) = make_uint2(lo[pc], hi[pc]);
+  }
+  if constexpr (ACT) {
+    for (int k = tid; k < KS * 32; k += kThreads) {
+      const int kc = min(k, Cin - 1);
+      Ps[0][k] = p.act.mean[kc];
+      Ps[1][k] = p.act.invstd[kc];
+      Ps[2][k] = p.act.gamma[kc];
+      Ps[3][k] = p.act.beta[kc];
+    }
+  }
+  float bv[NB];
+#pragma unroll
+  for (int j = 0; j < NB; ++j) bv[j] = (p.bias && 32 * j + li < Cout) ? p.bias[32 * j + li] : 0.f;
+  float ssum[NB], qsum[NB];
+#pragma unroll
+  for (int j = 0; j < NB; ++j) ssum[j] = qsum[j] = 0.f;
+  __syncthreads();
+
+  const unsigned char* wlo[2];
+  const unsigned char* whi[2];
+#pragma unroll
+  for (int s = 0; s < 2; ++s) {
+    wlo[s] = Wl + li * 64 + (((2 * s + lh) ^ ((li >> 2) & 3)) * 16);
+    unsigned hi = 65536u;
+    if constexpr (SLABWISE) asm volatile("" : "+v"(hi));
+    whi[s] = wlo[s] + hi;
+  }
+  const int64_t ntiles = (p.R + 31) / 32;
+  const int64_t t_begin = (int64_t)blockIdx.x * p.tiles_per_wg;
+  const int64_t t_end = min(ntiles, t_begin + p.tiles_per_wg);
+  float* st = tiles[wave];
+  constexpr int PF = SLABWISE ? 1 : KS == 1 ? 3 : KS == 2 ? 2 : 1;
+  float4 an[PF][KS][4];
+  auto load_a = [&](float4 (&dst)[KS][4], int64_t t) {
+    const int64_t row = min(t * 32 + li, p.R - 1);
+    const float* xrow = p.X + (size_t)row * p.ldx;
+#pragma unroll
+    for (int sl = 0; sl < KS; ++sl)
+#pragma unroll
+      for (int tt = 0; tt < 4; ++tt) dst[sl][tt] = *reinterpret_cast<const float4*>(xrow + min(32 * sl + 8 * tt + 4 * lh, Cin - 4));
+  };
+  auto load_slab = [&](float4 (&dst)[4], int64_t t, int sl) {
+    const int64_t row = min(t * 32 + li, p.R - 1);
+    const float* xrow = p.X + (size_t)row * p.ldx;
+    int k0 = 4 * lh;
+    asm volatile("" : "+v"(k0));
+#pragma unroll
+    for (int tt = 0; tt < 4; ++tt) dst[tt] = *reinterpret_cast<const float4*>(xrow + min(32 * sl + 8 * tt + k0, Cin - 4));
+  };
+#pragma unroll
+  for (int u = 0; u < PF; ++u)
+    if (t_begin + wave + NW * u < t_end) load_a(an[u], t_begin + wave + NW * u);
+  for (int64_t tb = t_begin + wave; tb < t_end; tb += NW * PF) {
+#pragma unroll
+   for (int u = 0; u < PF; ++u) {
+    const int64_t t = tb + NW * u;
+    if (t >= t_end) break;
+    float4 ac[SLABWISE ? 1 : KS][4];
+    if constexpr (!SLABWISE) {
+#pragma unroll
+      for (int sl = 0; sl < KS; ++sl)
+#pragma unroll
+        for (int tt = 0; tt < 4; ++tt) ac[sl][tt] = an[u][sl][tt];
+      if (t + NW * PF < t_end) load_a(an[u], t + NW * PF);
+    }
+    f32x16 acc[NB];
+#pragma unroll
+    for (int j = 0; j < NB; ++j)
+#pragma unroll
+      for (int i = 0; i < 16; ++i) acc[j][i] = 0.f;
+#pragma unroll
+    for (int sl = 0; sl < KS; ++sl) {
+      float v[4][4];
+#pragma unroll
+      for (int tt = 0; tt < 4; ++tt) {
+        const float4 a4 = SLABWISE ? an[u][sl][tt] : ac[SLABWISE ? 0 : sl][tt];
+        v[tt][0] = a4.x; v[tt][1] = a4.y; v[tt][2] = a4.z; v[tt][3] = a4.w;
+        if constexpr (ACT) {
+          const int k = 32 * sl + 8 * tt + 4 * lh;
+          const float4 m4 = *reinterpret_cast<const float4*>(&Ps[0][k]), i4 = *reinterpret_cast<const float4*>(&Ps[1][k]);
+          const float4 g4 = *reinterpret_cast<const float4*>(&Ps[2][k]), b4 = *reinterpret_cast<const float4*>(&Ps[3][k]);
+          const float pm[4] = {m4.x, m4.y, m4.z, m4.w}, pi[4] = {i4.x, i4.y, i4.z, i4.w};
+          const float pg[4] = {g4.x, g4.y, g4.z, g4.w}, pb[4] = {b4.x, b4.y, b4.z, b4.w};
+#pragma unroll
+          for (int e = 0; e < 4; ++e) {
+            const float a = ((v[tt][e] - pm[e]) * pi[e]) * pg[e] + pb[e];
+            v[tt][e] = a > 0.f ? a : 0.f;
+          }
+        }
+      }
+      if constexpr (SLABWISE) load_slab(an[u][sl], t + NW, sl);
+#pragma unroll
+      for (int s = 0; s < 2; ++s) {
+        unsigned q0[NS], q1[NS], q2[NS], q3[NS];
+        split_pair<NS>(v[2 * s][0], v[2 * s][1], q0);
+        split_pair<NS>(v[2 * s][2], v[2 * s][3], q1);
+        split_pair<NS>(v[2 * s + 1][0], v[2 * s + 1][1], q2);
+        split_pair<NS>(v[2 * s + 1][2], v[2 * s + 1][3], q3);
+        u32x4 af[NS];
+#pragma unroll
+        for (int pc = 0; pc < NS; ++pc) af[pc] = u32x4{q0[pc], q1[pc], q2[pc], q3[pc]};
+        constexpr int JG = NB >= 2 ? 2 : 1;
+#pragma unroll
+        for (int j0 = 0; j0 < NB; j0 += JG) {
+          u32x4 bfr[JG][NS];
+#pragma unroll
+          for (int jj = 0; jj < JG; ++jj) {
+            const int co = 32 * (j0 + jj) + li;
+#pragma unroll
+            for (int pc = 0; pc < NS; ++pc)
+              if constexpr (SLABWISE) {
+                const unsigned off = ((unsigned)(sl * NS + pc) * kCols + 32 * (j0 + jj)) * 64;
+                bfr[jj][pc] = *reinterpret_cast<const u32x4*>((off < 65536u ? wlo[s] : whi[s]) + (off & 65535u));
+              } else {
+                bfr[jj][pc] = *reinterpret_cast<const u32x4*>(Wl + ((size_t)(sl * NS + pc) * kCols + co) * 64 + (((2 * s + lh) ^ ((co >> 2) & 3)) * 16));
+              }
+          }
+#pragma unroll
+          for (int qd = 0; qd < SP::N; ++qd)
+#pragma unroll
+            for (int jj = 0; jj < JG; ++jj)
+              acc[j0 + jj] = __builtin_amdgcn_mfma_f32_32x32x16_bf16(__builtin_bit_cast(bf16x8, af[SP::A[qd]]),
+                                                                     __builtin_bit_cast(bf16x8, bfr[jj][SP::B[qd]]), acc[j0 + jj], 0, 0, 0);
+        }
+      }
+    }
+    const int64_t r0 = t * 32;
+#pragma unroll
+    for (int j = 0; j < NB; ++j) {
+      const bool cok = 32 * j + li < Cout;
+      float s = 0.f, q = 0.f;
+      if constexpr (POOL) {
+        float vmax = -INFINITY, vmin = INFINITY;
+        int rmax = 0, rmin = 0;
+#pragma unroll
+        for (int i = 0; i < 16; ++i) {
+          const int m = (i & 3) + 8 * (i >> 2) + 4 * lh;
+          const float y = acc[j][i] + bv[j];
+          s += y;
+          q += y * y;
+          if (y > vmax) { vmax = y; rmax = m; }
+          if (y < vmin) { vmin = y; rmin = m; }
+        }
+        const float omax = __shfl_xor(vmax, 32, kWave), omin = __shfl_xor(vmin, 32, kWave);
+        const int ormax = __shfl_xor(rmax, 32, kWave), ormin = __shfl_xor(rmin, 32, kWave);
+        if (omax > vmax || (omax == vmax && ormax < rmax)) { vmax = omax; rmax = ormax; }
+        if (omin < vmin || (omin == vmin && ormin < rmin)) { vmin = omin; rmin = ormin; }
+        if (lh == 0 && cok) {
+          const size_t o = (size_t)t * Cout + 32 * j + li;
+          p.ymax[o] = vmax;
+          p.ymin[o] = vmin;
+          p.amax[o] = (uint8_t)rmax;
+          p.amin[o] = (uint8_t)rmin;
+        }
+        if (!cok) s = q = 0.f;
+        ssum[j] += s;
+        qsum[j] += q;
+        continue;
+      }
+#pragma unroll
+      for (int i = 0; i < 16; ++i) {
+        const int m = (i & 3) + 8 * (i >> 2) + 4 * lh;
+        float y = acc[j][i] + bv[j];
+        y = (r0 + m < p.R && cok) ? y : 0.f;
+        s += y;
+        q += y * y;
+        st[m * kSLd + li] = y;
+      }
+      ssum[j] += s;
+      qsum[j] += q;
+      __builtin_amdgcn_wave_barrier();
+#pragma unroll
+      for (int pp = 0; pp < 4; ++pp) {
+        const int row = pp * 8 + (lane >> 3), c4 = (lane & 7) * 4;
+        const f32x4 vv = *reinterpret_cast<const f32x4*>(st + row * kSLd + c4);
+        const int64_t r = r0 + row;
+        const int cc = 32 * j + c4;
+        if (r < p.R && cc < Cout) __builtin_nontemporal_store(vv, reinterpret_cast<f32x4*>(p.Y + (size_t)r * Cout + cc));
+      }
+      __builtin_amdgcn_wave_barrier();
+    }
+   }
+  }
+  auto wave_sum = [&](int which, int col) {
+    double r = sred[which][0][col];
+#pragma unroll
+    for (int w = 1; w < NW; ++w) r += sred[which][w][col];
+    return r;
+  };
+  if (p.partial) {
+#pragma unroll
+    for (int j = 0; j < NB; ++j) {
+      const float s = ssum[j] + __shfl_xor(ssum[j], 32, kWave), q = qsum[j] + __shfl_xor(qsum[j], 32, kWave);
+      if (lane < 32) {
+        sred[0][wave][32 * j + li] = (double)s;
+        sred[1][wave][32 * j + li] = (double)q;
+      }
+    }
+    __syncthreads();
+    for (int col = tid; col < kCols; col += kThreads)
+      if (col < Cout) {
+        p.partial[((size_t)blockIdx.x * 2 + 0) * Cout + col] = wave_sum(0, col);
+        p.partial[((size_t)blockIdx.x * 2 + 1) * Cout + col] = wave_sum(1, col);
+      }
+  } else if (p.stat) {
+#pragma unroll
+    for (int j = 0; j < NB; ++j) {
+      const float s = ssum[j] + __shfl_xor(ssum[j], 32, kWave), q = qsum[j] + __shfl_xor(qsum[j], 32, kWave);
+      if (lane < 32) {
+        sred[0][wave][32 * j + li] = (double)s;
+        sred[1][wave][32 * j + li] = (double)q;
+      }
+    }
+    __syncthreads();
+    for (int col = tid; col < kCols; col += kThreads)
+      if (col < Cout) {
+        atomicAdd(p.stat + col, wave_sum(0, col));
+        atomicAdd(p.stat + Cout + col, wave_sum(1, col));
+      }
+    if (p.finalize) {
+      __shared__ unsigned last;
+      wait_vm_complete();
+      __syncthreads();
+      unsigned* ticket = reinterpret_cast<unsigned*>(p.stat + 2 * Cout);
+      if (tid == 0) last = atomicAdd(ticket, 1u) == gridDim.x - 1 ? 1u : 0u;
+      __syncthreads();
+      if (!last) return;
+      const BnFinalize& fin = p.fin;
+      for (int c = tid; c < Cout; c += kThreads) {
+        const double s1 = __hip_atomic_load(p.stat + c, __ATOMIC_RELAXED, __HIP_MEMORY_SCOPE_AGENT);
+        const double s2 = __hip_atomic_load(p.stat + Cout + c, __ATOMIC_RELAXED, __HIP_MEMORY_SCOPE_AGENT);
+        const double m = s1 / (double)fin.rows;
+        double var = s2 / (double)fin.rows - m * m;
+        if (var < 0.0) var = 0.0;
+        fin.mean[c] = (float)m;
+        fin.invstd[c] = (float)(1.0 / sqrt(var + (double)fin.eps));
+        if (fin.running_mean) {
+          const double unbiased = fin.rows > 1 ? var * ((double)fin.rows / (double)(fin.rows - 1)) : var;
+          fin.running_mean[c] = (float)((1.0 - fin.momentum) * (double)fin.running_mean[c] + fin.momentum * m);
+          fin.running_var[c] = (float)((1.0 - fin.momentum) * (double)fin.running_var[c] + fin.momentum * unbiased);
+        }
+      }
+      if (tid == 0) {
+        if (fin.num_batches_tracked) *fin.num_batches_tracked += 1;
+        *ticket = 0u;
+      }
+    }
+  }
diff --git a/mvpnet_amd/csrc/sa_common.h b/mvpnet_amd/csrc/sa_common.h
--- a/mvpnet_amd/csrc/sa_common.h
+++ b/mvpnet_amd/csrc/sa_common.h
@@ -7,9 +7,9 @@
 constexpr int kFLd = 36;
 
 
-template <int NS>
+template <int NS, int NT = kFT>
 __device__ __forceinline__ void stage_weight(unsigned char* Wl, const float* __restrict__ W, int Cout, int Cin, int cols, int slabs, int tid) {
-  for (int t = tid; t < cols * slabs * 8; t += kFT) {
+  for (int t = tid; t < cols * slabs * 8; t += NT) {
     const int co = t % cols, kqi = t / cols;
     const int k = 4 * kqi;
     float v[4];
diff --git a/mvpnet_amd/csrc/sa_train.hip b/mvpnet_amd/csrc/sa_train.hip
--- a/mvpnet_amd/csrc/sa_train.hip
+++ b/mvpnet_amd/csrc/sa_train.hip
@@ -16,9 +16,9 @@
   int N, M, C1;
 };
 
-template <int C1B>
+template <int C1B, int NT = kFT>
 __device__ __forceinline__ void stage_layer1(const SaSrc& p, float* P1 , float (*Wx)[4], int tid) {
-  for (int k = tid; k < C1B * 32; k += kFT) {
+  for (int k = tid; k < C1B * 32; k += NT) {
     const int kc = min(k, p.C1 - 1);
 #pragma unroll
     for (int a = 0; a < 4; ++a) P1[a * (C1B * 32) + k] = p.bn1[a] ? p.bn1[a][kc] : 0.f;
@@ -92,8 +92,8 @@
     }
 }
 
-template <int NB>
-__device__ __forceinline__ void stats_tail(const float (&ssum)[NB], const float (&qsum)[NB], double (*sred)[4][NB * 32], double* stat, int C,
+template <int NB, int NW = 4>
+__device__ __forceinline__ void stats_tail(const float (&ssum)[NB], const float (&qsum)[NB], double (*sred)[NW][NB * 32], double* stat, int C,
                                            const BnFinalize& fin, bool finalize) {
   const int tid = threadIdx.x, lane = tid & 63, wave = tid >> 6, li = lane & 31;
 #pragma unroll
@@ -105,10 +105,16 @@
     }
   }
   __syncthreads();
-  for (int col = tid; col < NB * 32; col += kFT)
+  for (int col = tid; col < NB * 32; col += 64 * NW)
     if (col < C) {
-      atomicAdd(stat + col, sred[0][0][col] + sred[0][1][col] + sred[0][2][col] + sred[0][3][col]);
-      atomicAdd(stat + C + col, sred[1][0][col] + sred[1][1][col] + sred[1][2][col] + sred[1][3][col]);
+      double s = sred[0][0][col], q = sred[1][0][col];
+#pragma unroll
+      for (int w = 1; w < NW; ++w) {
+        s += sred[0][w][col];
+        q += sred[1][w][col];
+      }
+      atomicAdd(stat + col, s);
+      atomicAdd(stat + C + col, q);
     }
   if (!finalize) return;
   __shared__ unsigned last;
@@ -118,7 +124,7 @@
   if (tid == 0) last = atomicAdd(ticket, 1u) == gridDim.x - 1 ? 1u : 0u;
   __syncthreads();
   if (!last) return;
-  for (int c = tid; c < C; c += kFT) {
+  for (int c = tid; c < C; c += 64 * NW) {
     const double s1 = __hip_atomic_load(stat + c, __ATOMIC_RELAXED, __HIP_MEMORY_SCOPE_AGENT);
     const double s2 = __hip_atomic_load(stat + C + c, __ATOMIC_RELAXED, __HIP_MEMORY_SCOPE_AGENT);
     const double m = s1 / (double)fin.rows;
@@ -155,130 +161,14 @@
 
 template <int C1B, int C2B, int C3B, int NS, int STAGE>
 __global__ __launch_bounds__(kFT) void sa_train_fwd_kernel(SaFwdArgs p) {
-  constexpr bool PF = STAGE == 2;
-  constexpr int kW2 = C1B * NS * C2B * 32 * 64;
-  constexpr int kW3 = STAGE == 3 ? C2B * NS * C3B * 32 * 64 : 16;
-  constexpr int NBS = STAGE == 3 ? C3B : C2B;
-  __shared__ __attribute__((aligned(16))) unsigned char W2l[kW2];
-  __shared__ __attribute__((aligned(16))) unsigned char W3l[kW3];
-  __shared__ __attribute__((aligned(16))) float P1[4 * C1B * 32];
-  __shared__ __attribute__((aligned(16))) float Wx[C1B * 32][4];
-  __shared__ __attribute__((aligned(16))) float tiles[4][32 * kFLd];
-  __shared__ double sred[2][4][NBS * 32];
-  const int tid = threadIdx.x, lane = tid & 63, wave = tid >> 6;
-  const int li = lane & 31, lh = lane >> 5;
-  const int C1 = p.s.C1, C2 = p.C2, C3 = p.C3;
-  stage_weight<NS>(W2l, p.W2, C2, C1, C2B * 32, C1B, tid);
-  if constexpr (STAGE == 3) stage_weight<NS>(W3l, p.W3, C3, C2, C3B * 32, C2B, tid);
-  stage_layer1<C1B>(p.s, P1, Wx, tid);
-  float m2[C2B], i2[C2B], g2[C2B], b2[C2B];
-#pragma unroll
-  for (int j = 0; j < C2B; ++j) {
-    m2[j] = i2[j] = g2[j] = b2[j] = 0.f;
-    if constexpr (STAGE == 3) {
-      const int col = min(32 * j + li, C2 - 1);
-      m2[j] = p.bn2[0][col]; i2[j] = p.bn2[1][col]; g2[j] = p.bn2[2][col]; b2[j] = p.bn2[3][col];
-    }
-  }
-  float ssum[NBS], qsum[NBS];
-#pragma unroll
-  for (int j = 0; j < NBS; ++j) ssum[j] = qsum[j] = 0.f;
-  __syncthreads();
-  float* st = tiles[wave];
-  const int64_t t_begin = (int64_t)blockIdx.x * p.tiles_per_wg;
-  const int64_t t_end = min(p.s.G, t_begin + p.tiles_per_wg);
-  int g = __builtin_amdgcn_readfirstlane((int)(t_begin + wave));
-  BallRows<C1B> rn;
-  int64_t jn = -1;
-  if (PF) {
-    if (g < t_end) gather_issue<C1B>(p.s, g, p.s.index[(size_t)g * 32 + li], lh, rn);
-    if (g + 4 < t_end) jn = p.s.index[(size_t)(g + 4) * 32 + li];
-  } else if (g < t_end) {
-    jn = p.s.index[(size_t)g * 32 + li];
-  }
-  for (; g < t_end; g += 4) {
-    BallRows<C1B> rc = rn;
-    if (PF && g + 4 < t_end) {
-      gather_issue<C1B>(p.s, g + 4, jn, lh, rn);
-      if (g + 8 < t_end) jn = p.s.index[(size_t)(g + 8) * 32 + li];
-    }
-    if (!PF) {
-      const int64_t j = jn;
-      if (g + 4 < t_end) jn = p.s.index[(size_t)(g + 4) * 32 + li];
-      gather_issue<C1B>(p.s, g, j, lh, rc);
-    }
-    float v1[C1B][4][4], dif[3];
-    gather_finish<C1B>(rc, lh, Wx, v1, dif);
-    act_rows<C1B>(v1, P1, lh);
-    f32x16 acc2[C2B];
-    layer_mfma<C1B, C2B, NS>(v1, W2l, li, lh, acc2);
-    if constexpr (STAGE == 2) {
-#pragma unroll
-      for (int jb = 0; jb < C2B; ++jb) {
-        float s = 0.f, q = 0.f;
-#pragma unroll
-        for (int i = 0; i < 16; ++i) {
-          const float y = acc2[jb][i];
-          s += y;
-          q += y * y;
-        }
-        ssum[jb] += s;
-        qsum[jb] += q;
-      }
-    } else {
-      float v2[C2B][4][4];
-#pragma unroll
-      for (int jb = 0; jb < C2B; ++jb) {
-#pragma unroll
-        for (int i = 0; i < 16; ++i) {
-          const int m = (i & 3) + 8 * (i >> 2) + 4 * lh;
-          const float a = ((acc2[jb][i] - m2[jb]) * i2[jb]) * g2[jb] + b2[jb];
-          st[m * kFLd + li] = a > 0.f ? a : 0.f;
-        }
-        __builtin_amdgcn_wave_barrier();
-#pragma unroll
-        for (int tt = 0; tt < 4; ++tt) {
-          const float4 a = *reinterpret_cast<const float4*>(st + li * kFLd + 8 * tt + 4 * lh);
-          v2[jb][tt][0] = a.x; v2[jb][tt][1] = a.y; v2[jb][tt][2] = a.z; v2[jb][tt][3] = a.w;
-        }
-        __builtin_amdgcn_wave_barrier();
-      }
-      f32x16 acc3[C3B];
-      layer_mfma<C2B, C3B, NS>(v2, W3l, li, lh, acc3);
-#pragma unroll
-      for (int jb = 0; jb < C3B; ++jb) {
-        const bool cok = 32 * jb + li < C3;
-        float s = 0.f, q = 0.f;
-        float vmax = -INFINITY, vmin = INFINITY;
-        int rmax = 0, rmin = 0;
-#pragma unroll
-        for (int i = 0; i < 16; ++i) {
-          const int m = (i & 3) + 8 * (i >> 2) + 4 * lh;
-          const float y = acc3[jb][i];
-          s += y;
-          q += y * y;
-          if (y > vmax) { vmax = y; rmax = m; }
-          if (y < vmin) { vmin = y; rmin = m; }
-        }
-        const float omax = __shfl_xor(vmax, 32, kWave), omin = __shfl_xor(vmin, 32, kWave);
-        const int ormax = __shfl_xor(rmax, 32, kWave), ormin = __shfl_xor(rmin, 32, kWave);
-        if (omax > vmax || (omax == vmax && ormax < rmax)) { vmax = omax; rmax = ormax; }
-        if (omin < vmin || (omin == vmin && ormin < rmin)) { vmin = omin; rmin = ormin; }
-        if (lh == 0 && cok) {
-          const size_t ob = (size_t)g * C3;
-          const unsigned o = (unsigned)(32 * jb + li);
-          (p.ymax + ob)[o] = vmax;
-          (p.ymin + ob)[o] = vmin;
-          (p.amax + ob)[o] = (uint8_t)rmax;
-          (p.amin + ob)[o] = (uint8_t)rmin;
-        }
-        if (!cok) s = q = 0.f;
-        ssum[jb] += s;
-        qsum[jb] += q;
-      }
-    }
-  }
-  stats_tail<NBS>(ssum, qsum, sred, p.stat, STAGE == 3 ? C3 : C2, p.fin, true);
+  constexpr int NW = 4;
+#include "sa_train_fwd_body.h"
+}
+
+template <int C1B, int C2B, int C3B, int NS, int STAGE>
+__global__ __launch_bounds__(2 * kFT) void sa_train_fwd_w8_kernel(SaFwdArgs p) {
+  constexpr int NW = 8;
+#include "sa_train_fwd_body.h"
 }
 
 struct SaBwdArgs {
@@ -957,10 +847,10 @@
   return K == 32 && C1 >= 4 && C1 <= 64 && C2 <= 64 && C3 <= 128 && C1 % 4 == 0 && C2 % 4 == 0 && C3 % 4 == 0;
 }
 
-int64_t grid_for(int64_t G, int64_t lds_bytes, int64_t* tiles_per_wg, int64_t max_per_cu = 4) {
+int64_t grid_for(int64_t G, int64_t lds_bytes, int64_t* tiles_per_wg, int64_t max_per_cu = 4, int64_t waves = 4) {
   const int64_t per_cu = std::max<int64_t>(1, std::min<int64_t>(max_per_cu, (150 * 1024) / lds_bytes));
   const int64_t wgs = std::max<int64_t>(1, std::min<int64_t>(std::min<int64_t>(1024, 256 * per_cu), cdiv(G, 16)));
-  *tiles_per_wg = cdiv(cdiv(G, wgs), 4) * 4;
+  *tiles_per_wg = cdiv(cdiv(G, wgs), waves) * waves;
   return cdiv(G, *tiles_per_wg);
 }
 
@@ -1014,7 +904,8 @@
   a.ymax = ymax; a.ymin = ymin; a.amax = amax; a.amin = amin;
   const int c1b = blocks_of(C1), c2b = blocks_of(C2), c3b = stage == 3 ? blocks_of(C3) : 1;
   const int64_t lds = (int64_t)ns * 2048 * (c1b * c2b + (stage == 3 ? c2b * c3b : 0)) + 32 * 1024;
-  const unsigned grid = (unsigned)grid_for(a.s.G, lds, &a.tiles_per_wg);
+  const bool w8 = g_fwd_waves == 8 && stage == 3 && ns == 3 && c1b == 2 && c2b == 2 && c3b == 4;
+  const unsigned grid = w8 ? (unsigned)grid_for(a.s.G, lds + 16 * 1024, &a.tiles_per_wg, 1, 8) : (unsigned)grid_for(a.s.G, lds, &a.tiles_per_wg);
   hipStream_t s = static_cast<hipStream_t>(stream);
 #define MVP_SAF(A_, B_, C_, ST_)                                                                                     \
   do {                                                                                                               \
@@ -1041,7 +932,10 @@
       case 212: MVP_SAF(2, 1, 2, 3); break;
       case 221: MVP_SAF(2, 2, 1, 3); break;
       case 222: MVP_SAF(2, 2, 2, 3); break;
-      case 224: MVP_SAF(2, 2, 4, 3); break;
+      case 224:
+        if (w8) hipLaunchKernelGGL((sa_train_fwd_w8_kernel<2, 2, 4, 3, 3>), dim3(grid), dim3(2 * kFT), 0, s, a);
+        else MVP_SAF(2, 2, 4, 3);
+        break;
       default: return MVP_EUNSUPPORTED;
     }
   }
diff --git a/mvpnet_amd/csrc/sa_train_fwd_body.h b/mvpnet_amd/csrc/sa_train_fwd_body.h
--- /dev/null
+++ b/mvpnet_amd/csrc/sa_train_fwd_body.h
@@ -0,0 +1,125 @@
+  constexpr int kThreads = 64 * NW;
+  constexpr bool PF = STAGE == 2;
+  constexpr int kW2 = C1B * NS * C2B * 32 * 64;
+  constexpr int kW3 = STAGE == 3 ? C2B * NS * C3B * 32 * 64 : 16;
+  constexpr int NBS = STAGE == 3 ? C3B : C2B;
+  __shared__ __attribute__((aligned(16))) unsigned char W2l[kW2];
+  __shared__ __attribute__((aligned(16))) unsigned char W3l[kW3];
+  __shared__ __attribute__((aligned(16))) float P1[4 * C1B * 32];
+  __shared__ __attribute__((aligned(16))) float Wx[C1B * 32][4];
+  __shared__ __attribute__((aligned(16))) float tiles[NW][32 * kFLd];
+  __shared__ double sred[2][NW][NBS * 32];
+  const int tid = threadIdx.x, lane = tid & 63, wave = tid >> 6;
+  const int li = lane & 31, lh = lane >> 5;
+  const int C1 = p.s.C1, C2 = p.C2, C3 = p.C3;
+  stage_weight<NS, kThreads>(W2l, p.W2, C2, C1, C2B * 32, C1B, tid);
+  if constexpr (STAGE == 3) stage_weight<NS, kThreads>(W3l, p.W3, C3, C2, C3B * 32, C2B, tid);
+  stage_layer1<C1B, kThreads>(p.s, P1, Wx, tid);
+  float m2[C2B], i2[C2B], g2[C2B], b2[C2B];
+#pragma unroll
+  for (int j = 0; j < C2B; ++j) {
+    m2[j] = i2[j] = g2[j] = b2[j] = 0.f;
+    if constexpr (STAGE == 3) {
+      const int col = min(32 * j + li, C2 - 1);
+      m2[j] = p.bn2[0][col]; i2[j] = p.bn2[1][col]; g2[j] = p.bn2[2][col]; b2[j] = p.bn2[3][col];
+    }
+  }
+  float ssum[NBS], qsum[NBS];
+#pragma unroll
+  for (int j = 0; j < NBS; ++j) ssum[j] = qsum[j] = 0.f;
+  __syncthreads();
+  float* st = tiles[wave];
+  const int64_t t_begin = (int64_t)blockIdx.x * p.tiles_per_wg;
+  const int64_t t_end = min(p.s.G, t_begin + p.tiles_per_wg);
+  int g = __builtin_amdgcn_readfirstlane((int)(t_begin + wave));
+  BallRows<C1B> rn;
+  int64_t jn = -1;
+  if (PF) {
+    if (g < t_end) gather_issue<C1B>(p.s, g, p.s.index[(size_t)g * 32 + li], lh, rn);
+    if (g + NW < t_end) jn = p.s.index[(size_t)(g + NW) * 32 + li];
+  } else if (g < t_end) {
+    jn = p.s.index[(size_t)g * 32 + li];
+  }
+  for (; g < t_end; g += NW) {
+    BallRows<C1B> rc = rn;
+    if (PF && g + NW < t_end) {
+      gather_issue<C1B>(p.s, g + NW, jn, lh, rn);
+      if (g + 2 * NW < t_end) jn = p.s.index[(size_t)(g + 2 * NW) * 32 + li];
+    }
+    if (!PF) {
+      const int64_t j = jn;
+      if (g + NW < t_end) jn = p.s.index[(size_t)(g + NW) * 32 + li];
+      gather_issue<C1B>(p.s, g, j, lh, rc);
+    }
+    float v1[C1B][4][4], dif[3];
+    gather_finish<C1B>(rc, lh, Wx, v1, dif);
+    act_rows<C1B>(v1, P1, lh);
+    f32x16 acc2[C2B];
+    layer_mfma<C1B, C2B, NS>(v1, W2l, li, lh, acc2);
+    if constexpr (STAGE == 2) {
+#pragma unroll
+      for (int jb = 0; jb < C2B; ++jb) {
+        float s = 0.f, q = 0.f;
+#pragma unroll
+        for (int i = 0; i < 16; ++i) {
+          const float y = acc2[jb][i];
+          s += y;
+          q += y * y;
+        }
+        ssum[jb] += s;
+        qsum[jb] += q;
+      }
+    } else {
+      float v2[C2B][4][4];
+#pragma unroll
+      for (int jb = 0; jb < C2B; ++jb) {
+#pragma unroll
+        for (int i = 0; i < 16; ++i) {
+          const int m = (i & 3) + 8 * (i >> 2) + 4 * lh;
+          const float a = ((acc2[jb][i] - m2[jb]) * i2[jb]) * g2[jb] + b2[jb];
+          st[m * kFLd + li] = a > 0.f ? a : 0.f;
+        }
+        __builtin_amdgcn_wave_barrier();
+#pragma unroll
+        for (int tt = 0; tt < 4; ++tt) {
+          const float4 a = *reinterpret_cast<const float4*>(st + li * kFLd + 8 * tt + 4 * lh);
+          v2[jb][tt][0] = a.x; v2[jb][tt][1] = a.y; v2[jb][tt][2] = a.z; v2[jb][tt][3] = a.w;
+        }
+        __builtin_amdgcn_wave_barrier();
+      }
+      f32x16 acc3[C3B];
+      layer_mfma<C2B, C3B, NS>(v2, W3l, li, lh, acc3);
+#pragma unroll
+      for (int jb = 0; jb < C3B; ++jb) {
+        const bool cok = 32 * jb + li < C3;
+        float s = 0.f, q = 0.f;
+        float vmax = -INFINITY, vmin = INFINITY;
+        int rmax = 0, rmin = 0;
+#pragma unroll
+        for (int i = 0; i < 16; ++i) {
+          const int m = (i & 3) + 8 * (i >> 2) + 4 * lh;
+          const float y = acc3[jb][i];
+          s += y;
+          q += y * y;
+          if (y > vmax) { vmax = y; rmax = m; }
+          if (y < vmin) { vmin = y; rmin = m; }
+        }
+        const float omax = __shfl_xor(vmax, 32, kWave), omin = __shfl_xor(vmin, 32, kWave);
+        const int ormax = __shfl_xor(rmax, 32, kWave), ormin = __shfl_xor(rmin, 32, kWave);
+        if (omax > vmax || (omax == vmax && ormax < rmax)) { vmax = omax; rmax = ormax; }
+        if (omin < vmin || (omin == vmin && ormin < rmin)) { vmin = omin; rmin = ormin; }
+        if (lh == 0 && cok) {
+          const size_t ob = (size_t)g * C3;
+          const unsigned o = (unsigned)(32 * jb + li);
+          (p.ymax + ob)[o] = vmax;
+          (p.ymin + ob)[o] = vmin;
+          (p.amax + ob)[o] = (uint8_t)rmax;
+          (p.amin + ob)[o] = (uint8_t)rmin;
+        }
+        if (!cok) s = q = 0.f;
+        ssum[jb] += s;
+        qsum[jb] += q;
+      }
+    }
+  }
+  stats_tail<NBS, NW>(ssum, qsum, sred, p.stat, STAGE == 3 ? C3 : C2, p.fin, true);
```

Result: no change. 5197 chunks/s (median of 4 runs) (+0.6%).
